# vivian556123/NeurIPS2024-CoVoMix

Measured on AMD Instinct MI355X. Metric: mel-frames/sec (VoMix 32-step + HiFi-GAN, Bx1000x80), higher is better.
Workload: dtype f16x3->f32 (fp32 operands split into fp16 hi/lo pairs, 3 MFMA products, fp32 accumulate); 1 GPU; VoMix 32-NFE (16 midpoint steps, CFG 0.7) + HiFi-GAN config_covomix, B=8 utterances x T=1000 frames per GPU, prompt 400; per_gpu_batch=8, frames=1000, nfe=32, parallelism=dp1 (utterance-sharded)

## Files before the change

### include/covomix_hip.h

```cpp
#ifndef COVOMIX_HIP_H
#define COVOMIX_HIP_H

#include <stdint.h>

#ifdef __cplusplus
extern "C" {
#endif

#define CVX_OK      0
#define CVX_EINVAL (-22)
#define CVX_EHIP   (-5)

#define CVX_ACT_NONE 0
#define CVX_ACT_GELU 1
#define CVX_ACT_SILU 2
#define CVX_ACT_TANH 3

typedef struct cvx_ctx {
    void*     stream;
    uint32_t* sat_flag;
    int32_t   n_cus;
    int32_t   flags;
} cvx_ctx;
#define CVX_CTX_NO_SATURATION_FLAG 1
typedef const cvx_ctx* cvx_stream_t;

#define CVX_ABI_VERSION 113
int         cvx_version(void);
const char* cvx_last_error_string(void);

int cvx_saturation_flag_reset(cvx_stream_t ctx);
int cvx_saturation_flag_query(uint32_t* host_out, int32_t reset, cvx_stream_t ctx);

int cvx_clock_stamps(uint64_t* stamps_dev, cvx_stream_t ctx);
int cvx_stream_create_cu_mask(const uint32_t* mask, int32_t n_words, void** out_stream);
int cvx_stream_destroy(void* stream);

typedef struct {
    const float* A;   int64_t lda;
    const float* A2;  int64_t lda2;  int32_t K1;
    const float* W;   int64_t ldw;
    float*       C;   int64_t ldc;
    const float* bias;
    const float* residual; int64_t ldr;
    int32_t M, N, K;
    int32_t act;
    const float* rope_cos; const float* rope_sin; int32_t rope_T; int32_t rope_cols;
} cvx_gemm_args;
int cvx_gemm_bias_act_f32(const cvx_gemm_args* a, cvx_stream_t s);

#define CVX_GEMM_F32_FORM_T64          0
#define CVX_GEMM_F32_FORM_T64_GENERIC  1
#define CVX_GEMM_F32_FORM_T128_DMA     2
#define CVX_GEMM_F32_FORM_T128_GENERIC 3
int cvx_gemm_f32_form(int32_t M, int32_t N, int32_t K);

typedef struct {
    const uint16_t* A_hi;  const uint16_t* A_lo;  int64_t lda_h;
    const uint16_t* A2_hi; const uint16_t* A2_lo; int64_t lda2_h;
    uint16_t* C_hi; uint16_t* C_lo; int64_t ldc_h;
    int32_t write_f32;
    uint16_t* Vt_hi; uint16_t* Vt_lo; int64_t vt_ld;
    float* workspace; int64_t workspace_floats;
    int32_t w_interleaved;
    int32_t flags;
    const float* a_scale_dev; const float* c_scale_dev; const float* vt_scale_dev;
    const float* c_gamma_dev; float* c_rowsq; int64_t c_rowsq_ld; const float* a_row_scale_dev;
    const uint16_t* R_hi; const uint16_t* R_lo; int64_t ldr_h; const float* r_scale_dev;
    const float* a2_scale_dev;
} cvx_gemm_split_io;
#define CVX_GEMM_FLAG_MEDIUM 8
#define CVX_GEMM_FLAG_NO_MEDIUM 16
#define CVX_GEMM_FLAG_ONE_TILE 4
#define CVX_GEMM_FLAG_TILE192 64
#define CVX_GEMM_FLAG_TILE256 128
#define CVX_GEMM_FLAG_TILE_MIXED 32
#define CVX_GEMM_FLAG_VT_PIECES 512
int cvx_split_f16(const float* w, uint16_t* hi, uint16_t* lo, int64_t n, float scale, cvx_stream_t s);
int cvx_split_f16_colscale_il(const float* W, int64_t ldw, int32_t N, int32_t K, const float* colscale, int64_t cs_ld,
                              const float* set_scale_dev, int64_t ss_ld, int32_t n_sets, float scale, uint16_t* out, cvx_stream_t s);
int cvx_split_f16_dev(const float* w, uint16_t* hi, uint16_t* lo, int64_t n, float scale, const float* scale_dev, cvx_stream_t s);
int cvx_gemm_f16x3(const cvx_gemm_args* a, const uint16_t* W_hi, const uint16_t* W_lo, float acc_scale,
                   const cvx_gemm_split_io* io, cvx_stream_t s);
typedef struct {
    const float* gamma; const float* beta;
    uint16_t* Y_hi; uint16_t* Y_lo; int64_t ldy_h;
    const float* y_scale_dev;
    float scale; float eps;
} cvx_gemm_norm;
int cvx_gemm_f16x3_norm(const cvx_gemm_args* a, const uint16_t* W_hi, const uint16_t* W_lo, float acc_scale,
                        const cvx_gemm_split_io* io, const cvx_gemm_norm* norm, cvx_stream_t s);
int64_t cvx_gemm_f16x3_workspace_floats(int32_t M, int32_t N, int32_t K, int32_t K1);

int cvx_adarmsnorm_f32(const float* x, const float* gamma, const float* beta, float* y,
                       uint16_t* y_hi, uint16_t* y_lo,
                       int64_t rows, int32_t D, int64_t rows_per_group, float scale, float eps,
                       cvx_stream_t s);
int cvx_rownorm_scale_f32(const float* rowsq, int64_t rows, int32_t parts, int64_t ld, float scale, float eps, float* out, cvx_stream_t s);
int cvx_adarmsnorm_scaled_f32(const float* x, const float* gamma, const float* beta, float* y,
                              uint16_t* y_hi, uint16_t* y_lo,
                              int64_t rows, int32_t D, int64_t rows_per_group, float scale, float eps,
                              const float* split_scale_dev, cvx_stream_t s);

int cvx_attention_f32(const float* qkv, float* out,
                      uint16_t* out_hi, uint16_t* out_lo,
                      int32_t Bt, int32_t T, int32_t H, float scale, cvx_stream_t s);

int cvx_attention_varlen_f32(const float* qkv, float* out, uint16_t* out_hi, uint16_t* out_lo,
                             const int32_t* cu_seqlens_dev, int32_t n_seq, int32_t max_T, int32_t H, float scale, cvx_stream_t s);

int cvx_attention_f16x3(const uint16_t* qk_hi, const uint16_t* qk_lo, const uint16_t* vt_hi, const uint16_t* vt_lo,
                        float* out, uint16_t* out_hi, uint16_t* out_lo,
                        int32_t Bt, int32_t T, int32_t Tp, int32_t H, float scale, cvx_stream_t s);
int cvx_attention_f16x3_scaled(const uint16_t* qk_hi, const uint16_t* qk_lo, const uint16_t* vt_hi, const uint16_t* vt_lo,
                               float* out, uint16_t* out_hi, uint16_t* out_lo,
                               int32_t Bt, int32_t T, int32_t Tp, int32_t H, float scale,
                               const float* qk_scale_dev, const float* v_scale_dev, const float* out_scale_dev, cvx_stream_t s);
int cvx_attention_f16x3_varlen(const uint16_t* qk_hi, const uint16_t* qk_lo, const uint16_t* vt_hi, const uint16_t* vt_lo,
                               float* out, uint16_t* out_hi, uint16_t* out_lo, const int32_t* cu_seqlens_dev,
                               int32_t n_seq, int32_t max_T, int64_t M, int32_t vt_ld, int32_t H, float scale,
                               const float* qk_scale_dev, const float* v_scale_dev, const float* out_scale_dev, cvx_stream_t s);

#define CVX_ATT_FORM_A 0
#define CVX_ATT_FORM_B 1
#define CVX_ATT_FORM_C 2
#define CVX_ATT_FORM_D 3
#define CVX_ATT_FORM_SINGLE_TERM 4
int cvx_attention_f16x3_form(int32_t n_seq, int32_t max_T, int64_t q_rows, int32_t H, int32_t single_term,
                             int32_t* query_block, int32_t* key_groups, int32_t* query_waves);

int cvx_dwconv31_gelu_res_f32(const float* x, const float* w, const float* bias, float* y,
                              int32_t Bt, int32_t T, int32_t C, cvx_stream_t s);
int cvx_dwconv31_gelu_res_varlen_f32(const float* x, const float* w, const float* bias, float* y,
                                     const int32_t* cu_seqlens_dev, int32_t n_seq, int32_t max_T, int32_t C, cvx_stream_t s);
int cvx_gemm_skinny_f32(const float* A, int32_t lda, const float* W, int64_t ldw, const float* bias, float* C, int64_t ldc,
                        int32_t M, int32_t N, int32_t K, int32_t act, cvx_stream_t s);
int cvx_cfg_combine_axpy_f32(const float* f_c, const float* f_n, const float* y, float cond_scale,
                             float coef, float* out, float* out2, float* out3, int64_t n, cvx_stream_t s);
int cvx_rk_stage_f32(const float* f_c, const float* f_n, const float* y, float cond_scale, const float* row_scale,
                     const float* const* k_prev, const float* w, int32_t m, float* k_out, float* out, float* out2, float* out3,
                     int64_t rows, int32_t dim, cvx_stream_t s);
#define CVX_RK_ERR_ROWS 32
int cvx_rk_stage_err_f32(const float* f_c, const float* f_n, const float* y, float cond_scale, const float* row_scale,
                         const float* const* k_prev, const float* w, const float* we, int32_t m, float* k_out, float* out, float* out2,
                         float* out3, int64_t rows, int32_t dim, const int32_t* map_dev, const int32_t* map_host, int32_t blocks,
                         float* partials, cvx_stream_t s);
int cvx_rk_err_finish_f32(const float* partials, const int32_t* map_dev, int32_t blocks, int32_t steps, int32_t n_seq, float* err,
                          cvx_stream_t s);

int cvx_embed_gather_f32(const int64_t* ids, int32_t S, const float* table, int32_t E, int32_t n_rows_table,
                         const float* cond, const float* cond_row, int32_t Cc, int64_t null_id,
                         float* out, int64_t M, cvx_stream_t s);

int cvx_time_fourier_f32(const float* times, const float* w, float* out, int32_t n, int32_t half,
                         cvx_stream_t s);

typedef struct { const int32_t* item_len_dev; int32_t mul, add; } cvx_item_lengths;
typedef struct {
    const float* x;  int32_t B, Cin, Lin;
    const float* Wp; const float* bias;
    float* out;      int32_t Cout, Lout;
    int32_t ksize, dil, pad, up;
    float in_slope;
    const float* res; const float* accum; float out_scale;
    cvx_item_lengths items;
} cvx_conv_args;
int     cvx_hifigan_conv1d_f32(const cvx_conv_args* a, cvx_stream_t s);
int64_t cvx_hifigan_packed_weight_floats(int32_t Cout, int32_t Cin, int32_t ksize);
int     cvx_hifigan_pack_weight_f32(const float* w, int32_t Cout, int32_t Cin, int32_t ksize,
                                    int32_t transposed, float* Wp);

int     cvx_hifigan_conv_transpose1d_f32(const cvx_conv_args* a, uint32_t* amax_bits_dev, cvx_stream_t s);
int64_t cvx_hifigan_conv_transpose1d_packed_floats(int32_t Cout, int32_t Cin, int32_t ksize, int32_t stride, int32_t pad_t);
int     cvx_hifigan_pack_conv_transpose1d_f32(const float* w, int32_t Cin, int32_t Cout, int32_t ksize, int32_t stride,
                                              int32_t pad_t, float* Wp);
int     cvx_pow2_scale_from_amax_f32(uint32_t* amax_bits_dev, float target, float* scale_dev, cvx_stream_t s);

int cvx_hifigan_post_f32(const float* x, const float* w, float bias, float* y,
                         int32_t B, int32_t Cin, int32_t L, float slope, cvx_stream_t s);

typedef struct {
    const uint16_t *z_hi, *z_lo;
    int32_t B, L, Lp, Cp_in, halo_l;
    const uint16_t *w_hi, *w_lo;
    float acc_scale;
    const float* bias;
    int32_t Np, ksize, dil;
    const float* res;
    const float* accum;
    float* out_x;
    float out_scale;
    uint16_t *out_zhi, *out_zlo;
    float z_slope;
    const float* z_scale_dev;
    cvx_item_lengths items;
} cvx_conv16_args;
int cvx_hifigan_conv1d_f16x3(const cvx_conv16_args* a, cvx_stream_t s);
int cvx_hifigan_conv1d_group_f16x3(const cvx_conv16_args* a, int32_t n, cvx_stream_t s);
int cvx_hifigan_conv1d_f16x3_form(int32_t Np, int32_t L, int32_t B, int32_t n_problems, int32_t cus);

typedef struct {
    const uint16_t *w_hi, *w_lo; float acc_scale; const float* bias;
} cvx_conv16_weights;
typedef struct {
    const float* x; const uint16_t *z_hi, *z_lo;
    int32_t B, L, Lp, Np, halo_l;
    cvx_conv16_weights c1[3], c2[3];
    int32_t ksize; int32_t dil[3];
    uint16_t *t_hi, *t_lo;
    float* xa; uint16_t *za_hi, *za_lo;
    float* xb; uint16_t *zb_hi, *zb_lo;
    const float* accum; float* out; float out_scale;
    const float* z_scale_dev;
    cvx_item_lengths items;
} cvx_resblock16_args;
int cvx_hifigan_resblock_f16x3(const cvx_resblock16_args* a, cvx_stream_t s);
int cvx_hifigan_resblock_stage_f16x3(const cvx_resblock16_args* blocks, int32_t n, cvx_stream_t s);

typedef struct {
    const float* x;
    int32_t B, L, Lp, Np, halo_l;
    cvx_conv16_weights c1, c2;
    int32_t ksize, dil;
    const float* accum; float* out; float out_scale;
    const float* z_scale_dev;
    int32_t flags;
    cvx_item_lengths items;
} cvx_respair16_args;
int cvx_hifigan_resblock_pair_f16x3(const cvx_respair16_args* a, cvx_stream_t s);

int cvx_hifigan_to_channels_last(const float* x, float* x_cl, uint16_t* z_hi, uint16_t* z_lo, int32_t B, int32_t C,
                                 int32_t L, int32_t Lp, int32_t Cp, int32_t halo_l, float slope, cvx_stream_t s);
int cvx_hifigan_to_channels_last_scaled(const float* x, float* x_cl, uint16_t* z_hi, uint16_t* z_lo, int32_t B, int32_t C,
                                        int32_t L, int32_t Lp, int32_t Cp, int32_t halo_l, float slope,
                                        const float* z_scale_dev ,
                                        cvx_stream_t s);
int cvx_hifigan_from_channels_last(const float* x_cl, float* x, int32_t B, int32_t C, int32_t L, int32_t Lp,
                                   int32_t Cp, int32_t halo_l, cvx_stream_t s);
typedef struct {
    const uint16_t *z_hi, *z_lo;
    int32_t B, L_in, Lp_in, Cp_in, halo_in;
    const uint16_t *w_hi, *w_lo;
    float acc_scale;
    const float* bias;
    int32_t Np_out, stride, n_tiles, tile_np;
    int32_t tile_taps[8], tile_pad[8];
    int64_t tile_w_off[8];
    float* out;
    int32_t L_out, Lp_out, halo_out;
    const float* z_scale_dev;
    uint32_t* amax_bits_dev;
    cvx_item_lengths items;
} cvx_convt16_args;
int cvx_hifigan_conv_transpose1d_f16x3(const cvx_convt16_args* a, cvx_stream_t s);
int cvx_hifigan_split_channels_last(const float* x_cl, uint16_t* z_hi, uint16_t* z_lo, int64_t n, float slope,
                                    const float* z_scale_dev, cvx_stream_t s);
int cvx_hifigan_post_channels_last_f32(const float* x_cl, const float* w, float bias, float* y, int32_t B, int32_t C, int32_t Np,
                                       int32_t L, int32_t Lp, int32_t halo_l, float slope, cvx_stream_t s);
int cvx_amax_pow2_scale_f32(const float* x, int64_t n, float target, float* scale_dev, uint32_t* scratch_dev, cvx_stream_t s);

int cvx_mel_magnitude_f32(const float* spec, float* mag, int64_t T, int32_t nb, int32_t nbp, cvx_stream_t s);
int cvx_mel_log_transpose_f32(const float* x, float* y, int64_t T, int32_t n_mels, cvx_stream_t s);

int cvx_wav_to_int16(const float* wav, int16_t* pcm, int64_t n, cvx_stream_t s);

typedef struct {
    const float *gamma_s, *wqkv_s, *wo_s;
    const float *gamma_c, *wq_c, *wo_c;
    const float *kv_c;
    const float *gamma_f, *w1, *b1, *w2, *b2;
    float *k_cache, *v_cache;
} cvx_t2s_layer;

typedef struct {
    int32_t dim, inner, heads, ff_inner, ff_inner_pad, depth, streams, vocab, dim_emb, n_ctx, max_len, top_k;
    int32_t batch, ctx_rows;
    float temperature;
    const cvx_t2s_layer* layers;
    const float *final_gamma, *emb, *rope_cos, *rope_sin, *uniforms;
    float *x, *q, *att, *h, *logits;
    int64_t* tokens;
    int32_t* state;
    float cfg_scale;
    int32_t uniform_steps;
    int32_t* queue;
    int32_t* dialogues;
    const float* start;
    int32_t filter_mode;
    float top_p;
    int32_t n_dialogues;
} cvx_t2s_decoder;

#define CVX_T2S_FILTER_TOP_K 0
#define CVX_T2S_FILTER_TOP_P 1

int cvx_t2s_decode_steps(const cvx_t2s_decoder* dec, int32_t n_steps, cvx_stream_t stream);

typedef struct {
    uint32_t struct_size;
    int32_t logprob_len;
    float* logprobs;
} cvx_t2s_scoring;

int cvx_t2s_decode_steps_scored(const cvx_t2s_decoder* dec, const cvx_t2s_scoring* scoring, int32_t n_steps, cvx_stream_t stream);

typedef struct cvx_t2s_per_dialogue {
    uint32_t struct_size;
    int32_t n_records;
    const void* table;
} cvx_t2s_per_dialogue;

int cvx_t2s_decode_steps_per_dialogue(const cvx_t2s_decoder* dec, const cvx_t2s_scoring* scoring, const cvx_t2s_per_dialogue* per,
                                      int32_t n_steps, cvx_stream_t stream);

#define CVX_T2S_FLAG_GUIDED 4

typedef struct cvx_t2s_mixed {
    uint32_t struct_size;
    int32_t n_guided;
} cvx_t2s_mixed;

int cvx_t2s_decode_steps_mixed(const cvx_t2s_decoder* dec, const cvx_t2s_scoring* scoring, const cvx_t2s_per_dialogue* per,
                               const cvx_t2s_mixed* mixed, int32_t n_steps, cvx_stream_t stream);

typedef struct cvx_t2s_rules {
    uint32_t struct_size;
    int32_t n_records;
    const void* table;
} cvx_t2s_rules;

int cvx_t2s_decode_steps_rules(const cvx_t2s_decoder* dec, const cvx_t2s_scoring* scoring, const cvx_t2s_per_dialogue* per,
                               const cvx_t2s_mixed* mixed, const cvx_t2s_rules* rules, int32_t n_steps, cvx_stream_t stream);

int cvx_t2s_rules_f32(const float* logits, const int64_t* history, const int32_t* hist_len, const void* table, int64_t rows, int32_t V,
                      int32_t hist_ld, int32_t eos_id, float* out, cvx_stream_t stream);

typedef struct cvx_t2s_beam {
    uint32_t struct_size;
    int32_t beam_size;
    int32_t hist_len;
    int32_t backtrack;
    float* scores;
    uint8_t* finished;
    int32_t* owner;
    int32_t* groups;
    int32_t* parents;
    int32_t* hist_tokens;
    float* hist_logprobs;
    float* short_lp;
    int32_t* short_tokens;
    float* logprobs;
} cvx_t2s_beam;

int cvx_t2s_beam_steps(const cvx_t2s_decoder* dec, const cvx_t2s_beam* beam, int32_t n_steps, cvx_stream_t stream);

typedef struct cvx_t2s_beam_queue {
    uint32_t struct_size;
    int32_t n_utterances;
    int32_t* queue;
    int32_t* utterances;
    const float* start;
    int32_t* parents;
    int32_t* hist_tokens;
    float* hist_logprobs;
    float* final_scores;
    int32_t* final_steps;
    uint8_t* final_finished;
    int64_t* tokens;
    float* logprobs;
} cvx_t2s_beam_queue;

int cvx_t2s_beam_queue_steps(const cvx_t2s_decoder* dec, const cvx_t2s_beam* beam, const cvx_t2s_beam_queue* bq, int32_t n_steps,
                             cvx_stream_t stream);

int cvx_t2s_beam_guided_steps(const cvx_t2s_decoder* dec, const cvx_t2s_beam* beam, int32_t n_steps, cvx_stream_t stream);

int cvx_t2s_beam_guided_queue_steps(const cvx_t2s_decoder* dec, const cvx_t2s_beam* beam, const cvx_t2s_beam_queue* bq, int32_t n_steps,
                                    cvx_stream_t stream);

int cvx_t2s_beam_select_f32(const float* logits, const float* scores_in, const uint8_t* finished_in, int32_t groups, int32_t beam_size,
                            int32_t streams, int32_t V, int32_t* parents, int64_t* tokens, float* token_lp, float* scores_out,
                            uint8_t* finished_out, cvx_stream_t stream);

int cvx_t2s_logprob_f32(const float* logits, const int64_t* tokens, int64_t rows, int32_t V, float* out, cvx_stream_t stream);

int cvx_t2s_sample_f32(const float* logits, const float* uniforms, int64_t rows, int32_t V, int32_t filter_mode, int32_t k,
                       float thres, float temperature, int64_t* tokens, uint8_t* kept, cvx_stream_t stream);

int cvx_geglu_f32(const float* h, float* out, int64_t rows, int32_t F, int64_t ld_out, cvx_stream_t stream);

int cvx_rope_attention_f32(const float* qkv, const float* rope_cos, const float* rope_sin, float* out,
                           int32_t Bt, int32_t T, int32_t H, float scale, float* workspace, cvx_stream_t s);
int64_t cvx_rope_attention_workspace_floats(int32_t Bt, int32_t T, int32_t H);
int cvx_hifigan_convt_f32(const cvx_conv_args* a, cvx_stream_t s);
typedef struct {
    const float* x; int32_t B, C, L;
    const float* Wp1[3]; const float* b1[3];
    const float* Wp2[3]; const float* b2[3];
    int32_t ksize; int32_t dil[3];
    float* tmp; float* out;
    const float* accum; float out_scale;
} cvx_resblock_args;
int cvx_hifigan_resblock_f32(const cvx_resblock_args* a, cvx_stream_t s);
int cvx_hifigan_pre_post_f32(const cvx_conv_args* pre, const float* post_x, const float* post_w, float post_bias,
                             float* post_y, int32_t B, int32_t C, int32_t L, float slope, cvx_stream_t s);


int64_t cvx_hubert_conv0_workspace_floats(int64_t L, int32_t C);
int cvx_hubert_conv0_gn_gelu_f32(const float* wav, int64_t n_samples, const float* w, int32_t C, int32_t k, int32_t stride,
                                 const float* gn_gamma, const float* gn_beta, float eps,
                                 float* out, float* workspace, int64_t workspace_floats, cvx_stream_t s);

int cvx_layernorm_f32(const float* x, const float* gamma, const float* beta, float* y,
                      int64_t rows, int32_t D, float eps, cvx_stream_t s);

int cvx_hubert_group_pack_f32(const float* x, float* out, int32_t T, int32_t D, int32_t groups, int32_t halo, cvx_stream_t s);

int cvx_kmeans_argmin_f32(const float* x, const float* dots, const float* cnorm, int64_t* labels, float* margin,
                          int64_t T, int32_t D, int32_t K, cvx_stream_t s);

typedef struct {
    const float* w; const uint16_t* w_hi; const uint16_t* w_lo; float inv_scale;
    const float* bias;
    int32_t N, K;
} cvx_linear;
typedef struct {
    cvx_linear qkv, out, fc1, fc2;
    const float *ln1_g, *ln1_b, *ln2_g, *ln2_b;
} cvx_hubert_layer;
typedef struct {
    int32_t n_conv; int32_t conv_k[8], conv_stride[8], conv_c[8];
    const float *conv0_w, *gn_g, *gn_b;
    cvx_linear conv[8];
    const float *ln_g, *ln_b;
    cvx_linear proj;
    int32_t dim, heads, pos_k, pos_groups;
    const cvx_linear* pos;
    const float *enc_ln_g, *enc_ln_b;
    int32_t n_layers; const cvx_hubert_layer* layers;
} cvx_hubert_model;
int32_t cvx_hubert_frames(const cvx_hubert_model* m, int64_t n_samples);
int64_t cvx_hubert_workspace_bytes(const cvx_hubert_model* m, int64_t n_samples);
int cvx_hubert_extract_features(const cvx_hubert_model* m, const float* wav, int64_t n_samples, int32_t output_layer,
                                float* out, void* workspace, int64_t workspace_bytes, cvx_stream_t s);

int cvx_resample_fir_f32(const float* x, int64_t n, const float* kern, int32_t up, int32_t down, int32_t width,
                         float* out, int64_t n_out, cvx_stream_t s);

#ifdef __cplusplus
}
#endif
#endif
```

### neurips2024-covomix_amd/_lib.py

```python
from __future__ import annotations

import ctypes as C
import os

import torch

_HERE = os.path.dirname(os.path.abspath(__file__))
LIB_PATH = os.environ.get("CVX_LIB_PATH") or os.path.join(_HERE, "libcovomix_hip.so")

_f32p = C.POINTER(C.c_float)
ABI_VERSION = 113


class GemmArgs(C.Structure):
    _fields_ = [
        ("A", C.c_void_p), ("lda", C.c_int64),
        ("A2", C.c_void_p), ("lda2", C.c_int64), ("K1", C.c_int32),
        ("W", C.c_void_p), ("ldw", C.c_int64),
        ("C", C.c_void_p), ("ldc", C.c_int64),
        ("bias", C.c_void_p),
        ("residual", C.c_void_p), ("ldr", C.c_int64),
        ("M", C.c_int32), ("N", C.c_int32), ("K", C.c_int32),
        ("act", C.c_int32),
        ("rope_cos", C.c_void_p), ("rope_sin", C.c_void_p), ("rope_T", C.c_int32), ("rope_cols", C.c_int32),
    ]


class GemmSplitIO(C.Structure):
    _fields_ = [
        ("A_hi", C.c_void_p), ("A_lo", C.c_void_p), ("lda_h", C.c_int64),
        ("A2_hi", C.c_void_p), ("A2_lo", C.c_void_p), ("lda2_h", C.c_int64),
        ("C_hi", C.c_void_p), ("C_lo", C.c_void_p), ("ldc_h", C.c_int64),
        ("write_f32", C.c_int32),
        ("Vt_hi", C.c_void_p), ("Vt_lo", C.c_void_p), ("vt_ld", C.c_int64),
        ("workspace", C.c_void_p), ("workspace_floats", C.c_int64),
        ("w_interleaved", C.c_int32),
        ("flags", C.c_int32),
        ("a_scale_dev", C.c_void_p), ("c_scale_dev", C.c_void_p), ("vt_scale_dev", C.c_void_p),
        ("c_gamma_dev", C.c_void_p), ("c_rowsq", C.c_void_p), ("c_rowsq_ld", C.c_int64), ("a_row_scale_dev", C.c_void_p),
        ("R_hi", C.c_void_p), ("R_lo", C.c_void_p), ("ldr_h", C.c_int64), ("r_scale_dev", C.c_void_p),
        ("a2_scale_dev", C.c_void_p),
    ]


class GemmNorm(C.Structure):
    _fields_ = [
        ("gamma", C.c_void_p), ("beta", C.c_void_p),
        ("Y_hi", C.c_void_p), ("Y_lo", C.c_void_p), ("ldy_h", C.c_int64),
        ("y_scale_dev", C.c_void_p),
        ("scale", C.c_float), ("eps", C.c_float),
    ]


class ItemLengths(C.Structure):
    _fields_ = [("item_len_dev", C.c_void_p), ("mul", C.c_int32), ("add", C.c_int32)]


class ConvArgs(C.Structure):
    _fields_ = [
        ("x", C.c_void_p), ("B", C.c_int32), ("Cin", C.c_int32), ("Lin", C.c_int32),
        ("Wp", C.c_void_p), ("bias", C.c_void_p),
        ("out", C.c_void_p), ("Cout", C.c_int32), ("Lout", C.c_int32),
        ("ksize", C.c_int32), ("dil", C.c_int32), ("pad", C.c_int32), ("up", C.c_int32),
        ("in_slope", C.c_float),
        ("res", C.c_void_p), ("accum", C.c_void_p), ("out_scale", C.c_float),
        ("items", ItemLengths),
    ]


class Conv16Args(C.Structure):
    _fields_ = [
        ("z_hi", C.c_void_p), ("z_lo", C.c_void_p),
        ("B", C.c_int32), ("L", C.c_int32), ("Lp", C.c_int32), ("Cp_in", C.c_int32), ("halo_l", C.c_int32),
        ("w_hi", C.c_void_p), ("w_lo", C.c_void_p), ("acc_scale", C.c_float), ("bias", C.c_void_p),
        ("Np", C.c_int32), ("ksize", C.c_int32), ("dil", C.c_int32),
        ("res", C.c_void_p), ("accum", C.c_void_p), ("out_x", C.c_void_p), ("out_scale", C.c_float),
        ("out_zhi", C.c_void_p), ("out_zlo", C.c_void_p), ("z_slope", C.c_float),
        ("z_scale_dev", C.c_void_p),
        ("items", ItemLengths),
    ]


class ConvT16Args(C.Structure):
    _fields_ = [
        ("z_hi", C.c_void_p), ("z_lo", C.c_void_p),
        ("B", C.c_int32), ("L_in", C.c_int32), ("Lp_in", C.c_int32), ("Cp_in", C.c_int32), ("halo_in", C.c_int32),
        ("w_hi", C.c_void_p), ("w_lo", C.c_void_p), ("acc_scale", C.c_float), ("bias", C.c_void_p),
        ("Np_out", C.c_int32), ("stride", C.c_int32), ("n_tiles", C.c_int32), ("tile_np", C.c_int32),
        ("tile_taps", C.c_int32 * 8), ("tile_pad", C.c_int32 * 8), ("tile_w_off", C.c_int64 * 8),
        ("out", C.c_void_p), ("L_out", C.c_int32), ("Lp_out", C.c_int32), ("halo_out", C.c_int32),
        ("z_scale_dev", C.c_void_p), ("amax_bits_dev", C.c_void_p),
        ("items", ItemLengths),
    ]


class Conv16Weights(C.Structure):
    _fields_ = [("w_hi", C.c_void_p), ("w_lo", C.c_void_p), ("acc_scale", C.c_float), ("bias", C.c_void_p)]


class Resblock16Args(C.Structure):
    _fields_ = [("x", C.c_void_p), ("z_hi", C.c_void_p), ("z_lo", C.c_void_p),
                ("B", C.c_int32), ("L", C.c_int32), ("Lp", C.c_int32), ("Np", C.c_int32), ("halo_l", C.c_int32),
                ("c1", Conv16Weights * 3), ("c2", Conv16Weights * 3),
                ("ksize", C.c_int32), ("dil", C.c_int32 * 3),
                ("t_hi", C.c_void_p), ("t_lo", C.c_void_p),
                ("xa", C.c_void_p), ("za_hi", C.c_void_p), ("za_lo", C.c_void_p),
                ("xb", C.c_void_p), ("zb_hi", C.c_void_p), ("zb_lo", C.c_void_p),
                ("accum", C.c_void_p), ("out", C.c_void_p), ("out_scale", C.c_float),
                ("z_scale_dev", C.c_void_p), ("items", ItemLengths)]


class Respair16Args(C.Structure):
    _fields_ = [("x", C.c_void_p),
                ("B", C.c_int32), ("L", C.c_int32), ("Lp", C.c_int32), ("Np", C.c_int32), ("halo_l", C.c_int32),
                ("c1", Conv16Weights), ("c2", Conv16Weights),
                ("ksize", C.c_int32), ("dil", C.c_int32),
                ("accum", C.c_void_p), ("out", C.c_void_p), ("out_scale", C.c_float),
                ("z_scale_dev", C.c_void_p), ("flags", C.c_int32), ("items", ItemLengths)]


class Ctx(C.Structure):
    _fields_ = [("stream", C.c_void_p), ("sat_flag", C.c_void_p), ("n_cus", C.c_int32), ("flags", C.c_int32)]


CTX_NO_SATURATION_FLAG = 1


class T2SLayer(C.Structure):
    _fields_ = [(n, C.c_void_p) for n in ("gamma_s", "wqkv_s", "wo_s", "gamma_c", "wq_c", "wo_c", "kv_c",
                                          "gamma_f", "w1", "b1", "w2", "b2", "k_cache", "v_cache")]


class T2SDecoder(C.Structure):
    _fields_ = [(n, C.c_int32) for n in ("dim", "inner", "heads", "ff_inner", "ff_inner_pad", "depth", "streams", "vocab",
                                         "dim_emb", "n_ctx", "max_len", "top_k", "batch", "ctx_rows")] + \
               [("temperature", C.c_float), ("layers", C.POINTER(T2SLayer))] + \
               [(n, C.c_void_p) for n in ("final_gamma", "emb", "rope_cos", "rope_sin", "uniforms",
                                          "x", "q", "att", "h", "logits", "tokens", "state")] + [("cfg_scale", C.c_float)] + \
               [("uniform_steps", C.c_int32), ("queue", C.c_void_p), ("dialogues", C.c_void_p), ("start", C.c_void_p)] + \
               [("filter_mode", C.c_int32), ("top_p", C.c_float), ("n_dialogues", C.c_int32)]


T2S_FILTER_TOP_K, T2S_FILTER_TOP_P = 0, 1
T2S_FLAG_IGNORE_EOS, T2S_FLAG_FORCED = 1, 2


class T2SScoring(C.Structure):
    _fields_ = [("struct_size", C.c_uint32), ("logprob_len", C.c_int32), ("logprobs", C.c_void_p)]


class T2SPerDialogue(C.Structure):
    _fields_ = [("struct_size", C.c_uint32), ("n_records", C.c_int32), ("table", C.c_void_p)]


T2S_PER_WORDS = 8
T2S_FLAG_GUIDED = 4


class T2SMixed(C.Structure):
    _fields_ = [("struct_size", C.c_uint32), ("n_guided", C.c_int32)]


class T2SRules(C.Structure):
    _fields_ = [("struct_size", C.c_uint32), ("n_records", C.c_int32), ("table", C.c_void_p)]


T2S_RULES_WORDS = 4
T2S_RULES_MAX_NGRAM = 8


class T2SBeam(C.Structure):
    _fields_ = [("struct_size", C.c_uint32), ("beam_size", C.c_int32), ("hist_len", C.c_int32), ("backtrack", C.c_int32)] + \
               [(n, C.c_void_p) for n in ("scores", "finished", "owner", "groups", "parents", "hist_tokens", "hist_logprobs", "short_lp",
                                          "short_tokens", "logprobs")]


class T2SBeamQueue(C.Structure):
    _fields_ = [("struct_size", C.c_uint32), ("n_utterances", C.c_int32)] + \
               [(n, C.c_void_p) for n in ("queue", "utterances", "start", "parents", "hist_tokens", "hist_logprobs", "final_scores",
                                          "final_steps", "final_finished", "tokens", "logprobs")]


class ResblockArgs(C.Structure):
    _fields_ = [("x", C.c_void_p), ("B", C.c_int32), ("C", C.c_int32), ("L", C.c_int32),
                ("Wp1", C.c_void_p * 3), ("b1", C.c_void_p * 3), ("Wp2", C.c_void_p * 3), ("b2", C.c_void_p * 3),
                ("ksize", C.c_int32), ("dil", C.c_int32 * 3),
                ("tmp", C.c_void_p), ("out", C.c_void_p), ("accum", C.c_void_p), ("out_scale", C.c_float)]


class Linear(C.Structure):
    _fields_ = [("w", C.c_void_p), ("w_hi", C.c_void_p), ("w_lo", C.c_void_p), ("inv_scale", C.c_float),
                ("bias", C.c_void_p), ("N", C.c_int32), ("K", C.c_int32)]


class HubertLayer(C.Structure):
    _fields_ = [("qkv", Linear), ("out", Linear), ("fc1", Linear), ("fc2", Linear)] + \
               [(n, C.c_void_p) for n in ("ln1_g", "ln1_b", "ln2_g", "ln2_b")]


class HubertModel(C.Structure):
    _fields_ = [("n_conv", C.c_int32), ("conv_k", C.c_int32 * 8), ("conv_stride", C.c_int32 * 8), ("conv_c", C.c_int32 * 8),
                ("conv0_w", C.c_void_p), ("gn_g", C.c_void_p), ("gn_b", C.c_void_p),
                ("conv", Linear * 8),
                ("ln_g", C.c_void_p), ("ln_b", C.c_void_p),
                ("proj", Linear),
                ("dim", C.c_int32), ("heads", C.c_int32), ("pos_k", C.c_int32), ("pos_groups", C.c_int32),
                ("pos", C.POINTER(Linear)),
                ("enc_ln_g", C.c_void_p), ("enc_ln_b", C.c_void_p),
                ("n_layers", C.c_int32), ("layers", C.POINTER(HubertLayer))]


SIGNATURES = {
    "cvx_version": (C.c_int, []),
    "cvx_hifigan_conv1d_f16x3": (C.c_int, [C.POINTER(Conv16Args), C.c_void_p]),
    "cvx_hifigan_conv_transpose1d_f16x3": (C.c_int, [C.POINTER(ConvT16Args), C.c_void_p]),
    "cvx_hifigan_split_channels_last": (C.c_int, [C.c_void_p, C.c_void_p, C.c_void_p, C.c_int64, C.c_float, C.c_void_p, C.c_void_p]),
    "cvx_hifigan_post_channels_last_f32": (C.c_int, [C.c_void_p, C.c_void_p, C.c_float, C.c_void_p, C.c_int32, C.c_int32, C.c_int32,
                                                     C.c_int32, C.c_int32, C.c_int32, C.c_float, C.c_void_p]),
    "cvx_hifigan_to_channels_last": (C.c_int, [C.c_void_p, C.c_void_p, C.c_void_p, C.c_void_p, C.c_int32, C.c_int32, C.c_int32,
                                               C.c_int32, C.c_int32, C.c_int32, C.c_float, C.c_void_p]),
    "cvx_hifigan_from_channels_last": (C.c_int, [C.c_void_p, C.c_void_p, C.c_int32, C.c_int32, C.c_int32, C.c_int32, C.c_int32,
                                                 C.c_int32, C.c_void_p]),
    "cvx_mel_magnitude_f32": (C.c_int, [C.c_void_p, C.c_void_p, C.c_int64, C.c_int32, C.c_int32, C.c_void_p]),
    "cvx_mel_log_transpose_f32": (C.c_int, [C.c_void_p, C.c_void_p, C.c_int64, C.c_int32, C.c_void_p]),
    "cvx_t2s_decode_steps": (C.c_int, [C.POINTER(T2SDecoder), C.c_int32, C.c_void_p]),
    "cvx_t2s_decode_steps_scored": (C.c_int, [C.POINTER(T2SDecoder), C.POINTER(T2SScoring), C.c_int32, C.c_void_p]),
    "cvx_t2s_decode_steps_per_dialogue": (C.c_int, [C.POINTER(T2SDecoder), C.POINTER(T2SScoring), C.POINTER(T2SPerDialogue), C.c_int32,
                                                    C.c_void_p]),
    "cvx_t2s_decode_steps_mixed": (C.c_int, [C.POINTER(T2SDecoder), C.POINTER(T2SScoring), C.POINTER(T2SPerDialogue), C.POINTER(T2SMixed),
                                             C.c_int32, C.c_void_p]),
    "cvx_t2s_decode_steps_rules": (C.c_int, [C.POINTER(T2SDecoder), C.POINTER(T2SScoring), C.POINTER(T2SPerDialogue), C.POINTER(T2SMixed),
                                             C.POINTER(T2SRules), C.c_int32, C.c_void_p]),
    "cvx_t2s_rules_f32": (C.c_int, [C.c_void_p, C.c_void_p, C.c_void_p, C.c_void_p, C.c_int64, C.c_int32, C.c_int32, C.c_int32, C.c_void_p,
                                    C.c_void_p]),
    "cvx_t2s_beam_steps": (C.c_int, [C.POINTER(T2SDecoder), C.POINTER(T2SBeam), C.c_int32, C.c_void_p]),
    "cvx_t2s_beam_queue_steps": (C.c_int, [C.POINTER(T2SDecoder), C.POINTER(T2SBeam), C.POINTER(T2SBeamQueue), C.c_int32, C.c_void_p]),
    "cvx_t2s_beam_guided_steps": (C.c_int, [C.POINTER(T2SDecoder), C.POINTER(T2SBeam), C.c_int32, C.c_void_p]),
    "cvx_t2s_beam_guided_queue_steps": (C.c_int, [C.POINTER(T2SDecoder), C.POINTER(T2SBeam), C.POINTER(T2SBeamQueue), C.c_int32, C.c_void_p]),
    "cvx_t2s_beam_select_f32": (C.c_int, [C.c_void_p, C.c_void_p, C.c_void_p, C.c_int32, C.c_int32, C.c_int32, C.c_int32, C.c_void_p, C.c_void_p,
                                          C.c_void_p, C.c_void_p, C.c_void_p, C.c_void_p]),
    "cvx_t2s_logprob_f32": (C.c_int, [C.c_void_p, C.c_void_p, C.c_int64, C.c_int32, C.c_void_p, C.c_void_p]),
    "cvx_t2s_sample_f32": (C.c_int, [C.c_void_p, C.c_void_p, C.c_int64, C.c_int32, C.c_int32, C.c_int32, C.c_float, C.c_float,
                                     C.c_void_p, C.c_void_p, C.c_void_p]),
    "cvx_geglu_f32": (C.c_int, [C.c_void_p, C.c_void_p, C.c_int64, C.c_int32, C.c_int64, C.c_void_p]),
    "cvx_hubert_conv0_workspace_floats": (C.c_int64, [C.c_int64, C.c_int32]),
    "cvx_hubert_conv0_gn_gelu_f32": (C.c_int, [C.c_void_p, C.c_int64, C.c_void_p, C.c_int32, C.c_int32, C.c_int32, C.c_void_p,
                                               C.c_void_p, C.c_float, C.c_void_p, C.c_void_p, C.c_int64, C.c_void_p]),
    "cvx_layernorm_f32": (C.c_int, [C.c_void_p, C.c_void_p, C.c_void_p, C.c_void_p, C.c_int64, C.c_int32, C.c_float, C.c_void_p]),
    "cvx_hubert_group_pack_f32": (C.c_int, [C.c_void_p, C.c_void_p, C.c_int32, C.c_int32, C.c_int32, C.c_int32, C.c_void_p]),
    "cvx_kmeans_argmin_f32": (C.c_int, [C.c_void_p, C.c_void_p, C.c_void_p, C.c_void_p, C.c_void_p, C.c_int64, C.c_int32,
                                        C.c_int32, C.c_void_p]),
    "cvx_resample_fir_f32": (C.c_int, [C.c_void_p, C.c_int64, C.c_void_p, C.c_int32, C.c_int32, C.c_int32, C.c_void_p,
                                       C.c_int64, C.c_void_p]),
    "cvx_hubert_frames": (C.c_int32, [C.POINTER(HubertModel), C.c_int64]),
    "cvx_hubert_workspace_bytes": (C.c_int64, [C.POINTER(HubertModel), C.c_int64]),
    "cvx_hubert_extract_features": (C.c_int, [C.POINTER(HubertModel), C.c_void_p, C.c_int64, C.c_int32, C.c_void_p, C.c_void_p,
                                              C.c_int64, C.c_void_p]),
    "cvx_rope_attention_f32": (C.c_int, [C.c_void_p, C.c_void_p, C.c_void_p, C.c_void_p, C.c_int32, C.c_int32, C.c_int32,
                                         C.c_float, C.c_void_p, C.c_void_p]),
    "cvx_hifigan_convt_f32": (C.c_int, [C.POINTER(ConvArgs), C.c_void_p]),
    "cvx_hifigan_resblock_f32": (C.c_int, [C.POINTER(ResblockArgs), C.c_void_p]),
    "cvx_hifigan_resblock_f16x3": (C.c_int, [C.POINTER(Resblock16Args), C.c_void_p]),
    "cvx_hifigan_resblock_stage_f16x3": (C.c_int, [C.POINTER(Resblock16Args), C.c_int32, C.c_void_p]),
    "cvx_hifigan_conv1d_group_f16x3": (C.c_int, [C.POINTER(Conv16Args), C.c_int32, C.c_void_p]),
    "cvx_hifigan_conv1d_f16x3_form": (C.c_int, [C.c_int32, C.c_int32, C.c_int32, C.c_int32, C.c_int32]),
    "cvx_hifigan_resblock_pair_f16x3": (C.c_int, [C.POINTER(Respair16Args), C.c_void_p]),
    "cvx_hifigan_conv_transpose1d_f32": (C.c_int, [C.POINTER(ConvArgs), C.c_void_p, C.c_void_p]),
    "cvx_hifigan_conv_transpose1d_packed_floats": (C.c_int64, [C.c_int32, C.c_int32, C.c_int32, C.c_int32, C.c_int32]),
    "cvx_hifigan_pack_conv_transpose1d_f32": (C.c_int, [C.c_void_p, C.c_int32, C.c_int32, C.c_int32, C.c_int32, C.c_int32, C.c_void_p]),
    "cvx_pow2_scale_from_amax_f32": (C.c_int, [C.c_void_p, C.c_float, C.c_void_p, C.c_void_p]),
    "cvx_hifigan_pre_post_f32": (C.c_int, [C.POINTER(ConvArgs), C.c_void_p, C.c_void_p, C.c_float, C.c_void_p, C.c_int32,
                                           C.c_int32, C.c_int32, C.c_float, C.c_void_p]),
    "cvx_last_error_string": (C.c_char_p, []),
    "cvx_gemm_bias_act_f32": (C.c_int, [C.POINTER(GemmArgs), C.c_void_p]),
    "cvx_gemm_f32_form": (C.c_int, [C.c_int32, C.c_int32, C.c_int32]),
    "cvx_split_f16": (C.c_int, [C.c_void_p, C.c_void_p, C.c_void_p, C.c_int64, C.c_float, C.c_void_p]),
    "cvx_gemm_f16x3_workspace_floats": (C.c_int64, [C.c_int32, C.c_int32, C.c_int32, C.c_int32]),
    "cvx_rope_attention_workspace_floats": (C.c_int64, [C.c_int32, C.c_int32, C.c_int32]),
    "cvx_hifigan_to_channels_last_scaled": (C.c_int, [C.c_void_p, C.c_void_p, C.c_void_p, C.c_void_p, C.c_int32, C.c_int32, C.c_int32,
                                                      C.c_int32, C.c_int32, C.c_int32, C.c_float, C.c_void_p, C.c_void_p]),
    "cvx_amax_pow2_scale_f32": (C.c_int, [C.c_void_p, C.c_int64, C.c_float, C.c_void_p, C.c_void_p, C.c_void_p]),
    "cvx_split_f16_dev": (C.c_int, [C.c_void_p, C.c_void_p, C.c_void_p, C.c_int64, C.c_float, C.c_void_p, C.c_void_p]),
    "cvx_split_f16_colscale_il": (C.c_int, [C.c_void_p, C.c_int64, C.c_int32, C.c_int32, C.c_void_p, C.c_int64, C.c_void_p, C.c_int64, C.c_int32,
                                            C.c_float, C.c_void_p, C.c_void_p]),
    "cvx_rownorm_scale_f32": (C.c_int, [C.c_void_p, C.c_int64, C.c_int32, C.c_int64, C.c_float, C.c_float, C.c_void_p, C.c_void_p]),
    "cvx_adarmsnorm_scaled_f32": (C.c_int, [C.c_void_p, C.c_void_p, C.c_void_p, C.c_void_p, C.c_void_p, C.c_void_p, C.c_int64,
                                            C.c_int32, C.c_int64, C.c_float, C.c_float, C.c_void_p, C.c_void_p]),
    "cvx_attention_f16x3_scaled": (C.c_int, [C.c_void_p, C.c_void_p, C.c_void_p, C.c_void_p, C.c_void_p, C.c_void_p, C.c_void_p,
                                             C.c_int32, C.c_int32, C.c_int32, C.c_int32, C.c_float, C.c_void_p, C.c_void_p,
                                             C.c_void_p, C.c_void_p]),
    "cvx_gemm_f16x3": (C.c_int, [C.POINTER(GemmArgs), C.c_void_p, C.c_void_p, C.c_float, C.POINTER(GemmSplitIO),
                                 C.c_void_p]),
    "cvx_gemm_f16x3_norm": (C.c_int, [C.POINTER(GemmArgs), C.c_void_p, C.c_void_p, C.c_float, C.POINTER(GemmSplitIO),
                                      C.POINTER(GemmNorm), C.c_void_p]),
    "cvx_adarmsnorm_f32": (C.c_int, [C.c_void_p, C.c_void_p, C.c_void_p, C.c_void_p, C.c_void_p, C.c_void_p, C.c_int64, C.c_int32,
                                     C.c_int64, C.c_float, C.c_float, C.c_void_p]),
    "cvx_attention_f32": (C.c_int, [C.c_void_p, C.c_void_p, C.c_void_p, C.c_void_p, C.c_int32, C.c_int32, C.c_int32, C.c_float,
                                    C.c_void_p]),
    "cvx_attention_f16x3": (C.c_int, [C.c_void_p, C.c_void_p, C.c_void_p, C.c_void_p, C.c_void_p, C.c_void_p, C.c_void_p,
                                      C.c_int32, C.c_int32, C.c_int32, C.c_int32, C.c_float, C.c_void_p]),
    "cvx_dwconv31_gelu_res_f32": (C.c_int, [C.c_void_p, C.c_void_p, C.c_void_p, C.c_void_p, C.c_int32, C.c_int32,
                                            C.c_int32, C.c_void_p]),
    "cvx_cfg_combine_axpy_f32": (C.c_int, [C.c_void_p, C.c_void_p, C.c_void_p, C.c_float, C.c_float, C.c_void_p,
                                           C.c_void_p, C.c_void_p, C.c_int64, C.c_void_p]),
    "cvx_rk_stage_f32": (C.c_int, [C.c_void_p, C.c_void_p, C.c_void_p, C.c_float, C.c_void_p, C.POINTER(C.c_void_p), C.POINTER(C.c_float),
                                   C.c_int32, C.c_void_p, C.c_void_p, C.c_void_p, C.c_void_p, C.c_int64, C.c_int32, C.c_void_p]),
    "cvx_rk_stage_err_f32": (C.c_int, [C.c_void_p, C.c_void_p, C.c_void_p, C.c_float, C.c_void_p, C.POINTER(C.c_void_p), C.POINTER(C.c_float),
                                       C.POINTER(C.c_float), C.c_int32, C.c_void_p, C.c_void_p, C.c_void_p, C.c_void_p, C.c_int64, C.c_int32,
                                       C.c_void_p, C.c_void_p, C.c_int32, C.c_void_p, C.c_void_p]),
    "cvx_rk_err_finish_f32": (C.c_int, [C.c_void_p, C.c_void_p, C.c_int32, C.c_int32, C.c_int32, C.c_void_p, C.c_void_p]),
    "cvx_embed_gather_f32": (C.c_int, [C.c_void_p, C.c_int32, C.c_void_p, C.c_int32, C.c_int32, C.c_void_p,
                                       C.c_void_p, C.c_int32, C.c_int64, C.c_void_p, C.c_int64, C.c_void_p]),
    "cvx_time_fourier_f32": (C.c_int, [C.c_void_p, C.c_void_p, C.c_void_p, C.c_int32, C.c_int32, C.c_void_p]),
    "cvx_hifigan_conv1d_f32": (C.c_int, [C.POINTER(ConvArgs), C.c_void_p]),
    "cvx_hifigan_packed_weight_floats": (C.c_int64, [C.c_int32, C.c_int32, C.c_int32]),
    "cvx_hifigan_pack_weight_f32": (C.c_int, [C.c_void_p, C.c_int32, C.c_int32, C.c_int32, C.c_int32, C.c_void_p]),
    "cvx_hifigan_post_f32": (C.c_int, [C.c_void_p, C.c_void_p, C.c_float, C.c_void_p, C.c_int32, C.c_int32,
                                       C.c_int32, C.c_float, C.c_void_p]),
    "cvx_wav_to_int16": (C.c_int, [C.c_void_p, C.c_void_p, C.c_int64, C.c_void_p]),
    "cvx_saturation_flag_reset": (C.c_int, [C.c_void_p]),
    "cvx_saturation_flag_query": (C.c_int, [C.POINTER(C.c_uint32), C.c_int32, C.c_void_p]),
    "cvx_stream_create_cu_mask": (C.c_int, [C.POINTER(C.c_uint32), C.c_int32, C.POINTER(C.c_void_p)]),
    "cvx_stream_destroy": (C.c_int, [C.c_void_p]),
    "cvx_clock_stamps": (C.c_int, [C.c_void_p, C.c_void_p]),
    "cvx_attention_varlen_f32": (C.c_int, [C.c_void_p, C.c_void_p, C.c_void_p, C.c_void_p, C.c_void_p, C.c_int32, C.c_int32,
                                           C.c_int32, C.c_float, C.c_void_p]),
    "cvx_attention_f16x3_varlen": (C.c_int, [C.c_void_p, C.c_void_p, C.c_void_p, C.c_void_p, C.c_void_p, C.c_void_p, C.c_void_p,
                                             C.c_void_p, C.c_int32, C.c_int32, C.c_int64, C.c_int32, C.c_int32, C.c_float,
                                             C.c_void_p, C.c_void_p, C.c_void_p, C.c_void_p]),
    "cvx_attention_f16x3_form": (C.c_int, [C.c_int32, C.c_int32, C.c_int64, C.c_int32, C.c_int32, C.POINTER(C.c_int32), C.POINTER(C.c_int32),
                                           C.POINTER(C.c_int32)]),
    "cvx_gemm_skinny_f32": (C.c_int, [C.c_void_p, C.c_int32, C.c_void_p, C.c_int64, C.c_void_p, C.c_void_p, C.c_int64, C.c_int32, C.c_int32,
                                      C.c_int32, C.c_int32, C.c_void_p]),
    "cvx_dwconv31_gelu_res_varlen_f32": (C.c_int, [C.c_void_p, C.c_void_p, C.c_void_p, C.c_void_p, C.c_void_p, C.c_int32,
                                                   C.c_int32, C.c_int32, C.c_void_p]),
}

_lib = None


class CovomixHipError(RuntimeError):
    pass


def load() -> C.CDLL:
    global _lib
    if _lib is not None:
        return _lib
    if not os.path.isfile(LIB_PATH):
        raise CovomixHipError(
            f"{LIB_PATH} not found: the gfx950 HIP library has not been built. "
            "Run `python -c 'import __graft_entry__ as g; g.build()'` (needs hipcc). "
            "covomix_amd has no CPU / PyTorch fallback.")
    lib = C.CDLL(LIB_PATH)
    lib.cvx_version.restype = C.c_int
    if lib.cvx_version() != ABI_VERSION:
        raise CovomixHipError(f"{LIB_PATH} reports ABI version {lib.cvx_version()}, this binding is written for {ABI_VERSION}: "
                              "rebuild the library (`python -c 'import __graft_entry__ as g; g.build()'`)")
    for name, (res, args) in SIGNATURES.items():
        fn = getattr(lib, name)
        fn.restype = res
        fn.argtypes = args
    _lib = lib
    return lib


_DEBUG_SYNC = os.environ.get("CVX_DEBUG_SYNC") == "1"


def check(rc: int, what: str = "") -> None:
    if _DEBUG_SYNC:
        import sys
        import torch
        print("[cvx]", what, file=sys.stderr, flush=True)
        torch.cuda.synchronize()
    if rc != 0:
        msg = load().cvx_last_error_string()
        raise CovomixHipError(f"{what or 'covomix_hip'} failed (rc={rc}): {msg.decode() if msg else ''}")
```

### neurips2024-covomix_amd/csrc/elementwise.hip

```cpp
#include "cvx_common.h"
#include <algorithm>
#include <stdarg.h>
#include <string.h>

static thread_local char g_err[512] = "";
void cvx_set_error(const char* fmt, ...)
{
    va_list ap;
    va_start(ap, fmt);
    vsnprintf(g_err, sizeof(g_err), fmt, ap);
    va_end(ap);
}
extern "C" const char* cvx_last_error_string(void) { return g_err; }

#include <mutex>
#include <map>
#include <set>
#include <utility>
void cvx_allow_dynamic_lds(const void* kernel, int bytes)
{
    static std::mutex mu;
    static std::map<std::pair<int, const void*>, int> granted;
    int dev = 0;
    if (hipGetDevice(&dev) != hipSuccess) dev = 0;
    std::lock_guard<std::mutex> lock(mu);
    int& g = granted[std::make_pair(dev, kernel)];
    if (bytes > g) {
        (void)hipFuncSetAttribute(kernel, hipFuncAttributeMaxDynamicSharedMemorySize, bytes);
        g = bytes;
    }
}
int cvx_device_cus()
{
    static std::mutex mu;
    static int n_cu[64] = {};
    int dev = 0;
    if (hipGetDevice(&dev) != hipSuccess || dev < 0 || dev >= 64) dev = 0;
    std::lock_guard<std::mutex> lock(mu);
    if (n_cu[dev] == 0) {
        int v = 0;
        if (hipDeviceGetAttribute(&v, hipDeviceAttributeMultiprocessorCount, dev) != hipSuccess || v <= 0) v = 256;
        n_cu[dev] = v;
    }
    return n_cu[dev];
}
extern "C" int cvx_stream_create_cu_mask(const uint32_t* mask, int32_t n_words, void** out)
{
    CVX_REQUIRE(mask && out && n_words > 0 && n_words <= 64, "stream_create_cu_mask: bad arguments");
    int bits = 0;
    for (int i = 0; i < n_words; ++i) bits += __builtin_popcount(mask[i]);
    CVX_REQUIRE(bits > 0, "stream_create_cu_mask: empty mask");
    hipStream_t st = nullptr;
    const hipError_t e = hipExtStreamCreateWithCUMask(&st, (uint32_t)n_words, mask);
    if (e != hipSuccess) { cvx_set_error("stream_create_cu_mask: hipExtStreamCreateWithCUMask failed: %s", hipGetErrorString(e)); return CVX_EHIP; }
    *out = reinterpret_cast<void*>(st);
    return CVX_OK;
}
extern "C" int cvx_stream_destroy(void* stream)
{
    CVX_REQUIRE(stream, "stream_destroy: the NULL stream");
    const hipError_t e = hipStreamDestroy(reinterpret_cast<hipStream_t>(stream));
    if (e != hipSuccess) { cvx_set_error("stream_destroy: %s", hipGetErrorString(e)); return CVX_EHIP; }
    return CVX_OK;
}
extern "C" int cvx_saturation_flag_reset(cvx_stream_t s)
{
    uint32_t* f = cvx_sat_flag_for(s);
    CVX_REQUIRE(f && (reinterpret_cast<uintptr_t>(f) & 3) == 0, "saturation_flag_reset: the context carries no (4-byte aligned) saturation flag");
    if (hipMemsetAsync(f, 0, sizeof(uint32_t), cvx_hip_stream(s)) != hipSuccess) { cvx_set_error("saturation_flag: memset failed"); return CVX_EHIP; }
    return CVX_OK;
}
extern "C" int cvx_saturation_flag_query(uint32_t* host_out, int32_t reset, cvx_stream_t s)
{
    uint32_t* f = cvx_sat_flag_for(s);
    CVX_REQUIRE(f && host_out, "saturation_flag_query: the context carries no saturation flag / null output");
    hipStream_t st = cvx_hip_stream(s);
    if (hipMemcpyAsync(host_out, f, sizeof(uint32_t), hipMemcpyDeviceToHost, st) != hipSuccess ||
        hipStreamSynchronize(st) != hipSuccess) { cvx_set_error("saturation_flag: read failed: %s", hipGetErrorString(hipGetLastError())); return CVX_EHIP; }
    if (reset && hipMemsetAsync(f, 0, sizeof(uint32_t), st) != hipSuccess) { cvx_set_error("saturation_flag: memset failed"); return CVX_EHIP; }
    return CVX_OK;
}
namespace {
__global__ __launch_bounds__(64) void clock_stamp_kernel(unsigned long long* __restrict__ out)
{
    unsigned xcc, hwid;
    asm volatile("s_getreg_b32 %0, hwreg(HW_REG_XCC_ID)" : "=s"(xcc));
    asm volatile("s_getreg_b32 %0, hwreg(HW_REG_HW_ID)" : "=s"(hwid));
    __builtin_amdgcn_s_sleep(64);
    const unsigned long long t = __builtin_readcyclecounter(), r = __builtin_amdgcn_s_memrealtime();
    const unsigned slot = ((xcc & 7) << 8) | ((hwid >> 8) & 0xFF);
    if (threadIdx.x == 0) { out[2 * slot] = t; out[2 * slot + 1] = r; }
}
}
extern "C" int cvx_clock_stamps(uint64_t* stamps_dev, cvx_stream_t s)
{
    CVX_REQUIRE(stamps_dev && (reinterpret_cast<uintptr_t>(stamps_dev) & 7) == 0, "clock_stamps: null / unaligned output");
    hipLaunchKernelGGL(clock_stamp_kernel, dim3(4096), dim3(64), 0, cvx_hip_stream(s), reinterpret_cast<unsigned long long*>(stamps_dev));
    CVX_CHECK_LAUNCH("cvx_clock_stamps");
    return CVX_OK;
}
extern "C" int cvx_version(void) { return CVX_ABI_VERSION; }

namespace {

__device__ __forceinline__ float wave_sum(float v)
{
#pragma unroll
    for (int o = 32; o > 0; o >>= 1) v += __shfl_xor(v, o, 64);
    return v;
}

typedef _Float16 f16x4_t __attribute__((ext_vector_type(4)));
__device__ __forceinline__ void store_split4(_Float16* hi, _Float16* lo, int64_t off, const f32x4 o, CvxSat& amax)
{
    cvx_amax4(amax, o);
    if (lo == hi + 32) off = ((off >> 5) << 6) | (off & 31);
    f16x4_t h, l;
#pragma unroll
    for (int e = 0; e < 4; ++e) {
        const float x = fminf(fmaxf(o[e], -65504.f), 65504.f);
        h[e] = (_Float16)x;
        l[e] = (_Float16)(x - (float)h[e]);
    }
    *reinterpret_cast<f16x4_t*>(hi + off) = h;
    if (lo) *reinterpret_cast<f16x4_t*>(lo + off) = l;
}

template <int NV>
__global__ __launch_bounds__(256) void adarmsnorm_kernel(const float* __restrict__ x, const float* __restrict__ gamma,
                                                        const float* __restrict__ beta, float* __restrict__ y,
                                                        _Float16* __restrict__ y_hi, _Float16* __restrict__ y_lo,
                                                        int64_t rows, int D, int64_t rows_per_group, float scale, float eps,
                                                        const float* __restrict__ split_scale, uint32_t* __restrict__ sat)
{
    const int lane = threadIdx.x & 63;
    const int64_t row = (int64_t)blockIdx.x * 4 + (threadIdx.x >> 6);
    if (row >= rows) return;
    CvxSat amax;
    const float ssc = split_scale ? *split_scale : 1.f;
    const float* xr = x + row * D;
    const int64_t g = row / rows_per_group;
    const float* gr = gamma + g * D;
    const float* br = beta ? beta + g * D : nullptr;
    float* yr = y ? y + row * D : nullptr;
    const int nvec = D >> 2;

    f32x4 v[NV], gv[NV], bv[NV];
#pragma unroll
    for (int i = 0; i < NV; ++i) {
        const int j = lane + 64 * i;
        if (j < nvec) v[i] = gload4(xr + 4 * j);
    }
#pragma unroll
    for (int i = 0; i < NV; ++i) {
        const int j = lane + 64 * i;
        if (j < nvec) {
            gv[i] = gload4(gr + 4 * j);
            if (br) bv[i] = gload4(br + 4 * j);
        }
    }
    float ss = 0.f;
#pragma unroll
    for (int i = 0; i < NV; ++i) {
        const int j = lane + 64 * i;
        if (j < nvec) ss += v[i][0] * v[i][0] + v[i][1] * v[i][1] + v[i][2] * v[i][2] + v[i][3] * v[i][3];
    }
    ss = wave_sum(ss);
    const float inv = scale / fmaxf(sqrtf(ss), eps);
#pragma unroll
    for (int i = 0; i < NV; ++i) {
        const int j = lane + 64 * i;
        if (j < nvec) {
            const f32x4 gg = gv[i];
            f32x4 o;
#pragma unroll
            for (int e = 0; e < 4; ++e) o[e] = v[i][e] * inv * gg[e];
            if (br) {
                const f32x4 bb = bv[i];
#pragma unroll
                for (int e = 0; e < 4; ++e) o[e] += bb[e];
            }
            if (y) *reinterpret_cast<f32x4*>(yr + 4 * j) = o;
            if (y_hi) { const f32x4 os = {o[0] * ssc, o[1] * ssc, o[2] * ssc, o[3] * ssc}; store_split4(y_hi, y_lo, row * D + 4 * j, os, amax); }
        }
    }
    cvx_sat_commit(sat, amax);
}

__global__ __launch_bounds__(256) void adarmsnorm_generic_kernel(const float* __restrict__ x, const float* __restrict__ gamma,
                                                                const float* __restrict__ beta, float* __restrict__ y,
                                                                _Float16* __restrict__ y_hi, _Float16* __restrict__ y_lo,
                                                                int64_t rows, int D, int64_t rows_per_group, float scale, float eps,
                                                                const float* __restrict__ split_scale, uint32_t* __restrict__ sat)
{
    const int lane = threadIdx.x & 63;
    const int64_t row = (int64_t)blockIdx.x * 4 + (threadIdx.x >> 6);
    if (row >= rows) return;
    CvxSat amax;
    const float ssc = split_scale ? *split_scale : 1.f;
    const float* xr = x + row * D;
    const int64_t g = row / rows_per_group;
    float ss = 0.f;
    for (int j = lane; j < (D >> 2); j += 64) {
        const f32x4 t = *reinterpret_cast<const f32x4*>(xr + 4 * j);
        ss += t[0] * t[0] + t[1] * t[1] + t[2] * t[2] + t[3] * t[3];
    }
    ss = wave_sum(ss);
    const float inv = scale / fmaxf(sqrtf(ss), eps);
    for (int j = lane; j < (D >> 2); j += 64) {
        const f32x4 t = *reinterpret_cast<const f32x4*>(xr + 4 * j);
        const f32x4 gg = *reinterpret_cast<const f32x4*>(gamma + g * D + 4 * j);
        f32x4 o;
#pragma unroll
        for (int e = 0; e < 4; ++e) o[e] = t[e] * inv * gg[e];
        if (beta) {
            const f32x4 bb = *reinterpret_cast<const f32x4*>(beta + g * D + 4 * j);
#pragma unroll
            for (int e = 0; e < 4; ++e) o[e] += bb[e];
        }
        if (y) *reinterpret_cast<f32x4*>(y + row * D + 4 * j) = o;
        if (y_hi) { const f32x4 os = {o[0] * ssc, o[1] * ssc, o[2] * ssc, o[3] * ssc}; store_split4(y_hi, y_lo, row * D + 4 * j, os, amax); }
    }
    cvx_sat_commit(sat, amax);
}

constexpr int DW_K = 31, DW_TT = 16;
__global__ __launch_bounds__(256) void dwconv31_kernel(const float* __restrict__ x, const float* __restrict__ w,
                                                      const float* __restrict__ bias, float* __restrict__ y,
                                                      int T, int C, const int* __restrict__ cu_seqlens)
{
    const int c = blockIdx.x * 256 + threadIdx.x;
    if (c >= C) return;
    const int t0 = blockIdx.y * DW_TT;
    int64_t base = (int64_t)blockIdx.z * T * C;
    if (cu_seqlens) {
        const int r0 = cu_seqlens[blockIdx.z];
        T = cu_seqlens[blockIdx.z + 1] - r0;
        base = (int64_t)r0 * C;
        if (t0 >= T) return;
    }
    float wk[DW_K];
#pragma unroll
    for (int k = 0; k < DW_K; ++k) wk[k] = w[c * DW_K + k];
    float xs[DW_TT + DW_K - 1];
#pragma unroll
    for (int i = 0; i < DW_TT + DW_K - 1; ++i) {
        const int t = t0 + i - DW_K / 2;
        xs[i] = (t >= 0 && t < T) ? x[base + (int64_t)t * C + c] : 0.f;
    }
    const float bc = bias[c];
#pragma unroll
    for (int o = 0; o < DW_TT; o += 2) {
        float a0 = bc, a1 = bc;
#pragma unroll
        for (int k = 0; k < DW_K; ++k) { a0 = fmaf(wk[k], xs[o + k], a0); a1 = fmaf(wk[k], xs[o + 1 + k], a1); }
        const f32x2 g2 = gelu_fast2(f32x2{a0, a1});
        const int t = t0 + o;
        if (t < T) y[base + (int64_t)t * C + c] = g2[0] + xs[o + DW_K / 2];
        if (t + 1 < T) y[base + (int64_t)(t + 1) * C + c] = g2[1] + xs[o + 1 + DW_K / 2];
    }
}

constexpr int SK_M = 32;
constexpr int SK_KC = 1024;
constexpr int SK_Q = 16;
__global__ __launch_bounds__(256) void gemm_skinny_kernel(const float* __restrict__ A, int lda, const float* __restrict__ W, int64_t ldw,
                                                         const float* __restrict__ bias, float* __restrict__ Cm, int64_t ldc,
                                                         int M, int N, int K, int act)
{
    extern __shared__ __attribute__((aligned(16))) float sk_a[];
    const int tid = threadIdx.x, lane = tid & 63, wid = tid >> 6;
    const int KC = min(K, SK_KC), ldA = KC + 4;
    const int i31 = lane & 31, g = lane >> 5;
    const float* ar = sk_a + (size_t)i31 * ldA + 4 * g;
    const int n_tiles = (N + 31) / 32;
    for (int tile0 = blockIdx.x * 4; tile0 < n_tiles; tile0 += gridDim.x * 4) {
        const int tile = tile0 + wid;
        const bool active = tile < n_tiles;
        const int n0 = tile * 32;
        f32x16 acc0, acc1;
#pragma unroll
        for (int r = 0; r < 16; ++r) { acc0[r] = 0.f; acc1[r] = 0.f; }
        for (int kc = 0; kc < K; kc += KC) {
            const int kn = min(KC, K - kc), k4 = kn >> 2, nq = kn >> 3;
            __syncthreads();
            for (int i = tid; i < SK_M * k4; i += 256) {
                const int m = i / k4, c = i - m * k4;
                *reinterpret_cast<f32x4*>(sk_a + (size_t)m * ldA + 4 * c) = m < M ? gload4(A + (size_t)m * lda + kc + 4 * c) : f32x4{0.f, 0.f, 0.f, 0.f};
            }
            __syncthreads();
            if (!active) continue;
            const float* wr = W + (int64_t)min(n0 + i31, N - 1) * ldw + kc + 4 * g;
            f32x4 wb[2][SK_Q];
#pragma unroll
            for (int u = 0; u < SK_Q; ++u) wb[0][u] = u < nq ? gload4_nt(wr + 8 * u) : f32x4{0.f, 0.f, 0.f, 0.f};
            for (int q0 = 0; q0 < nq; q0 += 2 * SK_Q) {
#pragma unroll
                for (int half = 0; half < 2; ++half) {
                    const int qb = q0 + half * SK_Q;
                    if (qb < nq) {
#pragma unroll
                        for (int u = 0; u < SK_Q; ++u)
                            wb[half ^ 1][u] = qb + SK_Q + u < nq ? gload4_nt(wr + 8 * (qb + SK_Q + u)) : f32x4{0.f, 0.f, 0.f, 0.f};
#pragma unroll
                        for (int u = 0; u < SK_Q; ++u) {
                            if (qb + u < nq) {
                                const f32x4 av = *reinterpret_cast<const f32x4*>(ar + 8 * (qb + u));
                                const f32x4 wv = wb[half][u];
                                acc0 = __builtin_amdgcn_mfma_f32_32x32x2f32(wv[0], av[0], acc0, 0, 0, 0);
                                acc1 = __builtin_amdgcn_mfma_f32_32x32x2f32(wv[1], av[1], acc1, 0, 0, 0);
                                acc0 = __builtin_amdgcn_mfma_f32_32x32x2f32(wv[2], av[2], acc0, 0, 0, 0);
                                acc1 = __builtin_amdgcn_mfma_f32_32x32x2f32(wv[3], av[3], acc1, 0, 0, 0);
                            }
                        }
                    }
                }
            }
        }
        if (!active) continue;
        if (i31 < M) {
#pragma unroll
            for (int r = 0; r < 16; ++r) {
                const int n = n0 + (r & 3) + 8 * (r >> 2) + 4 * g;
                if (n < N) {
                    float v = acc0[r] + acc1[r];
                    if (bias) v += bias[n];
                    if (act == CVX_ACT_SILU) v = silu(v);
                    else if (act == CVX_ACT_GELU) v = gelu_erf(v);
                    else if (act == CVX_ACT_TANH) v = tanhf(v);
                    Cm[(int64_t)i31 * ldc + n] = v;
                }
            }
        }
    }
}

__global__ __launch_bounds__(256) void cfg_axpy_kernel(const float* __restrict__ fc, const float* __restrict__ fn,
                                                      const float* y, float s, float coef,
                                                      float* out, float* __restrict__ out2,
                                                      float* __restrict__ out3, int64_t n)
{
    const int64_t i = (int64_t)blockIdx.x * 256 + threadIdx.x;
    if (i >= n) return;
    float v = fc[i];
    if (fn) v = v * (1.0f + s) - s * fn[i];
    const float o = y[i] + v * coef;
    out[i] = o;
    if (out2) out2[i] = o;
    if (out3) out3[i] = o;
}

struct RkStage {
    const float* fc; const float* fn; const float* y; const float* row_scale;
    const float* k0; const float* k1; const float* k2;
    float wk0, wk1, wk2, wv, s;
    float* k_out; float* out; float* out2; float* out3;
    int64_t n;
    int dim;
};

__device__ __forceinline__ float rk_cfg_combine(float v, float f, float s)
{
#pragma clang fp contract(off)
    const float a = v * (1.0f + s), b = s * f;
    return a - b;
}

template <int V, bool KEEP = false>
__device__ __forceinline__ void rk_stage_elems(const RkStage& a, int64_t i0, float* vo = nullptr)
{
    float v[V], o[V];
    if constexpr (V == 4) {
        const float4 t = *reinterpret_cast<const float4*>(a.fc + i0);
        v[0] = t.x; v[1] = t.y; v[2] = t.z; v[3] = t.w;
    } else v[0] = a.fc[i0];
    if (a.fn) {
        float f[V], s[V];
        if constexpr (V == 4) {
            const float4 t = *reinterpret_cast<const float4*>(a.fn + i0);
            f[0] = t.x; f[1] = t.y; f[2] = t.z; f[3] = t.w;
        } else f[0] = a.fn[i0];
        if (a.row_scale) {
            int64_t r = i0 / a.dim;
            int rem = (int)(i0 - r * a.dim);
#pragma unroll
            for (int e = 0; e < V; ++e) {
                s[e] = a.row_scale[r];
                if (++rem == a.dim) { rem = 0; ++r; }
            }
#pragma unroll
            for (int e = 0; e < V; ++e)
                if (s[e] != 1.0f) v[e] = rk_cfg_combine(v[e], f[e], s[e]);
        } else {
#pragma unroll
            for (int e = 0; e < V; ++e) v[e] = rk_cfg_combine(v[e], f[e], a.s);
        }
    }
    if constexpr (V == 4) {
        const float4 t = *reinterpret_cast<const float4*>(a.y + i0);
        o[0] = t.x; o[1] = t.y; o[2] = t.z; o[3] = t.w;
    } else o[0] = a.y[i0];
    if (a.k_out) {
        if constexpr (V == 4) *reinterpret_cast<float4*>(a.k_out + i0) = make_float4(v[0], v[1], v[2], v[3]);
        else a.k_out[i0] = v[0];
    }
#define RK_ADD_STAGE(K, W)                                                              \
    if ((W) != 0.f) {                                                                   \
        if constexpr (V == 4) {                                                         \
            const float4 t = *reinterpret_cast<const float4*>((K) + i0);                \
            o[0] = __builtin_fmaf(t.x, (W), o[0]); o[1] = __builtin_fmaf(t.y, (W), o[1]);   \
            o[2] = __builtin_fmaf(t.z, (W), o[2]); o[3] = __builtin_fmaf(t.w, (W), o[3]);   \
        } else o[0] = __builtin_fmaf((K)[i0], (W), o[0]);                               \
    }
    RK_ADD_STAGE(a.k0, a.wk0)
    RK_ADD_STAGE(a.k1, a.wk1)
    RK_ADD_STAGE(a.k2, a.wk2)
#undef RK_ADD_STAGE
    if (a.wv != 0.f) {
#pragma unroll
        for (int e = 0; e < V; ++e) o[e] = __builtin_fmaf(v[e], a.wv, o[e]);
    }
    if constexpr (V == 4) {
        const float4 t = make_float4(o[0], o[1], o[2], o[3]);
        *reinterpret_cast<float4*>(a.out + i0) = t;
        if (a.out2) *reinterpret_cast<float4*>(a.out2 + i0) = t;
        if (a.out3) *reinterpret_cast<float4*>(a.out3 + i0) = t;
    } else {
        a.out[i0] = o[0];
        if (a.out2) a.out2[i0] = o[0];
        if (a.out3) a.out3[i0] = o[0];
    }
    if constexpr (KEEP) {
#pragma unroll
        for (int e = 0; e < V; ++e) { vo[e] = v[e]; vo[V + e] = o[e]; }
    }
}

template <int V>
__global__ __launch_bounds__(256) void rk_stage_kernel(const RkStage a)
{
    const int64_t i0 = ((int64_t)blockIdx.x * 256 + threadIdx.x) * V;
    if (i0 >= a.n) return;
    if (V == 1 || i0 + V <= a.n) { rk_stage_elems<V>(a, i0); return; }
    for (int64_t i = i0; i < a.n; ++i) rk_stage_elems<1>(a, i);
}

struct RkErr {
    const float* e0; const float* e1; const float* e2;
    float we0, we1, we2, wev;
    const int32_t* map;
    float2* partials;
};

template <int V>
__device__ __forceinline__ void rk_err_elems(const RkStage& a, const RkErr& e, int64_t i0, float& sd, float& so)
{
    float vo[2 * V], d[V];
    rk_stage_elems<V, true>(a, i0, vo);
    const float *v = vo, *o = vo + V;
#pragma unroll
    for (int l = 0; l < V; ++l) d[l] = 0.f;
#define RK_ERR_STAGE(K, W)                                                              \
    if ((W) != 0.f) {                                                                   \
        if constexpr (V == 4) {                                                         \
            const float4 t = *reinterpret_cast<const float4*>((K) + i0);                \
            d[0] = __builtin_fmaf(t.x, (W), d[0]); d[1] = __builtin_fmaf(t.y, (W), d[1]);   \
            d[2] = __builtin_fmaf(t.z, (W), d[2]); d[3] = __builtin_fmaf(t.w, (W), d[3]);   \
        } else d[0] = __builtin_fmaf((K)[i0], (W), d[0]);                               \
    }
    RK_ERR_STAGE(e.e0, e.we0)
    RK_ERR_STAGE(e.e1, e.we1)
    RK_ERR_STAGE(e.e2, e.we2)
#undef RK_ERR_STAGE
    if (e.wev != 0.f) {
#pragma unroll
        for (int l = 0; l < V; ++l) d[l] = __builtin_fmaf(v[l], e.wev, d[l]);
    }
#pragma unroll
    for (int l = 0; l < V; ++l) {
        sd = __builtin_fmaf(d[l], d[l], sd);
        so = __builtin_fmaf(o[l], o[l], so);
    }
}

template <int V>
__global__ __launch_bounds__(256) void rk_err_stage_kernel(const RkStage a, const RkErr e)
{
    __shared__ float red[8];
    const int32_t* mp = e.map + 3 * (int64_t)blockIdx.x;
    const int64_t base = (int64_t)mp[0] * a.dim;
    const int64_t cnt = (base >= 0 && base < a.n) ? ((int64_t)mp[1] * a.dim < a.n - base ? (int64_t)mp[1] * a.dim : a.n - base) : 0;
    float sd = 0.f, so = 0.f;
    for (int64_t i = (int64_t)threadIdx.x * V; i < cnt; i += 256 * V) rk_err_elems<V>(a, e, base + i, sd, so);
    sd = wave_sum(sd);
    so = wave_sum(so);
    const int wave = threadIdx.x >> 6;
    if ((threadIdx.x & 63) == 0) { red[wave] = sd; red[4 + wave] = so; }
    __syncthreads();
    if (threadIdx.x == 0)
        e.partials[blockIdx.x] = make_float2(((red[0] + red[1]) + red[2]) + red[3], ((red[4] + red[5]) + red[6]) + red[7]);
}

__global__ __launch_bounds__(256) void rk_err_finish_kernel(const float2* __restrict__ partials, const int32_t* __restrict__ map,
                                                            float2* __restrict__ err, int steps, int n_seq, int blocks)
{
    const int i = blockIdx.x * 256 + threadIdx.x;
    if (i >= steps * n_seq) return;
    const int step = i / n_seq, q = i - step * n_seq;
    const float2* p = partials + (int64_t)step * blocks;
    float sd = 0.f, so = 0.f;
    for (int b = 0; b < blocks; ++b)
        if (map[3 * b + 2] == q) { sd += p[b].x; so += p[b].y; }
    err[i] = make_float2(sd, so);
}

__global__ __launch_bounds__(256) void embed_gather_kernel(const int64_t* __restrict__ ids, int S,
                                                          const float* __restrict__ table, int E, int n_rows_table,
                                                          const float* __restrict__ cond, const float* __restrict__ cond_row,
                                                          int Cc, int64_t null_id, float* __restrict__ out)
{
    const int64_t m = blockIdx.x;
    const int width = S * E + Cc;
    float* o = out + m * width;
    for (int j = threadIdx.x; j < width; j += 256) {
        float v;
        if (j < S * E) {
            const int s = j / E, e = j - s * E;
            int64_t id = ids ? ids[m * S + s] : null_id;
            id = id < 0 ? 0 : (id >= n_rows_table ? n_rows_table - 1 : id);
            v = table[id * E + e];
        } else {
            const int cidx = j - S * E;
            v = cond_row ? cond_row[cidx] : cond[m * Cc + cidx];
        }
        o[j] = v;
    }
}

__global__ __launch_bounds__(256) void time_fourier_kernel(const float* __restrict__ times, const float* __restrict__ w,
                                                          float* __restrict__ out, int half)
{
    const int i = blockIdx.x;
    const float t = times[i];
    for (int j = threadIdx.x; j < half; j += 256) {
        const float ang = t * w[j] * 2.0f * 3.14159265358979323846f;
        out[(int64_t)i * 2 * half + j] = sinf(ang);
        out[(int64_t)i * 2 * half + half + j] = cosf(ang);
    }
}

__global__ __launch_bounds__(256) void wav_to_int16_kernel(const float* __restrict__ wav, int16_t* __restrict__ pcm, int64_t n)
{
    const int64_t i = (int64_t)blockIdx.x * 256 + threadIdx.x;
    if (i >= n) return;
    const float v = wav[i] * 32768.0f;
    pcm[i] = (int16_t)(int32_t)v;
}

__global__ __launch_bounds__(256) void mel_magnitude_kernel(const float* __restrict__ spec, float* __restrict__ mag,
                                                           int64_t T, int nb, int nbp)
{
    const int64_t i = (int64_t)blockIdx.x * 256 + threadIdx.x;
    if (i >= T * nbp) return;
    const int64_t t = i / nbp;
    const int k = (int)(i - t * nbp);
    float v = 0.f;
    if (k < nb) {
        const float re = spec[t * 2 * nb + k], im = spec[t * 2 * nb + nb + k];
        v = sqrtf(re * re + im * im + 1e-9f);
    }
    mag[i] = v;
}

__global__ __launch_bounds__(256) void mel_log_transpose_kernel(const float* __restrict__ x, float* __restrict__ y, int64_t T, int n_mels)
{
    const int64_t i = (int64_t)blockIdx.x * 256 + threadIdx.x;
    if (i >= T * n_mels) return;
    const int m = (int)(i / T);
    const int64_t t = i - (int64_t)m * T;
    y[i] = logf(fmaxf(x[t * n_mels + m], 1e-5f));
}

}

extern "C" int cvx_mel_magnitude_f32(const float* spec, float* mag, int64_t T, int32_t nb, int32_t nbp, cvx_stream_t s)
{
    CVX_REQUIRE(spec && mag && T >= 0 && nb > 0 && nbp >= nb, "mel_magnitude: bad arguments");
    if (T == 0) return CVX_OK;
    hipLaunchKernelGGL(mel_magnitude_kernel, dim3((unsigned)((T * nbp + 255) / 256)), dim3(256), 0, cvx_hip_stream(s),
                       spec, mag, T, nb, nbp);
    CVX_CHECK_LAUNCH("cvx_mel_magnitude_f32");
    return CVX_OK;
}

extern "C" int cvx_mel_log_transpose_f32(const float* x, float* y, int64_t T, int32_t n_mels, cvx_stream_t s)
{
    CVX_REQUIRE(x && y && T >= 0 && n_mels > 0, "mel_log_transpose: bad arguments");
    if (T == 0) return CVX_OK;
    hipLaunchKernelGGL(mel_log_transpose_kernel, dim3((unsigned)((T * n_mels + 255) / 256)), dim3(256), 0,
                       cvx_hip_stream(s), x, y, T, n_mels);
    CVX_CHECK_LAUNCH("cvx_mel_log_transpose_f32");
    return CVX_OK;
}

extern "C" int cvx_adarmsnorm_scaled_f32(const float* x, const float* gamma, const float* beta, float* y,
                                  uint16_t* y_hi_, uint16_t* y_lo_,
                                  int64_t rows, int32_t D, int64_t rows_per_group, float scale, float eps,
                                  const float* split_scale_dev, cvx_stream_t s)
{
    CVX_REQUIRE(x && gamma && (y || y_hi_) && (y_hi_ || !y_lo_), "adarmsnorm: null pointer");
    _Float16* y_hi = reinterpret_cast<_Float16*>(y_hi_);
    _Float16* y_lo = reinterpret_cast<_Float16*>(y_lo_);
    CVX_REQUIRE(rows >= 0 && D > 0 && D % 4 == 0 && rows_per_group > 0, "adarmsnorm: bad shape rows=%ld D=%d", (long)rows, D);
    CVX_REQUIRE(!(y_hi && y_lo == y_hi + 32) || D % 32 == 0, "adarmsnorm: an interleaved pair (y_lo == y_hi + 32) needs D %% 32 == 0 (D=%d)", D);
    if (rows == 0) return CVX_OK;
    hipStream_t st = cvx_hip_stream(s);
    dim3 grid((unsigned)((rows + 3) / 4));
    if (y_hi) CVX_REQUIRE_SAT(s);
    uint32_t* sat = y_hi ? cvx_sat_flag_for(s) : nullptr;
    if (D <= 256)       hipLaunchKernelGGL(adarmsnorm_kernel<1>, grid, dim3(256), 0, st, x, gamma, beta, y, y_hi, y_lo, rows, D, rows_per_group, scale, eps, split_scale_dev, sat);
    else if (D <= 512)  hipLaunchKernelGGL(adarmsnorm_kernel<2>, grid, dim3(256), 0, st, x, gamma, beta, y, y_hi, y_lo, rows, D, rows_per_group, scale, eps, split_scale_dev, sat);
    else if (D <= 1024) hipLaunchKernelGGL(adarmsnorm_kernel<4>, grid, dim3(256), 0, st, x, gamma, beta, y, y_hi, y_lo, rows, D, rows_per_group, scale, eps, split_scale_dev, sat);
    else                hipLaunchKernelGGL(adarmsnorm_generic_kernel, grid, dim3(256), 0, st, x, gamma, beta, y, y_hi, y_lo, rows, D, rows_per_group, scale, eps, split_scale_dev, sat);
    CVX_CHECK_LAUNCH("cvx_adarmsnorm_scaled_f32");
    return CVX_OK;
}

extern "C" int cvx_adarmsnorm_f32(const float* x, const float* gamma, const float* beta, float* y,
                                  uint16_t* y_hi, uint16_t* y_lo,
                                  int64_t rows, int32_t D, int64_t rows_per_group, float scale, float eps,
                                  cvx_stream_t s)
{
    return cvx_adarmsnorm_scaled_f32(x, gamma, beta, y, y_hi, y_lo, rows, D, rows_per_group, scale, eps, nullptr, s);
}

namespace {
__global__ __launch_bounds__(256) void rownorm_scale_kernel(const float* __restrict__ rowsq, int64_t rows, int parts, int64_t ld,
                                                            float scale, float eps, float* __restrict__ out)
{
    const int64_t r = (int64_t)blockIdx.x * 256 + threadIdx.x;
    if (r >= rows) return;
    const float* p = rowsq + r * ld;
    float q = 0.f;
    if ((parts & 3) == 0 && (ld & 3) == 0) {
        for (int j = 0; j < parts; j += 4) { const f32x4 v = gload4(p + j); q += v[0]; q += v[1]; q += v[2]; q += v[3]; }
    } else {
        for (int j = 0; j < parts; ++j) q += p[j];
    }
    out[r] = scale / fmaxf(sqrtf(q), eps);
}
}

extern "C" int cvx_rownorm_scale_f32(const float* rowsq, int64_t rows, int32_t parts, int64_t ld, float scale, float eps, float* out, cvx_stream_t s)
{
    CVX_REQUIRE(rowsq && out && rows >= 0 && parts > 0 && parts <= 64 && ld >= parts && (((uintptr_t)rowsq & 15) == 0 || (parts & 3) || (ld & 3)),
                "rownorm_scale: bad arguments (rows=%ld parts=%d ld=%ld)", (long)rows, parts, (long)ld);
    if (rows == 0) return CVX_OK;
    hipLaunchKernelGGL(rownorm_scale_kernel, dim3((unsigned)((rows + 255) / 256)), dim3(256), 0, cvx_hip_stream(s),
                       rowsq, rows, parts, ld, scale, eps, out);
    CVX_CHECK_LAUNCH("cvx_rownorm_scale_f32");
    return CVX_OK;
}

namespace {
__global__ __launch_bounds__(256) void amax_kernel(const float* __restrict__ x, int64_t n, unsigned* __restrict__ amax_bits)
{
    __shared__ float part[4];
    float m = 0.f;
    const int64_t n4 = n / 4, stride = (int64_t)gridDim.x * 256;
    int64_t i = (int64_t)blockIdx.x * 256 + threadIdx.x;
    for (; i + 3 * stride < n4; i += 4 * stride) {
        f32x4 v[4];
#pragma unroll
        for (int u = 0; u < 4; ++u) v[u] = gload4(x + 4 * (i + u * stride));
#pragma unroll
        for (int u = 0; u < 4; ++u) m = fmaxf(m, fmaxf(fmaxf(fabsf(v[u][0]), fabsf(v[u][1])), fmaxf(fabsf(v[u][2]), fabsf(v[u][3]))));
    }
    for (; i < n4; i += stride) {
        const f32x4 v = gload4(x + 4 * i);
        m = fmaxf(m, fmaxf(fmaxf(fabsf(v[0]), fabsf(v[1])), fmaxf(fabsf(v[2]), fabsf(v[3]))));
    }
    if (blockIdx.x == 0 && threadIdx.x < (n & 3)) m = fmaxf(m, fabsf(x[4 * n4 + threadIdx.x]));
#pragma unroll
    for (int o = 32; o > 0; o >>= 1) m = fmaxf(m, __shfl_xor(m, o, 64));
    if ((threadIdx.x & 63) == 0) part[threadIdx.x >> 6] = m;
    __syncthreads();
    if (threadIdx.x == 0) {
        m = fmaxf(fmaxf(part[0], part[1]), fmaxf(part[2], part[3]));
        if (m > 0.f && m < __builtin_inff() && __float_as_uint(m) > __atomic_load_n(amax_bits, __ATOMIC_RELAXED))
            atomicMax(amax_bits, __float_as_uint(m));
    }
}
__global__ void pow2_scale_kernel(const unsigned* __restrict__ amax_bits, float target, float* __restrict__ scale)
{
    const float a = __uint_as_float(*amax_bits);
    float e = 0.f;
    if (a > 0.f) e = fminf(fmaxf(rintf(log2f(target / a)), -40.f), 40.f);
    *scale = exp2f(e);
}
}

extern "C" int cvx_amax_pow2_scale_f32(const float* x, int64_t n, float target, float* scale_dev, uint32_t* scratch_dev, cvx_stream_t s)
{
    CVX_REQUIRE(x && scale_dev && scratch_dev && n >= 0 && target > 0.f && ((uintptr_t)x & 15) == 0, "amax_pow2_scale: bad arguments");
    hipStream_t st = cvx_hip_stream(s);
    if (hipMemsetAsync(scratch_dev, 0, sizeof(uint32_t), st) != hipSuccess) { cvx_set_error("amax_pow2_scale: memset failed"); return CVX_EHIP; }
    if (n > 0) {
        const unsigned blocks = (unsigned)((n / 4 + 1023) / 1024 < 2048 ? (n / 4 + 1023) / 1024 + 1 : 2048);
        hipLaunchKernelGGL(amax_kernel, dim3(blocks), dim3(256), 0, st, x, n, scratch_dev);
    }
    hipLaunchKernelGGL(pow2_scale_kernel, dim3(1), dim3(1), 0, st, scratch_dev, target, scale_dev);
    if (hipMemsetAsync(scratch_dev, 0, sizeof(uint32_t), st) != hipSuccess) { cvx_set_error("amax_pow2_scale: memset failed"); return CVX_EHIP; }
    CVX_CHECK_LAUNCH("cvx_amax_pow2_scale_f32");
    return CVX_OK;
}

extern "C" int cvx_pow2_scale_from_amax_f32(uint32_t* amax_bits_dev, float target, float* scale_dev, cvx_stream_t s)
{
    CVX_REQUIRE(amax_bits_dev && scale_dev && target > 0.f, "pow2_scale_from_amax: bad arguments");
    hipStream_t st = cvx_hip_stream(s);
    hipLaunchKernelGGL(pow2_scale_kernel, dim3(1), dim3(1), 0, st, amax_bits_dev, target, scale_dev);
    if (hipMemsetAsync(amax_bits_dev, 0, sizeof(uint32_t), st) != hipSuccess) { cvx_set_error("pow2_scale_from_amax: memset failed"); return CVX_EHIP; }
    CVX_CHECK_LAUNCH("cvx_pow2_scale_from_amax_f32");
    return CVX_OK;
}

extern "C" int cvx_dwconv31_gelu_res_varlen_f32(const float* x, const float* w, const float* bias, float* y,
                                                const int32_t* cu_seqlens_dev, int32_t Bt, int32_t max_T, int32_t C, cvx_stream_t s)
{
    CVX_REQUIRE(x && w && bias && y, "dwconv31: null pointer");
    CVX_REQUIRE(Bt >= 0 && max_T > 0 && C > 0 && Bt <= 65535, "dwconv31: bad shape");
    CVX_REQUIRE(x != y, "dwconv31: in-place operation is not supported");
    if (Bt == 0) return CVX_OK;
    dim3 grid((C + 255) / 256, (max_T + DW_TT - 1) / DW_TT, Bt);
    hipLaunchKernelGGL(dwconv31_kernel, grid, dim3(256), 0, cvx_hip_stream(s), x, w, bias, y, max_T, C, cu_seqlens_dev);
    CVX_CHECK_LAUNCH("cvx_dwconv31_gelu_res_f32");
    return CVX_OK;
}

extern "C" int cvx_gemm_skinny_f32(const float* A, int32_t lda, const float* W, int64_t ldw, const float* bias, float* C, int64_t ldc,
                                   int32_t M, int32_t N, int32_t K, int32_t act, cvx_stream_t s)
{
    CVX_REQUIRE(A && W && C && M >= 0 && M <= SK_M && N >= 0 && K > 0 && K % 8 == 0 && lda >= K && lda % 4 == 0 && ldw >= K &&
                ldw % 4 == 0 && ldc >= N && act >= CVX_ACT_NONE && act <= CVX_ACT_TANH,
                "gemm_skinny: M <= 32, K a multiple of 8, lda / ldw multiples of 4 (M=%d N=%d K=%d)", M, N, K);
    CVX_REQUIRE(((uintptr_t)A & 15) == 0 && ((uintptr_t)W & 15) == 0, "gemm_skinny: 16-byte aligned operands");
    if (M == 0 || N == 0) return CVX_OK;
    const size_t lds = (size_t)SK_M * (std::min(K, SK_KC) + 4) * sizeof(float);
    cvx_allow_dynamic_lds(reinterpret_cast<const void*>(&gemm_skinny_kernel), (int)lds);
    const int64_t groups = ((int64_t)N + 127) / 128;
    const unsigned grid = (unsigned)std::min<int64_t>(groups, (int64_t)cvx_ctx_cus(s));
    hipLaunchKernelGGL(gemm_skinny_kernel, dim3(grid), dim3(256), lds, cvx_hip_stream(s), A, lda, W, ldw, bias, C, ldc, M, N, K, act);
    CVX_CHECK_LAUNCH("cvx_gemm_skinny_f32");
    return CVX_OK;
}

extern "C" int cvx_dwconv31_gelu_res_f32(const float* x, const float* w, const float* bias, float* y,
                                         int32_t Bt, int32_t T, int32_t C, cvx_stream_t s)
{
    return cvx_dwconv31_gelu_res_varlen_f32(x, w, bias, y, nullptr, Bt, T, C, s);
}

extern "C" int cvx_cfg_combine_axpy_f32(const float* f_c, const float* f_n, const float* y, float cond_scale,
                                        float coef, float* out, float* out2, float* out3, int64_t n, cvx_stream_t s)
{
    CVX_REQUIRE(f_c && y && out && n >= 0, "cfg_axpy: bad arguments");
    if (n == 0) return CVX_OK;
    hipLaunchKernelGGL(cfg_axpy_kernel, dim3((unsigned)((n + 255) / 256)), dim3(256), 0, cvx_hip_stream(s),
                       f_c, f_n, y, cond_scale, coef, out, out2, out3, n);
    CVX_CHECK_LAUNCH("cvx_cfg_combine_axpy_f32");
    return CVX_OK;
}

static int rk_stage_args(RkStage& a, bool* vec, const float* f_c, const float* f_n, const float* y, float cond_scale, const float* row_scale,
                         const float* const* k_prev, const float* w, int32_t m, float* k_out, float* out, float* out2, float* out3,
                         int64_t rows, int32_t dim)
{
    CVX_REQUIRE(f_c && y && out && w, "rk_stage: f_c, y, out and w must not be null");
    CVX_REQUIRE(m >= 0 && m <= 3, "rk_stage: at most 3 stored stages (m=%d)", m);
    CVX_REQUIRE(rows >= 0 && dim > 0, "rk_stage: bad shape (rows=%lld dim=%d)", (long long)rows, dim);
    CVX_REQUIRE(!row_scale || f_n, "rk_stage: row_scale without f_n");
    CVX_REQUIRE(m == 0 || k_prev, "rk_stage: k_prev is null");
    const float* k[3] = {nullptr, nullptr, nullptr};
    float wk[3] = {0.f, 0.f, 0.f};
    for (int j = 0; j < m; ++j) {
        CVX_REQUIRE(k_prev[j] || w[j] == 0.f, "rk_stage: k_prev[%d] is null and its weight is not 0", j);
        if (w[j] != 0.f) { k[j] = k_prev[j]; wk[j] = w[j]; }
    }
    CVX_REQUIRE(rows <= (int64_t)0x7fffffffffffLL / dim, "rk_stage: rows x dim too large");
    a.fc = f_c; a.fn = f_n; a.y = y; a.row_scale = row_scale;
    a.k0 = k[0]; a.k1 = k[1]; a.k2 = k[2];
    a.wk0 = wk[0]; a.wk1 = wk[1]; a.wk2 = wk[2]; a.wv = w[m]; a.s = cond_scale;
    a.k_out = k_out; a.out = out; a.out2 = out2; a.out3 = out3;
    a.n = rows * dim; a.dim = dim;
    uintptr_t bits = (uintptr_t)f_c | (uintptr_t)f_n | (uintptr_t)y | (uintptr_t)k[0] | (uintptr_t)k[1] | (uintptr_t)k[2] |
                     (uintptr_t)k_out | (uintptr_t)out | (uintptr_t)out2 | (uintptr_t)out3;
    *vec = (bits & 15) == 0;
    return CVX_OK;
}

extern "C" int cvx_rk_stage_f32(const float* f_c, const float* f_n, const float* y, float cond_scale, const float* row_scale,
                                const float* const* k_prev, const float* w, int32_t m, float* k_out, float* out, float* out2,
                                float* out3, int64_t rows, int32_t dim, cvx_stream_t s)
{
    RkStage a = {};
    bool vec = false;
    const int rc = rk_stage_args(a, &vec, f_c, f_n, y, cond_scale, row_scale, k_prev, w, m, k_out, out, out2, out3, rows, dim);
    if (rc != CVX_OK) return rc;
    if (a.n == 0) return CVX_OK;
    const int64_t threads = vec ? (a.n + 3) / 4 : a.n;
    const int64_t blocks = (threads + 255) / 256;
    CVX_REQUIRE(blocks <= 0x7fffffffLL, "rk_stage: rows x dim too large for one launch");
    if (vec) hipLaunchKernelGGL(rk_stage_kernel<4>, dim3((unsigned)blocks), dim3(256), 0, cvx_hip_stream(s), a);
    else hipLaunchKernelGGL(rk_stage_kernel<1>, dim3((unsigned)blocks), dim3(256), 0, cvx_hip_stream(s), a);
    CVX_CHECK_LAUNCH("cvx_rk_stage_f32");
    return CVX_OK;
}

extern "C" int cvx_rk_stage_err_f32(const float* f_c, const float* f_n, const float* y, float cond_scale, const float* row_scale,
                                    const float* const* k_prev, const float* w, const float* we, int32_t m, float* k_out, float* out,
                                    float* out2, float* out3, int64_t rows, int32_t dim, const int32_t* map_dev, const int32_t* map_host,
                                    int32_t blocks, float* partials, cvx_stream_t s)
{
    RkStage a = {};
    bool vec = false;
    const int rc = rk_stage_args(a, &vec, f_c, f_n, y, cond_scale, row_scale, k_prev, w, m, k_out, out, out2, out3, rows, dim);
    if (rc != CVX_OK) return rc;
    CVX_REQUIRE(we && map_dev && map_host && partials, "rk_stage_err: we, the map (device and host copy) and partials must not be null");
    CVX_REQUIRE(((uintptr_t)map_dev & 3) == 0 && ((uintptr_t)partials & 7) == 0, "rk_stage_err: map 4-byte, partials 8-byte aligned");
    CVX_REQUIRE(blocks >= 0 && rows <= 0x7fffffffLL, "rk_stage_err: bad block count %d / rows beyond int32", blocks);
    RkErr e = {};
    const float* k[3] = {nullptr, nullptr, nullptr};
    float wk[3] = {0.f, 0.f, 0.f};
    for (int j = 0; j < m; ++j) {
        CVX_REQUIRE(k_prev[j] || we[j] == 0.f, "rk_stage_err: k_prev[%d] is null and its error weight is not 0", j);
        if (we[j] != 0.f) { k[j] = k_prev[j]; wk[j] = we[j]; }
    }
    int64_t next = 0;
    for (int b = 0; b < blocks; ++b) {
        const int32_t r0 = map_host[3 * b], nr = map_host[3 * b + 1], q = map_host[3 * b + 2];
        CVX_REQUIRE(r0 == next && nr >= 1 && nr <= CVX_RK_ERR_ROWS && q >= 0, "rk_stage_err: map entry %d (first row %d, rows %d, sequence %d) "
                    "does not continue at row %lld with 1..%d rows", b, r0, nr, q, (long long)next, CVX_RK_ERR_ROWS);
        if (b > 0) {
            const int32_t pq = map_host[3 * b - 1], pn = map_host[3 * b - 2];
            CVX_REQUIRE(q == pq ? pn == CVX_RK_ERR_ROWS : q > pq, "rk_stage_err: map entry %d: sequence %d after %d (a short chunk ends its sequence)", b, q, pq);
        }
        next += nr;
    }
    CVX_REQUIRE(next == rows, "rk_stage_err: the map covers %lld rows, the launch has %lld", (long long)next, (long long)rows);
    if (a.n == 0) return CVX_OK;
    e.e0 = k[0]; e.e1 = k[1]; e.e2 = k[2];
    e.we0 = wk[0]; e.we1 = wk[1]; e.we2 = wk[2]; e.wev = we[m];
    e.map = map_dev; e.partials = reinterpret_cast<float2*>(partials);
    vec = vec && (((uintptr_t)k[0] | (uintptr_t)k[1] | (uintptr_t)k[2]) & 15) == 0 && dim % 4 == 0;
    if (vec) hipLaunchKernelGGL(rk_err_stage_kernel<4>, dim3((unsigned)blocks), dim3(256), 0, cvx_hip_stream(s), a, e);
    else hipLaunchKernelGGL(rk_err_stage_kernel<1>, dim3((unsigned)blocks), dim3(256), 0, cvx_hip_stream(s), a, e);
    CVX_CHECK_LAUNCH("cvx_rk_stage_err_f32");
    return CVX_OK;
}

extern "C" int cvx_rk_err_finish_f32(const float* partials, const int32_t* map_dev, int32_t blocks, int32_t steps, int32_t n_seq, float* err,
                                     cvx_stream_t s)
{
    CVX_REQUIRE(partials && map_dev && err, "rk_err_finish: partials, map and err must not be null");
    CVX_REQUIRE(((uintptr_t)partials & 7) == 0 && ((uintptr_t)err & 7) == 0 && ((uintptr_t)map_dev & 3) == 0, "rk_err_finish: 8-byte aligned partials and err");
    CVX_REQUIRE(blocks >= 0 && steps >= 0 && n_seq >= 0 && (int64_t)steps * n_seq <= 0x7fffffffLL && (int64_t)steps * blocks <= 0x7fffffffLL,
                "rk_err_finish: bad sizes (blocks=%d steps=%d sequences=%d)", blocks, steps, n_seq);
    const int64_t n = (int64_t)steps * n_seq;
    if (n == 0) return CVX_OK;
    hipLaunchKernelGGL(rk_err_finish_kernel, dim3((unsigned)((n + 255) / 256)), dim3(256), 0, cvx_hip_stream(s),
                       reinterpret_cast<const float2*>(partials), map_dev, reinterpret_cast<float2*>(err), steps, n_seq, blocks);
    CVX_CHECK_LAUNCH("cvx_rk_err_finish_f32");
    return CVX_OK;
}

extern "C" int cvx_embed_gather_f32(const int64_t* ids, int32_t S, const float* table, int32_t E, int32_t n_rows_table,
                                    const float* cond, const float* cond_row, int32_t Cc, int64_t null_id,
                                    float* out, int64_t M, cvx_stream_t s)
{
    CVX_REQUIRE(table && out && S > 0 && E > 0 && Cc >= 0 && M >= 0, "embed_gather: bad arguments");
    CVX_REQUIRE(cond || cond_row || Cc == 0, "embed_gather: cond and cond_row both null");
    if (M == 0) return CVX_OK;
    hipLaunchKernelGGL(embed_gather_kernel, dim3((unsigned)M), dim3(256), 0, cvx_hip_stream(s),
                       ids, S, table, E, n_rows_table, cond, cond_row, Cc, null_id, out);
    CVX_CHECK_LAUNCH("cvx_embed_gather_f32");
    return CVX_OK;
}

extern "C" int cvx_time_fourier_f32(const float* times, const float* w, float* out, int32_t n, int32_t half, cvx_stream_t s)
{
    CVX_REQUIRE(times && w && out && n >= 0 && half > 0, "time_fourier: bad arguments");
    if (n == 0) return CVX_OK;
    hipLaunchKernelGGL(time_fourier_kernel, dim3(n), dim3(256), 0, cvx_hip_stream(s), times, w, out, half);
    CVX_CHECK_LAUNCH("cvx_time_fourier_f32");
    return CVX_OK;
}

extern "C" int cvx_wav_to_int16(const float* wav, int16_t* pcm, int64_t n, cvx_stream_t s)
{
    CVX_REQUIRE(wav && pcm && n >= 0, "wav_to_int16: bad arguments");
    if (n == 0) return CVX_OK;
    hipLaunchKernelGGL(wav_to_int16_kernel, dim3((unsigned)((n + 255) / 256)), dim3(256), 0, cvx_hip_stream(s), wav, pcm, n);
    CVX_CHECK_LAUNCH("cvx_wav_to_int16");
    return CVX_OK;
}
```

### neurips2024-covomix_amd/csrc/gemm_common.h

```cpp
#pragma once
#include "cvx_common.h"

namespace cvxg {

constexpr int BN = 128;
constexpr int BK = 32;

__device__ __forceinline__ void tile_of_block(int tiles_m, int tiles_n, int map_mode, int& tile_m, int& tile_n)
{
    if (map_mode == 1) {
        const int xcd = blockIdx.x & 7, slot = blockIdx.x >> 3;
        tile_m = xcd + 8 * (slot / tiles_n);
        tile_n = slot % tiles_n;
    } else {
        tile_n = blockIdx.x % tiles_n;
        tile_m = blockIdx.x / tiles_n;
    }
}

struct SplitOut { _Float16* hi; _Float16* lo; int64_t ldc_h; int write_f32;
                  _Float16* vt_hi; _Float16* vt_lo; int64_t vt_ld;
                  const float* c_scale; const float* vt_scale; const float* a_scale;
                  int dbg; unsigned long long* trace;
                  uint32_t* sat;
                  const float* tw_gamma; float* rowsq; int rowsq_ld; const float* row_scale;
                  const _Float16* res_hi; const _Float16* res_lo; int64_t res_ld; const float* res_scale;
                  const float* a2_scale; };

__device__ __forceinline__ float total_acc_scale(float acc_scale, const SplitOut& so)
{
    const float* s = so.a2_scale ? so.a2_scale : so.a_scale;
    return s ? acc_scale / *s : acc_scale;
}
typedef _Float16 cvx_f16x4 __attribute__((ext_vector_type(4)));

__device__ __forceinline__ int vt_slot(int t) { return (t & ~12) | ((t & 4) << 1) | ((t & 8) >> 1); }

__device__ __forceinline__ int il_col(int c) { return ((c >> 5) << 6) | (c & 31); }

__device__ __forceinline__ void store_split(const SplitOut& so, int64_t idx, float v, float& amax)
{
    const float x = fminf(fmaxf(v, -65504.f), 65504.f);
    amax = cvx_amax3_c(amax, v, v);
    const _Float16 h = (_Float16)x;
    so.hi[idx] = h;
    if (so.lo) so.lo[idx] = (_Float16)(x - (float)h);
}

__device__ __forceinline__ void quad_transpose(float& v0, float& v1, float& v2, float& v3, int lane)
{
    const bool b0 = (lane & 1) != 0, b1 = (lane & 2) != 0;
    float x = b0 ? v0 : v1, y = b0 ? v2 : v3;
    float rx = __shfl_xor(x, 1, 64), ry = __shfl_xor(y, 1, 64);
    const float a0 = b0 ? rx : v0, a1 = b0 ? v1 : rx, a2 = b0 ? ry : v2, a3 = b0 ? v3 : ry;
    x = b1 ? a0 : a2; y = b1 ? a1 : a3;
    rx = __shfl_xor(x, 2, 64); ry = __shfl_xor(y, 2, 64);
    v0 = b1 ? rx : a0; v1 = b1 ? ry : a1; v2 = b1 ? a2 : rx; v3 = b1 ? a3 : ry;
}

enum : int { EPI_GENERIC = 0, EPI_QKV = 1,
             EPI_RES = 2,
             EPI_GELU_SPLIT = 3,
             EPI_BIAS = 4,
             EPI_RES_TW = 5,
             EPI_BIAS_TW = 6,
             EPI_GELU_RS = 7,
             EPI_QKV_RS = 8 };

template <int TM, int EPI = EPI_GENERIC>
__device__ __forceinline__ void gemm_epilogue(const cvx_gemm_args& p_in, f32x16 (&acc)[TM][2], int m0, int n0,
                                              int wm, int wn, int lane,
                                              const SplitOut so_in = SplitOut{nullptr, nullptr, 0, 1, nullptr, nullptr, 0})
{
    cvx_gemm_args p = p_in;
    SplitOut so = so_in;
    if constexpr (EPI == EPI_QKV) {
        p.act = CVX_ACT_NONE; p.bias = nullptr; p.residual = nullptr; so.write_f32 = 0;
        __builtin_assume(p.rope_cos != nullptr); __builtin_assume(so.vt_hi != nullptr); __builtin_assume(so.hi != nullptr);
    } else if constexpr (EPI == EPI_RES) {
        p.act = CVX_ACT_NONE; p.rope_cos = nullptr; so.write_f32 = 1; so.vt_hi = nullptr; so.vt_lo = nullptr;
        __builtin_assume(p.residual != nullptr);
    } else if constexpr (EPI == EPI_GELU_SPLIT) {
        p.act = CVX_ACT_GELU; p.rope_cos = nullptr; p.residual = nullptr; so.write_f32 = 0; so.vt_hi = nullptr; so.vt_lo = nullptr;
        __builtin_assume(p.bias != nullptr); __builtin_assume(so.hi != nullptr);
    } else if constexpr (EPI == EPI_BIAS) {
        p.act = CVX_ACT_NONE; p.rope_cos = nullptr; p.residual = nullptr; so.write_f32 = 1; so.vt_hi = nullptr; so.vt_lo = nullptr;
        so.hi = nullptr; so.lo = nullptr;
    }
    const int colw = n0 + wn * 64;
    if (colw >= p.N) return;
    const int c_lo = colw + (lane & 31);
    const int c_hi = c_lo + 32;
    if (so.vt_hi != nullptr && colw >= p.rope_cols) {
        if (colw >= p.N) return;
        const int H = p.rope_cols / 128, T = p.rope_T;
        const int head = (colw - p.rope_cols) / 64;
        const float b_lo_v = (p.bias && c_lo < p.N) ? p.bias[c_lo] : 0.f;
        const float b_hi_v = (p.bias && c_hi < p.N) ? p.bias[c_hi] : 0.f;
        const float vs = so.vt_scale ? *so.vt_scale : 1.f;
#pragma unroll
        for (int mi = 0; mi < TM; ++mi) {
#pragma unroll
            for (int rg = 0; rg < 4; ++rg) {
                const int row0 = m0 + wm * TM * 32 + mi * 32 + 8 * rg + 4 * (lane >> 5);
                if (row0 >= p.M) continue;
                const int b = row0 / T, t0 = row0 - b * T;
#pragma unroll
                for (int hsel = 0; hsel < 2; ++hsel) {
                    const int d = (lane & 31) + 32 * hsel;
                    const float bias = hsel ? b_hi_v : b_lo_v;
                    cvx_f16x4 vh, vl;
                    float amax = 0.f;
#pragma unroll
                    for (int e = 0; e < 4; ++e) {
                        const float xr = (acc[mi][hsel][4 * rg + e] + bias) * vs;
                        amax = cvx_amax3_c(amax, xr, xr);
                        const float x = fminf(fmaxf(xr, -65504.f), 65504.f);
                        vh[e] = (_Float16)x;
                        vl[e] = (_Float16)(x - (float)vh[e]);
                    }
                    cvx_sat_commit(so.sat, amax);
                    const int64_t base = ((int64_t)(b * H + head) * 64 + d) * so.vt_ld;
                    if ((t0 & 3) == 0 && t0 + 3 < T && row0 + 3 < p.M) {
                        *reinterpret_cast<cvx_f16x4*>(so.vt_hi + base + vt_slot(t0)) = vh;
                        if (so.vt_lo) *reinterpret_cast<cvx_f16x4*>(so.vt_lo + base + vt_slot(t0)) = vl;
                    } else {
#pragma unroll
                        for (int e = 0; e < 4; ++e) {
                            const int row = row0 + e;
                            if (row >= p.M) break;
                            const int bb = row / T, tt = row - bb * T;
                            const int64_t idx = ((int64_t)(bb * H + head) * 64 + d) * so.vt_ld + vt_slot(tt);
                            so.vt_hi[idx] = vh[e];
                            if (so.vt_lo) so.vt_lo[idx] = vl[e];
                        }
                    }
                }
            }
        }
        return;
    }
    const bool do_rope = (p.rope_cos != nullptr) && (colw < p.rope_cols);
    const float cs = (so.hi && so.c_scale) ? *so.c_scale : 1.f;
    const float b_lo = (p.bias && c_lo < p.N) ? p.bias[c_lo] : 0.f;
    const float b_hi = (p.bias && c_hi < p.N) ? p.bias[c_hi] : 0.f;

    const bool vec_ok = (EPI != EPI_GENERIC) || ((colw + 64 <= p.N) &&
                        (!so.write_f32 || (((uintptr_t)p.C & 15) == 0 && (p.ldc & 3) == 0)) &&
                        (!p.residual || (((uintptr_t)p.residual & 15) == 0 && (p.ldr & 3) == 0)) &&
                        (!so.hi || ((((uintptr_t)so.hi | (uintptr_t)so.lo) & 7) == 0 && (so.ldc_h & 3) == 0)));
    if (vec_ok) {
        const int q = lane & 3;
        const int c4_lo = colw + 4 * ((lane & 31) >> 2);
        constexpr int RA = 2, NG = TM * 4;
        f32x4 rb[RA + 1][2];
        auto load_res = [&](int gi, f32x4 (&r)[2]) {
            const int row_ = min(m0 + wm * TM * 32 + (gi >> 2) * 32 + 8 * (gi & 3) + 4 * (lane >> 5) + q, p.M - 1);
            const float* rp = p.residual + (int64_t)row_ * p.ldr + c4_lo;
            r[0] = *reinterpret_cast<const f32x4*>(rp);
            r[1] = *reinterpret_cast<const f32x4*>(rp + 32);
        };
        if (p.residual) {
#pragma unroll
            for (int a = 0; a < RA && a < NG; ++a) load_res(a, rb[a]);
        }
#pragma unroll
        for (int mi = 0; mi < TM; ++mi) {
#pragma unroll
            for (int rg = 0; rg < 4; ++rg) {
                const int gi = mi * 4 + rg;
                if (p.residual && gi + RA < NG) load_res(gi + RA, rb[(gi + RA) % (RA + 1)]);
                const int row0 = m0 + wm * TM * 32 + mi * 32 + 8 * rg + 4 * (lane >> 5);
                float lo[4], hi[4];
#pragma unroll
                for (int e = 0; e < 4; ++e) {
                    lo[e] = acc[mi][0][4 * rg + e] + b_lo;
                    hi[e] = acc[mi][1][4 * rg + e] + b_hi;
                    if (p.act == CVX_ACT_GELU) { lo[e] = gelu_erf(lo[e]); hi[e] = gelu_erf(hi[e]); }
                    else if (p.act == CVX_ACT_SILU) { lo[e] = silu(lo[e]); hi[e] = silu(hi[e]); }
                    if (do_rope) {
                        const int pos = min(row0 + e, p.M - 1) % p.rope_T;
                        const float c = p.rope_cos[pos * 32 + (lane & 31)];
                        const float s = p.rope_sin[pos * 32 + (lane & 31)];
                        const float nlo = __builtin_fmaf(lo[e], c, -__fmul_rn(hi[e], s));
                        const float nhi = __builtin_fmaf(hi[e], c, __fmul_rn(lo[e], s));
                        lo[e] = nlo; hi[e] = nhi;
                    }
                }
                quad_transpose(lo[0], lo[1], lo[2], lo[3], lane);
                quad_transpose(hi[0], hi[1], hi[2], hi[3], lane);
                const int row = row0 + q;
                if (row >= p.M) continue;
                f32x4 vlo = {lo[0], lo[1], lo[2], lo[3]}, vhi = {hi[0], hi[1], hi[2], hi[3]};
                if (p.residual) {
                    const f32x4 r0 = rb[gi % (RA + 1)][0], r1 = rb[gi % (RA + 1)][1];
#pragma unroll
                    for (int e = 0; e < 4; ++e) { vlo[e] += r0[e]; vhi[e] += r1[e]; }
                }
                if (so.write_f32) {
                    float* cp = p.C + (int64_t)row * p.ldc + c4_lo;
                    *reinterpret_cast<f32x4*>(cp) = vlo;
                    *reinterpret_cast<f32x4*>(cp + 32) = vhi;
                }
                if (so.hi) {
                    const bool il = so.lo == so.hi + 32;
                    const int64_t o = (int64_t)row * so.ldc_h + (il ? il_col(c4_lo) : c4_lo);
                    const int64_t o32 = il ? 64 : 32;
                    cvx_f16x4 h0, l0, h1, l1;
                    float amax = 0.f;
#pragma unroll
                    for (int e = 0; e < 4; ++e) {
                        const float s0 = vlo[e] * cs, s1 = vhi[e] * cs;
                        amax = cvx_amax3_c(amax, s0, s1);
                        const float x0 = fminf(fmaxf(s0, -65504.f), 65504.f);
                        const float x1 = fminf(fmaxf(s1, -65504.f), 65504.f);
                        h0[e] = (_Float16)x0; l0[e] = (_Float16)(x0 - (float)h0[e]);
                        h1[e] = (_Float16)x1; l1[e] = (_Float16)(x1 - (float)h1[e]);
                    }
                    cvx_sat_commit(so.sat, amax);
                    *reinterpret_cast<cvx_f16x4*>(so.hi + o) = h0;
                    *reinterpret_cast<cvx_f16x4*>(so.hi + o + o32) = h1;
                    if (so.lo) {
                        *reinterpret_cast<cvx_f16x4*>(so.lo + o) = l0;
                        *reinterpret_cast<cvx_f16x4*>(so.lo + o + o32) = l1;
                    }
                }
            }
        }
        return;
    }
    float amax_s = 0.f;
#pragma unroll
    for (int mi = 0; mi < TM; ++mi) {
#pragma unroll
        for (int r = 0; r < 16; ++r) {
            const int row = m0 + wm * TM * 32 + mi * 32 + mfma32_row(r, lane);
            if (row >= p.M) continue;
            float lo = acc[mi][0][r] + b_lo;
            float hi = acc[mi][1][r] + b_hi;
            if (p.act == CVX_ACT_GELU) { lo = gelu_erf(lo); hi = gelu_erf(hi); }
            else if (p.act == CVX_ACT_SILU) { lo = silu(lo); hi = silu(hi); }
            if (do_rope) {
                const int pos = row % p.rope_T;
                const float c = p.rope_cos[pos * 32 + (lane & 31)];
                const float s = p.rope_sin[pos * 32 + (lane & 31)];
                const float nlo = __builtin_fmaf(lo, c, -__fmul_rn(hi, s));
                const float nhi = __builtin_fmaf(hi, c, __fmul_rn(lo, s));
                lo = nlo; hi = nhi;
            }
            if (p.residual) {
                if (c_lo < p.N) lo += p.residual[(int64_t)row * p.ldr + c_lo];
                if (c_hi < p.N) hi += p.residual[(int64_t)row * p.ldr + c_hi];
            }
            if (so.write_f32) {
                if (c_lo < p.N) p.C[(int64_t)row * p.ldc + c_lo] = lo;
                if (c_hi < p.N) p.C[(int64_t)row * p.ldc + c_hi] = hi;
            }
            if (so.hi) {
                const bool il = so.lo == so.hi + 32;
                if (c_lo < p.N) store_split(so, (int64_t)row * so.ldc_h + (il ? il_col(c_lo) : c_lo), lo * cs, amax_s);
                if (c_hi < p.N) store_split(so, (int64_t)row * so.ldc_h + (il ? il_col(c_hi) : c_hi), hi * cs, amax_s);
            }
        }
    }
    cvx_sat_commit(so.sat, amax_s);
}

__device__ __forceinline__ void glds16(const void* g, void* lds_wave_base)
{
    __builtin_amdgcn_global_load_lds((const __attribute__((address_space(1))) void*)(uintptr_t)g,
                                     (__attribute__((address_space(3))) void*)lds_wave_base, 16, 0, 0);
}

struct PreSplitA { const _Float16* hi; const _Float16* lo; int64_t ld; const _Float16* hi2; const _Float16* lo2; int64_t ld2; };

bool launch_gemm_f16x3_p8s(const cvx_gemm_args& a, const PreSplitA& A, const _Float16* w_il, float acc_scale, const SplitOut& so,
                           hipStream_t st, int n_cu);

bool launch_gemm_f16x3_p8m(const cvx_gemm_args& a, const PreSplitA& A, const _Float16* w_il, float acc_scale, const SplitOut& so,
                           int ksplit, float* partial, hipStream_t st);

int classify_epilogue(const cvx_gemm_args& a, const SplitOut& so);

int validate_gemm_args(const cvx_gemm_args* a);

}
```

### neurips2024-covomix_amd/csrc/gemm_f16x3.hip

```cpp
#include "gemm_common.h"

namespace {

using namespace cvxg;
typedef _Float16 f16;
typedef _Float16 f16x4 __attribute__((ext_vector_type(4)));
typedef _Float16 f16x8 __attribute__((ext_vector_type(8)));

constexpr int TILE_H = 128 * BK;
constexpr float F16_MAX = 65504.f;

__device__ __forceinline__ void split4(const f32x4 v, f16x4& hi, f16x4& lo, float pre, float& amax)
{
#pragma unroll
    for (int e = 0; e < 4; ++e) {
        amax = cvx_amax3_c(amax, v[e] * pre, v[e] * pre);
        const float x = fminf(fmaxf(v[e] * pre, -F16_MAX), F16_MAX);
        const f16 h = (f16)x;
        hi[e] = h;
        lo[e] = (f16)(x - (float)h);
    }
}

__global__ __launch_bounds__(256, 2) void gemm_f16x3_kernel(const cvx_gemm_args p, const f16* __restrict__ Whi,
                                                           const f16* __restrict__ Wlo, float acc_scale, SplitOut so,
                                                           int tiles_m, int tiles_n, int map_mode)
{
    constexpr int TM = 2, BM = 128;
    extern __shared__ __attribute__((aligned(16))) f16 smem_h[];
    f16* const S0 = smem_h;
    constexpr int STAGE = 4 * TILE_H;

    const int tid = threadIdx.x, lane = tid & 63, wid = tid >> 6;
    const int wm = wid >> 1, wn = wid & 1;
    int tile_m, tile_n;
    tile_of_block(tiles_m, tiles_n, map_mode, tile_m, tile_n);
    if (tile_m >= tiles_m) return;
    const int m0 = tile_m * BM, n0 = tile_n * BN;

    const int srow = tid >> 3, sj = tid & 7;
    const float* pa[4];
    int64_t a_jump[4];
    int a_st[4];
#pragma unroll
    for (int i = 0; i < 4; ++i) {
        const int r = srow + 32 * i;
        const int row = min(m0 + r, p.M - 1);
        pa[i] = p.A + (int64_t)row * p.lda + 4 * sj;
        a_jump[i] = p.A2 ? (p.A2 + (int64_t)row * p.lda2 + 4 * sj) - (pa[i] + p.K1) : 0;
        const int chunk = (sj >> 1) ^ ((r >> 2) & 3);
        a_st[i] = r * BK + chunk * 8 + (sj & 1) * 4;
    }
    const f16* pwh[2];
    const f16* pwl[2];
#pragma unroll
    for (int j = 0; j < 2; ++j) {
        const int r = 32 * wid + 16 * j + (lane >> 2);
        const int c = (lane & 3) ^ ((r >> 2) & 3);
        const int64_t off = (int64_t)min(n0 + r, p.N - 1) * p.ldw + 8 * c;
        pwh[j] = Whi + off;
        pwl[j] = Wlo + off;
    }
    const int dma_off = 32 * wid * BK;
    const int switch_tile = p.A2 ? p.K1 / BK : -1;

    f32x16 acc[TM][2];
#pragma unroll
    for (int mi = 0; mi < TM; ++mi)
#pragma unroll
        for (int ni = 0; ni < 2; ++ni)
#pragma unroll
            for (int r = 0; r < 16; ++r) acc[mi][ni][r] = 0.f;

    const int i31 = lane & 31, g = lane >> 5, swz = (i31 >> 2) & 3;
    int foff[2];
#pragma unroll
    for (int s = 0; s < 2; ++s) foff[s] = i31 * BK + 8 * ((2 * s + g) ^ swz);
    const int a_row0 = wm * 64 * BK, b_row0 = wn * 64 * BK;

    f32x4 ra[4];
    const int nk = p.K / BK;
    const float a_pre = so.a_scale ? *so.a_scale : 1.0f;
    float a_amax = 0.f;
    {
        const bool sw = (0 == switch_tile);
#pragma unroll
        for (int i = 0; i < 4; ++i) { if (sw) pa[i] += a_jump[i]; ra[i] = gload4(pa[i]); pa[i] += BK; }
#pragma unroll
        for (int j = 0; j < 2; ++j) {
            glds16(pwh[j], S0 + 2 * TILE_H + dma_off + 16 * j * BK);
            glds16(pwl[j], S0 + 3 * TILE_H + dma_off + 16 * j * BK);
            pwh[j] += BK; pwl[j] += BK;
        }
#pragma unroll
        for (int i = 0; i < 4; ++i) {
            f16x4 hi, lo;
            split4(ra[i], hi, lo, a_pre, a_amax);
            *reinterpret_cast<f16x4*>(S0 + a_st[i]) = hi;
            *reinterpret_cast<f16x4*>(S0 + TILE_H + a_st[i]) = lo;
        }
    }
    __syncthreads();

    for (int kt = 0; kt < nk; ++kt) {
        const int cur = kt & 1;
        const bool has_next = kt + 1 < nk;
        const int adv = has_next ? BK : 0;
        const bool sw = (kt + 1 == switch_tile);
        f16* const Sc = S0 + cur * STAGE;
        f16* const Sn = S0 + (cur ^ 1) * STAGE;
#pragma unroll
        for (int j = 0; j < 2; ++j) {
            const f16* sh = pwh[j] - (has_next ? 0 : BK);
            const f16* sl = pwl[j] - (has_next ? 0 : BK);
            glds16(sh, Sn + 2 * TILE_H + dma_off + 16 * j * BK);
            glds16(sl, Sn + 3 * TILE_H + dma_off + 16 * j * BK);
            pwh[j] = sh + adv; pwl[j] = sl + adv;
        }
#pragma unroll
        for (int i = 0; i < 4; ++i) {
            const float* src = pa[i] + (sw ? a_jump[i] : 0) - (has_next ? 0 : BK);
            ra[i] = gload4(src);
            pa[i] = src + adv;
        }
        const f16* ah = Sc + a_row0;
        const f16* al = Sc + TILE_H + a_row0;
        const f16* wh = Sc + 2 * TILE_H + b_row0;
        const f16* wl = Sc + 3 * TILE_H + b_row0;
#pragma unroll
        for (int s = 0; s < 2; ++s) {
            f16x8 fah[TM], fal[TM], fwh[2], fwl[2];
#pragma unroll
            for (int mi = 0; mi < TM; ++mi) {
                fah[mi] = *reinterpret_cast<const f16x8*>(ah + mi * 32 * BK + foff[s]);
                fal[mi] = *reinterpret_cast<const f16x8*>(al + mi * 32 * BK + foff[s]);
            }
#pragma unroll
            for (int ni = 0; ni < 2; ++ni) {
                fwh[ni] = *reinterpret_cast<const f16x8*>(wh + ni * 32 * BK + foff[s]);
                fwl[ni] = *reinterpret_cast<const f16x8*>(wl + ni * 32 * BK + foff[s]);
            }
#pragma unroll
            for (int mi = 0; mi < TM; ++mi)
#pragma unroll
                for (int ni = 0; ni < 2; ++ni)
                    acc[mi][ni] = __builtin_amdgcn_mfma_f32_32x32x16_f16(fal[mi], fwh[ni], acc[mi][ni], 0, 0, 0);
#pragma unroll
            for (int mi = 0; mi < TM; ++mi)
#pragma unroll
                for (int ni = 0; ni < 2; ++ni)
                    acc[mi][ni] = __builtin_amdgcn_mfma_f32_32x32x16_f16(fah[mi], fwl[ni], acc[mi][ni], 0, 0, 0);
#pragma unroll
            for (int mi = 0; mi < TM; ++mi)
#pragma unroll
                for (int ni = 0; ni < 2; ++ni)
                    acc[mi][ni] = __builtin_amdgcn_mfma_f32_32x32x16_f16(fah[mi], fwh[ni], acc[mi][ni], 0, 0, 0);
        }
#pragma unroll
        for (int i = 0; i < 4; ++i) {
            f16x4 hi, lo;
            split4(ra[i], hi, lo, a_pre, a_amax);
            *reinterpret_cast<f16x4*>(Sn + a_st[i]) = hi;
            *reinterpret_cast<f16x4*>(Sn + TILE_H + a_st[i]) = lo;
        }
        __syncthreads();
    }
    cvx_sat_commit(so.sat, a_amax);
    acc_scale = total_acc_scale(acc_scale, so);
    if (acc_scale != 1.0f) {
#pragma unroll
        for (int mi = 0; mi < TM; ++mi)
#pragma unroll
            for (int ni = 0; ni < 2; ++ni)
#pragma unroll
                for (int r = 0; r < 16; ++r) acc[mi][ni][r] *= acc_scale;
    }
    gemm_epilogue<TM>(p, acc, m0, n0, wm, wn, lane, so);
}


template <int STAGES, int NT>
__global__ __launch_bounds__(256, (STAGES <= 2 ? 2 : 1)) void gemm_f16x3_dma_kernel(
    const cvx_gemm_args p_in, const PreSplitA A, const f16* __restrict__ Whi, const f16* __restrict__ Wlo,
    float acc_scale, SplitOut so, int tiles_m, int tiles_n, int map_mode, int k_per, float* __restrict__ partial)
{
    cvx_gemm_args p = p_in;
    acc_scale = total_acc_scale(acc_scale, so);
    const int k_begin = k_per > 0 ? (int)blockIdx.y * k_per : 0;
    if (k_per > 0) {
        p.K = k_per;
        p.C = partial + (int64_t)blockIdx.y * p.M * p.N; p.ldc = p.N;
        p.bias = nullptr; p.residual = nullptr; p.act = CVX_ACT_NONE; p.rope_cos = nullptr;
        so = SplitOut{nullptr, nullptr, 0, 1, nullptr, nullptr, 0};
    }
    constexpr int TM = 2, BM = 128;
    constexpr int STAGE = 4 * TILE_H;
    extern __shared__ __attribute__((aligned(16))) f16 smem_h[];
    f16* const S0 = smem_h;

    const int tid = threadIdx.x, lane = tid & 63, wid = tid >> 6;
    const int wm = wid >> 1, wn = wid & 1;
    int tile_m, tile_n;
    tile_of_block(tiles_m, tiles_n, map_mode, tile_m, tile_n);
    if (tile_m >= tiles_m) return;
    const int m0 = tile_m * BM, n0 = tile_n * BN;

    const f16* pah[2]; const f16* pal[2]; const f16* pwh[2]; const f16* pwl[2];
    int64_t jmp_h[2], jmp_l[2];
#pragma unroll
    for (int j = 0; j < 2; ++j) {
        const int r = 32 * wid + 16 * j + (lane >> 2);
        const int c = (lane & 3) ^ ((r >> 2) & 3);
        const int64_t ra = min(m0 + r, p.M - 1), rw = min(n0 + r, p.N - 1);
        pah[j] = A.hi + ra * A.ld + 8 * c;
        jmp_h[j] = A.hi2 ? (A.hi2 + ra * A.ld2 + 8 * c) - (pah[j] + p.K1) : 0;
        pwh[j] = Whi + rw * p.ldw + 8 * c;
        if constexpr (NT == 1) {
            pal[j] = pah[j] + BK; jmp_l[j] = jmp_h[j]; pwl[j] = pwh[j] + BK;
        } else {
            pal[j] = A.lo + ra * A.ld + 8 * c;
            jmp_l[j] = A.lo2 ? (A.lo2 + ra * A.ld2 + 8 * c) - (pal[j] + p.K1) : 0;
            pwl[j] = Wlo + rw * p.ldw + 8 * c;
        }
    }
    constexpr int KSTEP = (NT == 1) ? 2 * BK : BK;
    const int dma_off = 32 * wid * BK;
    if (k_begin > 0) {
        const bool in2 = A.hi2 && k_begin >= p.K1;
#pragma unroll
        for (int j = 0; j < 2; ++j) {
            pah[j] += k_begin + (in2 ? jmp_h[j] : 0);
            pal[j] += k_begin + (in2 ? jmp_l[j] : 0);
            pwh[j] += k_begin; pwl[j] += k_begin;
        }
    }
    const int switch_tile = (A.hi2 && k_begin < p.K1) ? (p.K1 - k_begin) / KSTEP : -1;
    const int nk = p.K / KSTEP;

    auto issue = [&](int t) {
        f16* const S = S0 + (t % STAGES) * STAGE + dma_off;
        const bool live = t < nk;
        const bool sw = live && (t == switch_tile);
        const int back = live ? 0 : KSTEP, adv = live ? KSTEP : 0;
#pragma unroll
        for (int j = 0; j < 2; ++j) {
            const f16* sh = pah[j] + (sw ? jmp_h[j] : 0) - back;
            const f16* sl = pal[j] + (sw ? jmp_l[j] : 0) - back;
            const f16* wh = pwh[j] - back;
            const f16* wl = pwl[j] - back;
            glds16(sh, S + 16 * j * BK);
            glds16(sl, S + TILE_H + 16 * j * BK);
            glds16(wh, S + 2 * TILE_H + 16 * j * BK);
            glds16(wl, S + 3 * TILE_H + 16 * j * BK);
            if (live) { pah[j] = sh + adv; pal[j] = sl + adv; pwh[j] = wh + adv; pwl[j] = wl + adv; }
        }
    };

    f32x16 acc[TM][2];
#pragma unroll
    for (int mi = 0; mi < TM; ++mi)
#pragma unroll
        for (int ni = 0; ni < 2; ++ni)
#pragma unroll
            for (int r = 0; r < 16; ++r) acc[mi][ni][r] = 0.f;

    const int i31 = lane & 31, g = lane >> 5, swz = (i31 >> 2) & 3;
    int foff[2];
#pragma unroll
    for (int s = 0; s < 2; ++s) foff[s] = i31 * BK + 8 * ((2 * s + g) ^ swz);
    const int a_row0 = wm * 64 * BK, b_row0 = wn * 64 * BK;

#pragma unroll
    for (int t = 0; t < STAGES - 1; ++t) issue(t);

    for (int kt = 0; kt < nk; ++kt) {
        if constexpr (STAGES == 2) asm volatile("s_waitcnt vmcnt(0)" ::: "memory");
        else if constexpr (STAGES == 3) asm volatile("s_waitcnt vmcnt(8)" ::: "memory");
        else asm volatile("s_waitcnt vmcnt(16)" ::: "memory");
        __builtin_amdgcn_s_barrier();
        issue(kt + STAGES - 1);
        const f16* Sc = S0 + (kt % STAGES) * STAGE;
        const f16* ah = Sc + a_row0;
        const f16* al = Sc + TILE_H + a_row0;
        const f16* wh = Sc + 2 * TILE_H + b_row0;
        const f16* wl = Sc + 3 * TILE_H + b_row0;
#pragma unroll
        for (int s = 0; s < 2; ++s) {
            f16x8 fah[TM], fal[TM], fwh[2], fwl[2];
#pragma unroll
            for (int mi = 0; mi < TM; ++mi) {
                fah[mi] = *reinterpret_cast<const f16x8*>(ah + mi * 32 * BK + foff[s]);
                fal[mi] = *reinterpret_cast<const f16x8*>(al + mi * 32 * BK + foff[s]);
            }
#pragma unroll
            for (int ni = 0; ni < 2; ++ni) {
                fwh[ni] = *reinterpret_cast<const f16x8*>(wh + ni * 32 * BK + foff[s]);
                fwl[ni] = *reinterpret_cast<const f16x8*>(wl + ni * 32 * BK + foff[s]);
            }
            if constexpr (NT == 1) {
#pragma unroll
                for (int mi = 0; mi < TM; ++mi)
#pragma unroll
                    for (int ni = 0; ni < 2; ++ni)
                        acc[mi][ni] = __builtin_amdgcn_mfma_f32_32x32x16_f16(fah[mi], fwh[ni], acc[mi][ni], 0, 0, 0);
#pragma unroll
                for (int mi = 0; mi < TM; ++mi)
#pragma unroll
                    for (int ni = 0; ni < 2; ++ni)
                        acc[mi][ni] = __builtin_amdgcn_mfma_f32_32x32x16_f16(fal[mi], fwl[ni], acc[mi][ni], 0, 0, 0);
            } else {
#pragma unroll
            for (int mi = 0; mi < TM; ++mi)
#pragma unroll
                for (int ni = 0; ni < 2; ++ni)
                    acc[mi][ni] = __builtin_amdgcn_mfma_f32_32x32x16_f16(fal[mi], fwh[ni], acc[mi][ni], 0, 0, 0);
#pragma unroll
            for (int mi = 0; mi < TM; ++mi)
#pragma unroll
                for (int ni = 0; ni < 2; ++ni)
                    acc[mi][ni] = __builtin_amdgcn_mfma_f32_32x32x16_f16(fah[mi], fwl[ni], acc[mi][ni], 0, 0, 0);
#pragma unroll
            for (int mi = 0; mi < TM; ++mi)
#pragma unroll
                for (int ni = 0; ni < 2; ++ni)
                    acc[mi][ni] = __builtin_amdgcn_mfma_f32_32x32x16_f16(fah[mi], fwh[ni], acc[mi][ni], 0, 0, 0);
            }
        }
    }
    asm volatile("s_waitcnt vmcnt(0)" ::: "memory");
    if (acc_scale != 1.0f) {
#pragma unroll
        for (int mi = 0; mi < TM; ++mi)
#pragma unroll
            for (int ni = 0; ni < 2; ++ni)
#pragma unroll
                for (int r = 0; r < 16; ++r) acc[mi][ni][r] *= acc_scale;
    }
    gemm_epilogue<TM>(p, acc, m0, n0, wm, wn, lane, so);
}

__global__ __launch_bounds__(256) void split_f16_kernel(const float* __restrict__ w, f16* __restrict__ hi,
                                                       f16* __restrict__ lo, int64_t n, float scale, const float* __restrict__ scale_dev,
                                                       uint32_t* __restrict__ sat)
{
    const int64_t i = (int64_t)blockIdx.x * 256 + threadIdx.x;
    if (i >= n) return;
    if (scale_dev) scale *= *scale_dev;
    cvx_sat_commit(sat, fabsf(w[i] * scale));
    const float x = fminf(fmaxf(w[i] * scale, -F16_MAX), F16_MAX);
    const f16 h = (f16)x;
    const int64_t o = (lo == hi + 32) ? (((i >> 5) << 6) | (i & 31)) : i;
    hi[o] = h;
    if (lo) lo[o] = (f16)(x - (float)h);
}

__global__ __launch_bounds__(256) void split_colscale_il_kernel(const float* __restrict__ W, int64_t ldw, int N, int K,
                                                               const float* __restrict__ colscale, int64_t cs_ld,
                                                               const float* __restrict__ set_scale, int64_t ss_ld, int n_sets, float scale,
                                                               f16* __restrict__ out, uint32_t* __restrict__ sat)
{
    const int k4 = K / 4;
    const int64_t i = (int64_t)blockIdx.x * 256 + threadIdx.x;
    if (i >= (int64_t)N * k4) return;
    const int n = (int)(i / k4), k = 4 * (int)(i - (int64_t)n * k4);
    const f32x4 w = gload4(W + (int64_t)n * ldw + k);
    const int64_t o = (int64_t)n * 2 * K + (((k >> 5) << 6) | (k & 31));
    float amax = 0.f;
    for (int s = 0; s < n_sets; ++s) {
        const f32x4 g = gload4(colscale + (int64_t)s * cs_ld + k);
        const float sc = scale * (set_scale ? set_scale[(int64_t)s * ss_ld] : 1.f);
        cvx_f16x4 h, l;
#pragma unroll
        for (int e = 0; e < 4; ++e) {
            float x = w[e] * g[e] * sc;
            amax = cvx_amax3_c(amax, x, x);
            x = fminf(fmaxf(x, -F16_MAX), F16_MAX);
            h[e] = (f16)x;
            l[e] = (f16)(x - (float)h[e]);
        }
        f16* dst = out + (int64_t)s * N * 2 * K + o;
        *reinterpret_cast<cvx_f16x4*>(dst) = h;
        *reinterpret_cast<cvx_f16x4*>(dst + 32) = l;
    }
    cvx_sat_commit(sat, amax);
}

}

extern "C" int cvx_split_f16_colscale_il(const float* W, int64_t ldw, int32_t N, int32_t K, const float* colscale, int64_t cs_ld,
                                         const float* set_scale_dev, int64_t ss_ld, int32_t n_sets, float scale, uint16_t* out, cvx_stream_t s)
{
    CVX_REQUIRE(W && colscale && out && N > 0 && K > 0 && K % 32 == 0 && ldw >= K && ldw % 4 == 0 && cs_ld % 4 == 0 && n_sets >= 0 &&
                (((uintptr_t)W | (uintptr_t)colscale | (uintptr_t)out) & 15) == 0,
                "split_f16_colscale_il: bad arguments (N=%d K=%d ldw=%ld cs_ld=%ld; K %% 32 == 0, 16-byte aligned rows)", N, K, (long)ldw, (long)cs_ld);
    if (n_sets == 0) return CVX_OK;
    CVX_REQUIRE_SAT(s);
    const int64_t n = (int64_t)N * (K / 4);
    hipLaunchKernelGGL(split_colscale_il_kernel, dim3((unsigned)((n + 255) / 256)), dim3(256), 0, cvx_hip_stream(s),
                       W, ldw, N, K, colscale, cs_ld, set_scale_dev, ss_ld, n_sets, scale, reinterpret_cast<f16*>(out), cvx_sat_flag_for(s));
    CVX_CHECK_LAUNCH("cvx_split_f16_colscale_il");
    return CVX_OK;
}

extern "C" int cvx_split_f16_dev(const float* w, uint16_t* hi, uint16_t* lo, int64_t n, float scale, const float* scale_dev,
                                 cvx_stream_t s)
{
    CVX_REQUIRE(w && hi && n >= 0, "split_f16: bad arguments");
    CVX_REQUIRE(lo != hi + 32 || n % 32 == 0, "split_f16: an interleaved pair (lo == hi + 32) needs n %% 32 == 0 (n=%ld)", (long)n);
    if (n == 0) return CVX_OK;
    CVX_REQUIRE_SAT(s);
    hipLaunchKernelGGL(split_f16_kernel, dim3((unsigned)((n + 255) / 256)), dim3(256), 0, cvx_hip_stream(s),
                       w, reinterpret_cast<f16*>(hi), reinterpret_cast<f16*>(lo), n, scale, scale_dev, cvx_sat_flag_for(s));
    CVX_CHECK_LAUNCH("cvx_split_f16");
    return CVX_OK;
}

extern "C" int cvx_split_f16(const float* w, uint16_t* hi, uint16_t* lo, int64_t n, float scale, cvx_stream_t s)
{
    return cvx_split_f16_dev(w, hi, lo, n, scale, nullptr, s);
}


__global__ __launch_bounds__(256) void splitk_reduce_kernel(const float* __restrict__ partial, int ksplit, const cvx_gemm_args p, SplitOut so)
{
    const int64_t i4 = ((int64_t)blockIdx.x * 256 + threadIdx.x) * 4;
    const int64_t total = (int64_t)p.M * p.N;
    if (i4 >= total) return;
    const int row = (int)(i4 / p.N), col = (int)(i4 - (int64_t)row * p.N);
    f32x4 v = *reinterpret_cast<const f32x4*>(partial + i4);
    for (int s = 1; s < ksplit; ++s) {
        const f32x4 w = *reinterpret_cast<const f32x4*>(partial + (int64_t)s * total + i4);
#pragma unroll
        for (int e = 0; e < 4; ++e) v[e] += w[e];
    }
#pragma unroll
    for (int e = 0; e < 4; ++e) {
        float x = v[e] + (p.bias ? p.bias[col + e] : 0.f);
        if (p.act == CVX_ACT_GELU) x = gelu_erf(x);
        else if (p.act == CVX_ACT_SILU) x = silu(x);
        if (p.residual) x += p.residual[(int64_t)row * p.ldr + col + e];
        v[e] = x;
    }
    if (so.write_f32) *reinterpret_cast<f32x4*>(p.C + (int64_t)row * p.ldc + col) = v;
    if (so.hi) {
        const float cs = so.c_scale ? *so.c_scale : 1.f;
        float amax = 0.f;
#pragma unroll
        for (int e = 0; e < 4; ++e) store_split(so, (int64_t)row * so.ldc_h + ((so.lo == so.hi + 32) ? il_col(col + e) : col + e), v[e] * cs, amax);
        cvx_sat_commit(so.sat, amax);
    }
}

typedef _Float16 f16x4_r __attribute__((ext_vector_type(4)));
__device__ __forceinline__ void store_split4_r(_Float16* hi, _Float16* lo, int64_t row_off, int col, const f32x4 o, CvxSat& amax)
{
    cvx_amax4(amax, o);
    const int64_t off = row_off + ((lo == hi + 32) ? il_col(col) : col);
    f16x4_r h, l;
#pragma unroll
    for (int e = 0; e < 4; ++e) {
        const float x = fminf(fmaxf(o[e], -65504.f), 65504.f);
        h[e] = (_Float16)x;
        l[e] = (_Float16)(x - (float)h[e]);
    }
    *reinterpret_cast<f16x4_r*>(hi + off) = h;
    if (lo) *reinterpret_cast<f16x4_r*>(lo + off) = l;
}
template <int NW>
__global__ __launch_bounds__(64 * NW) void splitk_reduce_norm_kernel(const float* __restrict__ partial, int ksplit, const cvx_gemm_args p, SplitOut so,
                                                                    const cvx_gemm_norm nm)
{
    __shared__ float qs[NW][64];
    const int lane = threadIdx.x & 63, wv = threadIdx.x >> 6;
    const int row = (int)blockIdx.x;
    const int64_t total = (int64_t)p.M * p.N;
    const int col = 4 * (int)threadIdx.x;
    const float* pr = partial + (int64_t)row * p.N + col;
    f32x4 v = gload4(pr);
    const f32x4 gv = gload4(nm.gamma + col);
    f32x4 bv = f32x4{0.f, 0.f, 0.f, 0.f}, rv = bv, bi = bv;
    if (nm.beta) bv = gload4(nm.beta + col);
    if (p.residual) rv = gload4(p.residual + (int64_t)row * p.ldr + col);
    if (p.bias) bi = gload4(p.bias + col);
    for (int s = 1; s < ksplit; ++s) {
        const f32x4 w = gload4(pr + (int64_t)s * total);
#pragma unroll
        for (int e = 0; e < 4; ++e) v[e] += w[e];
    }
    const float cs = (so.hi && so.c_scale) ? *so.c_scale : 1.f;
    const float ys = nm.y_scale_dev ? *nm.y_scale_dev : 1.f;
    CvxSat amax;
#pragma unroll
    for (int e = 0; e < 4; ++e) {
        float x = v[e] + (p.bias ? bi[e] : 0.f);
        if (p.residual) x += rv[e];
        v[e] = x;
    }
    if (so.write_f32) *reinterpret_cast<f32x4*>(p.C + (int64_t)row * p.ldc + col) = v;
    if (so.hi) store_split4_r(so.hi, so.lo, (int64_t)row * so.ldc_h, col, f32x4{v[0] * cs, v[1] * cs, v[2] * cs, v[3] * cs}, amax);
    float ss = 0.f;
    ss += v[0] * v[0] + v[1] * v[1] + v[2] * v[2] + v[3] * v[3];
    if (NW > 1) {
        qs[wv][lane] = ss;
        __syncthreads();
        ss = 0.f;
#pragma unroll
        for (int w = 0; w < NW; ++w) ss += qs[w][lane];
    }
#pragma unroll
    for (int o = 32; o > 0; o >>= 1) ss += __shfl_xor(ss, o, 64);
    const float inv = nm.scale / fmaxf(sqrtf(ss), nm.eps);
    f32x4 o;
#pragma unroll
    for (int e = 0; e < 4; ++e) o[e] = v[e] * inv * gv[e];
    if (nm.beta) {
#pragma unroll
        for (int e = 0; e < 4; ++e) o[e] += bv[e];
    }
    store_split4_r(reinterpret_cast<_Float16*>(nm.Y_hi), reinterpret_cast<_Float16*>(nm.Y_lo), (int64_t)row * nm.ldy_h, col,
                   f32x4{o[0] * ys, o[1] * ys, o[2] * ys, o[3] * ys}, amax);
    cvx_sat_commit(so.sat, amax);
}

template <int STAGES, int NT>
static void launch_dma(const cvx_gemm_args& a, const PreSplitA& A, const f16* wh, const f16* wl, float acc_scale,
                       const SplitOut& so, dim3 grid, int tiles_m, int tiles_n, int map_mode, hipStream_t st,
                       int k_per = 0, float* partial = nullptr)
{
    const size_t lds = (size_t)STAGES * 4 * TILE_H * sizeof(f16);
    cvx_allow_dynamic_lds(reinterpret_cast<const void*>(&gemm_f16x3_dma_kernel<STAGES, NT>), (int)lds);
    hipLaunchKernelGGL((gemm_f16x3_dma_kernel<STAGES, NT>), grid, dim3(256), lds, st, a, A, wh, wl, acc_scale, so,
                       tiles_m, tiles_n, map_mode, k_per, partial);
}

constexpr int SPLITK_MAX_GRID = 128;

static int splitk_factor(int M, int N, int K, int K1, bool has_a2)
{
    const int tiles = ((N + BN - 1) / BN) * ((((M + 127) / 128) + 7) / 8 * 8);
    if (tiles > SPLITK_MAX_GRID || N % 4 != 0) return 1;
    for (int cand = 4; cand >= 2; cand >>= 1) {
        const int kp = K / cand;
        if (K % cand == 0 && kp % 64 == 0 && kp >= 512 && (!has_a2 || K1 % kp == 0)) return cand;
    }
    return 1;
}

static int splitk_factor_p8m(int M, int N, int K, int K1, bool has_a2)
{
    const int tiles = ((N + 127) / 128) * ((M + 127) / 128);
    if (N % 4 != 0) return 1;
    for (int cand = 8; cand >= 2; cand >>= 1) {
        const int kp = K / cand;
        if (tiles * cand <= (cand == 8 ? 128 : 256) && K % (32 * cand) == 0 && kp >= (cand == 8 ? 128 : 256) && (!has_a2 || K1 % kp == 0)) return cand;
    }
    return 1;
}

extern "C" int64_t cvx_gemm_f16x3_workspace_floats(int32_t M, int32_t N, int32_t K, int32_t K1)
{
    if (M <= 0 || N <= 0 || K <= 0) return 0;
    const int f = splitk_factor(M, N, K, K1, K1 > 0);
    const int g = M < 2048 ? splitk_factor_p8m(M, N, K, K1, K1 > 0) : 1;
    const int m = f > g ? f : g;
    return m > 1 ? (int64_t)m * M * N : 0;
}

static int gemm_f16x3_impl(const cvx_gemm_args* a, const uint16_t* W_hi, const uint16_t* W_lo, float acc_scale,
                           const cvx_gemm_split_io* io, const cvx_gemm_norm* norm, cvx_stream_t s);

extern "C" int cvx_gemm_f16x3(const cvx_gemm_args* a, const uint16_t* W_hi, const uint16_t* W_lo, float acc_scale,
                              const cvx_gemm_split_io* io, cvx_stream_t s)
{
    return gemm_f16x3_impl(a, W_hi, W_lo, acc_scale, io, nullptr, s);
}

extern "C" int cvx_gemm_f16x3_norm(const cvx_gemm_args* a, const uint16_t* W_hi, const uint16_t* W_lo, float acc_scale,
                                   const cvx_gemm_split_io* io, const cvx_gemm_norm* norm, cvx_stream_t s)
{
    CVX_REQUIRE(a && norm && norm->gamma && norm->Y_hi, "gemm_f16x3_norm: null pointer");
    CVX_REQUIRE(a->act == CVX_ACT_NONE && a->ldc == a->N && a->N % 4 == 0 && (!io || io->write_f32 != 0 || !io->C_hi) && !a->rope_cos,
                "gemm_f16x3_norm: needs act == NONE, a contiguous fp32 C (ldc == N, written) and no RoPE");
    CVX_REQUIRE((norm->Y_lo == norm->Y_hi + 32 && norm->ldy_h == 2 * (int64_t)a->N && a->N % 32 == 0) || norm->ldy_h == a->N,
                "gemm_f16x3_norm: Y must be an interleaved pair with ldy_h == 2N or a plain pair with ldy_h == N");
    return gemm_f16x3_impl(a, W_hi, W_lo, acc_scale, io, norm, s);
}

static int gemm_f16x3_impl(const cvx_gemm_args* a, const uint16_t* W_hi, const uint16_t* W_lo, float acc_scale,
                           const cvx_gemm_split_io* io, const cvx_gemm_norm* norm, cvx_stream_t s)
{
    const int rc = cvxg::validate_gemm_args(a);
    if (rc != CVX_OK) return rc;
    bool norm_done = false;
    CVX_REQUIRE(W_hi, "gemm_f16x3: null split weights");
    const bool single = (W_lo == nullptr);
    CVX_REQUIRE(a->K % BK == 0 && a->ldw % 8 == 0, "gemm_f16x3: K must be a multiple of 32 and ldw of 8 (K=%d ldw=%ld)", a->K, (long)a->ldw);
    CVX_REQUIRE((((uintptr_t)W_hi | (uintptr_t)W_lo) & 15) == 0, "gemm_f16x3: split weights must be 16-byte aligned");
    const bool w_il = io && io->w_interleaved != 0;
    const bool a_il = io && io->A_hi && io->A_lo == io->A_hi + 32;
    if (w_il)
        CVX_REQUIRE(!single && W_lo == W_hi + 32 && a->ldw >= 2 * (int64_t)a->K && a_il,
                    "gemm_f16x3: interleaved weights need W_lo == W_hi + 32, ldw >= 2K and an interleaved pre-split A");
    if (a_il)
        CVX_REQUIRE(w_il && io->lda_h >= 2 * (int64_t)(a->A2 ? a->K1 : a->K) &&
                    (!a->A2 || (io->A2_lo == io->A2_hi + 32 && io->lda2_h >= 2 * (int64_t)(a->K - a->K1))),
                    "gemm_f16x3: interleaved A needs interleaved weights, lda_h >= 2K and an interleaved A2");
    else
        CVX_REQUIRE(!(io && a->A2 && io->A2_hi && io->A2_lo == io->A2_hi + 32),
                    "gemm_f16x3: A2 is an interleaved pair but A is not (both operands must use the same layout)");
    if (single)
        CVX_REQUIRE(io && io->A_hi && a->K % (2 * BK) == 0 && (!a->A2 || a->K1 % (2 * BK) == 0),
                    "gemm_f16x3: the single-term mode (W_lo == NULL) needs a pre-split A and K (K1) a multiple of 64");
    if ((io && (io->C_hi || io->Vt_hi)) || norm) CVX_REQUIRE_SAT(s);
    SplitOut so{nullptr, nullptr, 0, 1, nullptr, nullptr, 0};
    so.sat = cvx_sat_flag_for(s);
    PreSplitA A{nullptr, nullptr, 0, nullptr, nullptr, 0};
    if (io) {
        if (io->C_hi || io->C_lo) {
            CVX_REQUIRE(io->C_hi && (io->C_lo || single) && io->ldc_h >= ((io->Vt_hi && a->rope_cols > 0) ? a->rope_cols : a->N), "gemm_f16x3: bad split output");
            so.hi = reinterpret_cast<f16*>(io->C_hi); so.lo = reinterpret_cast<f16*>(io->C_lo); so.ldc_h = io->ldc_h;
        }
        so.write_f32 = (io->write_f32 != 0 || so.hi == nullptr) ? 1 : 0;
        so.c_scale = io->c_scale_dev; so.vt_scale = io->vt_scale_dev; so.a_scale = io->a_scale_dev;
        so.tw_gamma = io->c_gamma_dev; so.rowsq = io->c_rowsq; so.rowsq_ld = (int)io->c_rowsq_ld; so.row_scale = io->a_row_scale_dev;
        so.res_hi = reinterpret_cast<const f16*>(io->R_hi); so.res_lo = reinterpret_cast<const f16*>(io->R_lo); so.res_ld = io->ldr_h;
        so.res_scale = io->r_scale_dev; so.a2_scale = io->a2_scale_dev;
        so.dbg = 0; so.trace = nullptr;
        if (io->flags & CVX_GEMM_FLAG_ONE_TILE) so.dbg |= 8;
        if (io->flags & CVX_GEMM_FLAG_TILE192) so.dbg |= 16;
        if (io->flags & CVX_GEMM_FLAG_TILE256) so.dbg |= 32;
        if (io->flags & CVX_GEMM_FLAG_TILE_MIXED) so.dbg |= 64;
        if (io->flags & CVX_GEMM_FLAG_VT_PIECES) so.dbg |= 128;
        if (io->Vt_hi || io->Vt_lo) {
            CVX_REQUIRE(io->Vt_hi && (io->Vt_lo || single) && so.hi && a->rope_cos && a->rope_cols > 0 && a->rope_cols % 128 == 0 &&
                        (a->N - a->rope_cols) * 2 == a->rope_cols && io->vt_ld >= ((a->rope_T + 15) / 16) * 16 && io->vt_ld % 8 == 0 &&
                        a->M % a->rope_T == 0 && so.write_f32 == 0,
                        "gemm_f16x3: QKV-transpose output needs the RoPE arguments, N = 3*H*64, vt_ld >= T rounded up to 16 and write_f32 = 0");
            so.vt_hi = reinterpret_cast<f16*>(io->Vt_hi); so.vt_lo = reinterpret_cast<f16*>(io->Vt_lo); so.vt_ld = io->vt_ld;
        }
        if (io->A_hi || io->A_lo) {
            CVX_REQUIRE(io->A_hi && (io->A_lo || single) && io->lda_h % 8 == 0 && (((uintptr_t)io->A_hi | (uintptr_t)io->A_lo) & 15) == 0,
                        "gemm_f16x3: bad pre-split A");
            A.hi = reinterpret_cast<const f16*>(io->A_hi); A.lo = reinterpret_cast<const f16*>(io->A_lo); A.ld = io->lda_h;
            if (a->A2) {
                CVX_REQUIRE(io->A2_hi && (io->A2_lo || single) && io->lda2_h % 8 == 0 &&
                            (((uintptr_t)io->A2_hi | (uintptr_t)io->A2_lo) & 15) == 0, "gemm_f16x3: bad pre-split A2");
                A.hi2 = reinterpret_cast<const f16*>(io->A2_hi); A.lo2 = reinterpret_cast<const f16*>(io->A2_lo); A.ld2 = io->lda2_h;
            }
        }
    }
    const bool dn = so.tw_gamma || so.rowsq || so.row_scale || so.res_hi || so.res_lo || so.a2_scale;
    if (dn) {
        CVX_REQUIRE(!single && !norm && a->N % 64 == 0 && (!so.tw_gamma || (so.hi && ((uintptr_t)so.tw_gamma & 15) == 0)) &&
                    (!so.rowsq || (io->c_rowsq_ld >= a->N / 64 && io->c_rowsq_ld < (1ll << 20))),
                    "gemm_f16x3: deferred norm needs N %% 64 == 0, a split output for c_gamma_dev (16-byte aligned) and c_rowsq_ld >= N / 64");
        CVX_REQUIRE((so.res_hi == nullptr) == (so.res_lo == nullptr) && (!so.res_hi || (!a->residual && io->ldr_h >= (so.res_lo == so.res_hi + 32 ? 2 : 1) * (int64_t)a->N)),
                    "gemm_f16x3: a pair residual needs R_hi and R_lo, ldr_h >= N (2N interleaved) and residual == NULL");
    }
    if (a->M == 0) return CVX_OK;
    const int tiles_n = (a->N + BN - 1) / BN, tiles_m = (a->M + 127) / 128;
    const int map_mode = 1;
    const int grid_m = map_mode == 1 ? ((tiles_m + 7) / 8) * 8 : tiles_m;
    dim3 grid((unsigned)(grid_m * tiles_n));
    hipStream_t st = cvx_hip_stream(s);
    const f16* wh = reinterpret_cast<const f16*>(W_hi);
    const f16* wl = reinterpret_cast<const f16*>(W_lo);
    bool medium = a->M < 2048 || a->N < 512;
    if (!medium && A.hi && w_il && a_il && io && !(io->flags & (CVX_GEMM_FLAG_NO_MEDIUM | CVX_GEMM_FLAG_ONE_TILE))) {
        const long ncu = cvx_ctx_cus(s);
        const long t256 = (long)((a->M + 255) / 256) * ((a->N + 255) / 256), t192 = (long)((a->M + 191) / 192) * ((a->N + 255) / 256);
        const long t128 = (long)((a->M + 127) / 128) * ((a->N + 127) / 128);
        const double r256 = (double)((t256 + ncu - 1) / ncu), r192 = 0.8 * (double)((t192 + ncu - 1) / ncu);
        const double large = r192 < r256 ? r192 : r256, med = 0.31 * (double)((t128 + ncu - 1) / ncu);
        medium = (io->flags & CVX_GEMM_FLAG_MEDIUM) || med < 0.97 * large;
    }
    if (dn) {
        CVX_REQUIRE(A.hi && w_il && a_il && a->M >= 2048 && a->N >= 512,
                    "gemm_f16x3: deferred norm (c_gamma_dev / c_rowsq / a_row_scale_dev) runs on the large-problem 16x16x32 kernel only: "
                    "interleaved pre-split operands, M >= 2048, N >= 512 (M=%d N=%d K=%d)", a->M, a->N, a->K);
        medium = false;
    }
    if (A.hi && w_il && a_il && medium) {
        int ksplit = 1;
        if (io->workspace && !a->rope_cos && !so.vt_hi && a->ldc % 4 == 0) {
            const int f = splitk_factor_p8m(a->M, a->N, a->K, a->K1, a->A2 != nullptr);
            if (f > 1 && io->workspace_floats >= (int64_t)f * a->M * a->N) ksplit = f;
        }
        CVX_REQUIRE(cvxg::launch_gemm_f16x3_p8m(*a, A, wh, acc_scale, so, ksplit, ksplit > 1 ? io->workspace : nullptr, st),
                    "gemm_f16x3: interleaved operands below 2048 rows need N %% 16 == 0 (N %% 64 == 0 with RoPE), 16-byte aligned C / residual / "
                    "bias / RoPE tables and rope_cols %% 128 == 0 (M=%d N=%d K=%d)", a->M, a->N, a->K);
        if (ksplit > 1 && norm && a->N <= 1024 && a->N % 256 == 0 && a->ldc % 4 == 0 && (!a->residual || a->ldr % 4 == 0)) {
            const dim3 g((unsigned)a->M);
            if (a->N == 1024) hipLaunchKernelGGL(splitk_reduce_norm_kernel<4>, g, dim3(256), 0, st, io->workspace, ksplit, *a, so, *norm);
            else if (a->N == 768) hipLaunchKernelGGL(splitk_reduce_norm_kernel<3>, g, dim3(192), 0, st, io->workspace, ksplit, *a, so, *norm);
            else if (a->N == 512) hipLaunchKernelGGL(splitk_reduce_norm_kernel<2>, g, dim3(128), 0, st, io->workspace, ksplit, *a, so, *norm);
            else hipLaunchKernelGGL(splitk_reduce_norm_kernel<1>, g, dim3(64), 0, st, io->workspace, ksplit, *a, so, *norm);
            norm_done = true;
        } else if (ksplit > 1) {
            const int64_t quads = ((int64_t)a->M * a->N + 3) / 4;
            hipLaunchKernelGGL(splitk_reduce_kernel, dim3((unsigned)((quads + 255) / 256)), dim3(256), 0, st, io->workspace, ksplit, *a, so);
        }
    } else if (A.hi && w_il && a_il) {
        if (!cvxg::launch_gemm_f16x3_p8s(*a, A, wh, acc_scale, so, st, cvx_ctx_cus(s))) {
            CVX_REQUIRE(!dn, "gemm_f16x3: deferred norm (c_gamma_dev / c_rowsq / a_row_scale_dev) needs N %% 64 == 0 and 16-byte aligned epilogue "
                             "operands (M=%d N=%d K=%d)", a->M, a->N, a->K);
            CVX_REQUIRE(cvxg::launch_gemm_f16x3_p8m(*a, A, wh, acc_scale, so, 1, nullptr, st),
                        "gemm_f16x3: interleaved operands need N %% 16 == 0 (N %% 64 == 0 with RoPE), 16-byte aligned C / residual / bias / RoPE "
                        "tables and rope_cols %% 128 == 0 (M=%d N=%d K=%d)", a->M, a->N, a->K);
        }
    } else if (A.hi) {
        int ksplit = 1;
        if (io && io->workspace && !a->rope_cos && !so.vt_hi && a->ldc % 4 == 0) {
            const int f = splitk_factor(a->M, a->N, a->K, a->K1, a->A2 != nullptr);
            if (f > 1 && io->workspace_floats >= (int64_t)f * a->M * a->N) ksplit = f;
        }
        const int k_per = ksplit > 1 ? a->K / ksplit : 0;
        float* part = ksplit > 1 ? io->workspace : nullptr;
        dim3 g2(grid.x, (unsigned)ksplit);
        const bool deep = (int)(grid.x * ksplit) <= 256;
        if (deep) {
            if (single) launch_dma<4, 1>(*a, A, wh, wl, acc_scale, so, g2, tiles_m, tiles_n, map_mode, st, k_per, part);
            else launch_dma<4, 3>(*a, A, wh, wl, acc_scale, so, g2, tiles_m, tiles_n, map_mode, st, k_per, part);
        } else if (single) launch_dma<2, 1>(*a, A, wh, wl, acc_scale, so, g2, tiles_m, tiles_n, map_mode, st, k_per, part);
        else launch_dma<2, 3>(*a, A, wh, wl, acc_scale, so, g2, tiles_m, tiles_n, map_mode, st, k_per, part);
        if (ksplit > 1) {
            const int64_t quads = ((int64_t)a->M * a->N + 3) / 4;
            hipLaunchKernelGGL(splitk_reduce_kernel, dim3((unsigned)((quads + 255) / 256)), dim3(256), 0, st, part, ksplit, *a, so);
        }
    } else {
        const size_t lds = (size_t)2 * 4 * TILE_H * sizeof(f16);
        cvx_allow_dynamic_lds(reinterpret_cast<const void*>(gemm_f16x3_kernel), (int)lds);
        hipLaunchKernelGGL(gemm_f16x3_kernel, grid, dim3(256), lds, st, *a, wh, wl, acc_scale, so, tiles_m, tiles_n, map_mode);
    }
    CVX_CHECK_LAUNCH("cvx_gemm_f16x3");
    if (norm && !norm_done)
        return cvx_adarmsnorm_scaled_f32(a->C, norm->gamma, norm->beta, nullptr, norm->Y_hi, norm->Y_lo, a->M, a->N, a->M > 0 ? a->M : 1,
                                         norm->scale, norm->eps, norm->y_scale_dev, s);
    return CVX_OK;
}
```

### neurips2024-covomix_amd/csrc/gemm_f16x3_p8m.hip

```cpp
#include "gemm_p8s_epi.h"

namespace {

constexpr int MT_B = 128 * 128;
constexpr int MBUF_B = 2 * MT_B;
constexpr int NBUF = 5;
constexpr int MLDS_B = NBUF * MBUF_B;

#define CVX_P8M_BARRIER() asm volatile("s_barrier" ::: "memory")
#define CVX_P8M_WAIT_DMA() asm volatile("s_waitcnt vmcnt(8)" ::: "memory")
#define CVX_P8M_WAIT_LDS() asm volatile("s_waitcnt lgkmcnt(0)" ::: "memory")

template <bool HAS_A2, bool SWAP, bool PERM = false>
__device__ __forceinline__ void tile_mainloop_m(const cvx_gemm_args& p, const PreSplitA& A, const f16* __restrict__ W, char* smem,
                                                int m0, int n0, int kt0, int nk, int lane, int grp, int w4, int wr, int wc,
                                                f32x4 (&acc)[4][4])
{
    const uint32_t lds0 = (uint32_t)(uintptr_t)(__attribute__((address_space(3))) char*)smem;
    uint32_t offA[4], offA2[4], offW[4];
    const int64_t ldaB = A.ld * 2, lda2B = A.ld2 * 2, ldwB = p.ldw * 2;
#pragma unroll
    for (int j = 0; j < 4; ++j) {
        const int r = 32 * w4 + 8 * j + (lane >> 3);
        const uint32_t c = (uint32_t)(((lane & 7) ^ ((r >> 1) & 7)) * 16);
        const uint32_t ga = (uint32_t)min(m0 + r, p.M - 1), gb = (uint32_t)min(n0 + (PERM ? perm32(r) : r), p.N - 1);
        offA[j] = ga * (uint32_t)ldaB + c;
        offA2[j] = HAS_A2 ? ga * (uint32_t)lda2B + c : 0u;
        offW[j] = gb * (uint32_t)ldwB + c;
    }
    const uint32_t dst0 = (uint32_t)(32 * w4 * 128);
    const int t_sw = HAS_A2 ? p.K1 / 32 : 0x7fffffff;
    const char* const a1base = reinterpret_cast<const char*>(A.hi);
    const char* const a2base = reinterpret_cast<const char*>(A.hi2);
    const char* const wbase = reinterpret_cast<const char*>(W);

    auto issue = [&](int t, int buf) {
        const bool live = t < nk;
        const int u = kt0 + t;
        const uint32_t b = lds0 + (uint32_t)buf * MBUF_B + dst0;
        const char* abase = a1base + (int64_t)u * 128;
        uint32_t a0 = offA[0], a1 = offA[1], a2 = offA[2], a3 = offA[3];
        if constexpr (HAS_A2) {
            if (u >= t_sw) { abase = a2base + (int64_t)(u - t_sw) * 128; a0 = offA2[0]; a1 = offA2[1]; a2 = offA2[2]; a3 = offA2[3]; }
        }
        const char* wb = wbase + (int64_t)u * 128;
        uint32_t w0 = offW[0], w1 = offW[1], w2 = offW[2], w3 = offW[3];
        if (!live) { abase = wbase; wb = wbase; a0 = a1 = a2 = a3 = 0u; w0 = w1 = w2 = w3 = 0u; }
        dma2(a0, a1, b, b + 1024u, abase);
        dma2(w0, w1, b + MT_B, b + MT_B + 1024u, wb);
        dma2(a2, a3, b + 2048u, b + 3072u, abase);
        dma2(w2, w3, b + MT_B + 2048u, b + MT_B + 3072u, wb);
    };

    const int lr = lane & 15, kg = lane >> 4, sw8 = lr >> 1;
    const int aoh = (wr * 64 + lr) * 128 + 16 * (kg ^ sw8);
    const int aol = (wr * 64 + lr) * 128 + 16 * ((4 + kg) ^ sw8);
    const int boh = MT_B + (wc * 64 + lr) * 128 + 16 * (kg ^ sw8);
    const int bol = MT_B + (wc * 64 + lr) * 128 + 16 * ((4 + kg) ^ sw8);

    f16x8 fah[4], fal[4], fbh[4], fbl[4];

    issue(grp, grp);
    issue(grp + 2, grp + 2);
    CVX_P8M_WAIT_DMA();
    CVX_P8M_BARRIER();
    if (grp == 1) CVX_P8M_BARRIER();

#define CVX_P8M_MM(x, y, c) (SWAP ? __builtin_amdgcn_mfma_f32_16x16x32_f16(y, x, c, 0, 0, 0) : __builtin_amdgcn_mfma_f32_16x16x32_f16(x, y, c, 0, 0, 0))
    const int nit = (nk + 1) >> 1;
    int t = grp, bi = grp;
    for (int it = 0; it < nit; ++it, t += 2) {
        const char* sb = smem + bi * MBUF_B;
        const int bn = bi + 4 >= NBUF ? bi + 4 - NBUF : bi + 4;
#pragma unroll
        for (int i = 0; i < 4; ++i) {
            fbh[i] = *reinterpret_cast<const f16x8*>(sb + i * 16 * 128 + boh);
            fbl[i] = *reinterpret_cast<const f16x8*>(sb + i * 16 * 128 + bol);
        }
#pragma unroll
        for (int i = 0; i < 4; ++i) {
            fah[i] = *reinterpret_cast<const f16x8*>(sb + i * 16 * 128 + aoh);
            fal[i] = *reinterpret_cast<const f16x8*>(sb + i * 16 * 128 + aol);
        }
        issue(t + 4, bn);
        CVX_P8M_WAIT_LDS();
        CVX_P8M_BARRIER();
        if (t < nk) {
            __builtin_amdgcn_sched_barrier(0);
            __builtin_amdgcn_s_setprio(1);
#pragma unroll
            for (int i = 0; i < 4; ++i)
#pragma unroll
                for (int j = 0; j < 4; ++j) acc[i][j] = CVX_P8M_MM(fal[i], fbh[j], acc[i][j]);
#pragma unroll
            for (int i = 0; i < 4; ++i)
#pragma unroll
                for (int j = 0; j < 4; ++j) acc[i][j] = CVX_P8M_MM(fah[i], fbl[j], acc[i][j]);
#pragma unroll
            for (int i = 0; i < 4; ++i)
#pragma unroll
                for (int j = 0; j < 4; ++j) acc[i][j] = CVX_P8M_MM(fah[i], fbh[j], acc[i][j]);
            __builtin_amdgcn_s_setprio(0);
            __builtin_amdgcn_sched_barrier(0);
        }
        CVX_P8M_WAIT_DMA();
        CVX_P8M_BARRIER();
        bi = bi + 2 >= NBUF ? bi + 2 - NBUF : bi + 2;
    }
#undef CVX_P8M_MM
    if (grp == 0) CVX_P8M_BARRIER();
    asm volatile("s_waitcnt vmcnt(0)" ::: "memory");
}

template <bool HAS_A2, int EPI, bool PERM = false>
__global__ __launch_bounds__(512, 2) void gemm_f16x3_p8m_kernel(
    const cvx_gemm_args p_in, const PreSplitA A, const f16* __restrict__ W, float acc_scale, SplitOut so,
    int tiles_m, int tiles_n, int ksplit, int k_per, float* __restrict__ partial)
{
    extern __shared__ __attribute__((aligned(16))) char smem_p8m[];
    const int tid = threadIdx.x, lane = tid & 63;
    const int wid = __builtin_amdgcn_readfirstlane(tid >> 6);
    const int grp = wid >> 2, w4 = wid & 3, wr = w4 >> 1, wc = w4 & 1;
    int unit, tm;
    if (tiles_n * ksplit >= 8) {
        const int xcd = (int)blockIdx.x & 7, q = (int)blockIdx.x >> 3;
        unit = (q / tiles_m) * 8 + xcd; tm = q % tiles_m;
    } else {
        unit = (int)blockIdx.x % (tiles_n * ksplit); tm = (int)blockIdx.x / (tiles_n * ksplit);
    }
    if (unit >= tiles_n * ksplit || tm >= tiles_m) return;
    const int tn = unit % tiles_n, ks = unit / tiles_n;
    const int m0 = tm * 128, n0 = tn * 128;
    cvx_gemm_args p = p_in;
    acc_scale = total_acc_scale(acc_scale, so);
    int kt0 = 0, nk = p.K / 32;
    if (ksplit > 1) {
        kt0 = ks * (k_per / 32); nk = k_per / 32;
        p.C = partial + (int64_t)ks * p.M * p.N; p.ldc = p.N;
        p.bias = nullptr;
    }

    f32x4 acc[4][4];
#pragma unroll
    for (int mi = 0; mi < 4; ++mi)
#pragma unroll
        for (int ni = 0; ni < 4; ++ni) acc[mi][ni] = f32x4{0.f, 0.f, 0.f, 0.f};
    bool v_block = false;
    if constexpr (EPI == EPI_QKV) v_block = n0 >= p.rope_cols;
    const int row0 = m0 + wr * 64 + grp * 32, col0 = n0 + wc * 64;
    EpiPre<2> pre;
    epilogue_prefetch<EPI, 2, PERM>(p, so, row0, col0, lane, v_block, pre);
    if (v_block) tile_mainloop_m<HAS_A2, false, PERM>(p, A, W, smem_p8m, m0, n0, kt0, nk, lane, grp, w4, wr, wc, acc);
    else tile_mainloop_m<HAS_A2, true, PERM>(p, A, W, smem_p8m, m0, n0, kt0, nk, lane, grp, w4, wr, wc, acc);

    CVX_P8M_BARRIER();
    f32x4* const X = reinterpret_cast<f32x4*>(smem_p8m);
    const int mine = ((grp * 4 + w4) * 8) * 64 + lane, theirs = (((1 - grp) * 4 + w4) * 8) * 64 + lane;
    if (grp == 0) {
#pragma unroll
        for (int i = 0; i < 2; ++i)
#pragma unroll
            for (int j = 0; j < 4; ++j) X[mine + (i * 4 + j) * 64] = acc[2 + i][j];
    } else {
#pragma unroll
        for (int i = 0; i < 2; ++i)
#pragma unroll
            for (int j = 0; j < 4; ++j) X[mine + (i * 4 + j) * 64] = acc[i][j];
    }
    CVX_P8M_WAIT_LDS();
    CVX_P8M_BARRIER();
    f32x4 e[2][4];
    if (grp == 0) {
#pragma unroll
        for (int i = 0; i < 2; ++i)
#pragma unroll
            for (int j = 0; j < 4; ++j) e[i][j] = acc[i][j] + X[theirs + (i * 4 + j) * 64];
    } else {
#pragma unroll
        for (int i = 0; i < 2; ++i)
#pragma unroll
            for (int j = 0; j < 4; ++j) e[i][j] = X[theirs + (i * 4 + j) * 64] + acc[2 + i][j];
    }
    if (so.dbg & 1) return;
    if (v_block) epilogue_vt<2, true, false, PERM>(p, e, row0, col0, lane, so, acc_scale, &pre);
    else epilogue_rows<EPI, 2, true, PERM ? 1 : 0>(p, e, row0, col0, lane, so, acc_scale, &pre);
}

}

namespace cvxg {

bool launch_gemm_f16x3_p8m(const cvx_gemm_args& a, const PreSplitA& A, const f16* w_il, float acc_scale, const SplitOut& so,
                           int ksplit, float* partial, hipStream_t st)
{
    if (a.K % 32 != 0 || (A.hi2 && a.K1 % 32 != 0) || a.N % 16 != 0 || (a.N % 64 != 0 && (a.rope_cos || so.vt_hi))) return false;
    if ((int64_t)a.M * A.ld * 2 >= (int64_t)1 << 32 || (A.hi2 && (int64_t)a.M * A.ld2 * 2 >= (int64_t)1 << 32) ||
        (int64_t)a.N * a.ldw * 2 >= (int64_t)1 << 32) return false;
    SplitOut s2 = so;
    cvx_gemm_args a2 = a;
    int k_per = 0;
    if (ksplit > 1) {
        if (a.K % (32 * ksplit) != 0 || !partial || a.rope_cos || so.vt_hi) return false;
        k_per = a.K / ksplit;
        a2.act = CVX_ACT_NONE; a2.residual = nullptr; a2.rope_cos = nullptr; a2.rope_sin = nullptr;
        a2.C = partial; a2.ldc = a.N;
        s2.hi = nullptr; s2.lo = nullptr; s2.write_f32 = 1; s2.vt_hi = nullptr; s2.vt_lo = nullptr;
    }
    const bool vec = (!s2.write_f32 || (((uintptr_t)a2.C & 15) == 0 && (a2.ldc & 3) == 0)) &&
                     (!a2.residual || (((uintptr_t)a2.residual & 15) == 0 && (a2.ldr & 3) == 0)) &&
                     (!s2.hi || ((((uintptr_t)s2.hi | (uintptr_t)s2.lo) & 7) == 0 && (s2.ldc_h & 3) == 0)) &&
                     (!a2.bias || ((uintptr_t)a2.bias & 15) == 0) &&
                     (!a2.rope_cos || ((((uintptr_t)a2.rope_cos | (uintptr_t)a2.rope_sin) & 15) == 0 && a2.rope_cols % 128 == 0));
    if (!vec) return false;
    if (s2.vt_hi && !(a2.rope_cos && s2.hi && !s2.write_f32 && !a2.residual && a2.act == CVX_ACT_NONE)) return false;
    const int tn = (a.N + 127) / 128, tm = (a.M + 127) / 128;
    const int units = tn * (ksplit > 1 ? ksplit : 1);
    const dim3 grid((unsigned)(units >= 8 ? ((units + 7) / 8) * 8 * tm : units * tm));
    int epi = ksplit > 1 ? (int)EPI_BIAS : classify_epilogue(a2, s2);
    if (epi == EPI_QKV && a2.bias) epi = EPI_GENERIC;
    if (epi == EPI_GENERIC && s2.vt_hi) return false;
    const int ks = ksplit > 1 ? ksplit : 1;
    const bool perm = ksplit <= 1 && !A.hi2 && (epi == EPI_QKV || epi == EPI_GELU_SPLIT) && a.N % 64 == 0 && s2.hi &&
                      (((uintptr_t)s2.hi | (uintptr_t)s2.lo) & 15) == 0 && (s2.ldc_h & 7) == 0;
#define CVX_P8M_LAUNCH_P(E)                                                                                              \
    do {                                                                                                                \
        cvx_allow_dynamic_lds(reinterpret_cast<const void*>(&gemm_f16x3_p8m_kernel<false, E, true>), MLDS_B);            \
        hipLaunchKernelGGL((gemm_f16x3_p8m_kernel<false, E, true>), grid, dim3(512), MLDS_B, st, a2, A, w_il, acc_scale, s2, tm, tn, ks, k_per, partial); \
    } while (0)
    if (perm) {
        if (epi == EPI_QKV) CVX_P8M_LAUNCH_P(EPI_QKV); else CVX_P8M_LAUNCH_P(EPI_GELU_SPLIT);
        return true;
    }
#undef CVX_P8M_LAUNCH_P
#define CVX_P8M_LAUNCH(A2, E)                                                                                           \
    do {                                                                                                                \
        cvx_allow_dynamic_lds(reinterpret_cast<const void*>(&gemm_f16x3_p8m_kernel<A2, E>), MLDS_B);                    \
        hipLaunchKernelGGL((gemm_f16x3_p8m_kernel<A2, E>), grid, dim3(512), MLDS_B, st, a2, A, w_il, acc_scale, s2, tm, tn, ks, k_per, partial); \
    } while (0)
    if (A.hi2) {
        if (epi == EPI_BIAS) CVX_P8M_LAUNCH(true, EPI_BIAS); else CVX_P8M_LAUNCH(true, EPI_GENERIC);
    } else {
        switch (epi) {
            case EPI_QKV: CVX_P8M_LAUNCH(false, EPI_QKV); break;
            case EPI_RES: CVX_P8M_LAUNCH(false, EPI_RES); break;
            case EPI_GELU_SPLIT: CVX_P8M_LAUNCH(false, EPI_GELU_SPLIT); break;
            case EPI_BIAS: CVX_P8M_LAUNCH(false, EPI_BIAS); break;
            default: CVX_P8M_LAUNCH(false, EPI_GENERIC); break;
        }
    }
#undef CVX_P8M_LAUNCH
    return true;
}

}
```

Measured before the change: 23580 mel-frames/s.

## Add 64-row p8m GEMM tiles for narrow GEMMs and LDS-staged dwconv31

Result: no change. 23570 mel-frames/s, median of 3 (-0.0%).

```diff
diff --git a/include/covomix_hip.h b/include/covomix_hip.h
--- a/include/covomix_hip.h
+++ b/include/covomix_hip.h
@@ -76,6 +76,7 @@
 #define CVX_GEMM_FLAG_TILE256 128
 #define CVX_GEMM_FLAG_TILE_MIXED 32
 #define CVX_GEMM_FLAG_VT_PIECES 512
+#define CVX_GEMM_FLAG_MEDIUM_TILE128 1024
 int cvx_split_f16(const float* w, uint16_t* hi, uint16_t* lo, int64_t n, float scale, cvx_stream_t s);
 int cvx_split_f16_colscale_il(const float* W, int64_t ldw, int32_t N, int32_t K, const float* colscale, int64_t cs_ld,
                               const float* set_scale_dev, int64_t ss_ld, int32_t n_sets, float scale, uint16_t* out, cvx_stream_t s);
@@ -91,6 +92,7 @@
 int cvx_gemm_f16x3_norm(const cvx_gemm_args* a, const uint16_t* W_hi, const uint16_t* W_lo, float acc_scale,
                         const cvx_gemm_split_io* io, const cvx_gemm_norm* norm, cvx_stream_t s);
 int64_t cvx_gemm_f16x3_workspace_floats(int32_t M, int32_t N, int32_t K, int32_t K1);
+int cvx_gemm_f16x3_medium_tile_rows(int32_t M, int32_t N, int32_t K1, int32_t ksplit, int32_t flags, cvx_stream_t s);
 
 int cvx_adarmsnorm_f32(const float* x, const float* gamma, const float* beta, float* y,
                        uint16_t* y_hi, uint16_t* y_lo,
@@ -133,6 +135,11 @@
                               int32_t Bt, int32_t T, int32_t C, cvx_stream_t s);
 int cvx_dwconv31_gelu_res_varlen_f32(const float* x, const float* w, const float* bias, float* y,
                                      const int32_t* cu_seqlens_dev, int32_t n_seq, int32_t max_T, int32_t C, cvx_stream_t s);
+#define CVX_DWCONV_FORM_AUTO   0
+#define CVX_DWCONV_FORM_WINDOW 1
+#define CVX_DWCONV_FORM_STAGED 2
+int cvx_dwconv31_gelu_res_form_f32(const float* x, const float* w, const float* bias, float* y,
+                                   const int32_t* cu_seqlens_dev, int32_t n_seq, int32_t max_T, int32_t C, int32_t form, cvx_stream_t s);
 int cvx_gemm_skinny_f32(const float* A, int32_t lda, const float* W, int64_t ldw, const float* bias, float* C, int64_t ldc,
                         int32_t M, int32_t N, int32_t K, int32_t act, cvx_stream_t s);
 int cvx_cfg_combine_axpy_f32(const float* f_c, const float* f_n, const float* y, float cond_scale,
diff --git a/neurips2024-covomix_amd/_lib.py b/neurips2024-covomix_amd/_lib.py
--- a/neurips2024-covomix_amd/_lib.py
+++ b/neurips2024-covomix_amd/_lib.py
@@ -334,6 +334,9 @@
                                       C.c_int32, C.c_int32, C.c_void_p]),
     "cvx_dwconv31_gelu_res_varlen_f32": (C.c_int, [C.c_void_p, C.c_void_p, C.c_void_p, C.c_void_p, C.c_void_p, C.c_int32,
                                                    C.c_int32, C.c_int32, C.c_void_p]),
+    "cvx_gemm_f16x3_medium_tile_rows": (C.c_int, [C.c_int32, C.c_int32, C.c_int32, C.c_int32, C.c_int32, C.c_void_p]),
+    "cvx_dwconv31_gelu_res_form_f32": (C.c_int, [C.c_void_p, C.c_void_p, C.c_void_p, C.c_void_p, C.c_void_p, C.c_int32,
+                                                 C.c_int32, C.c_int32, C.c_int32, C.c_void_p]),
 }
 
 _lib = None
diff --git a/neurips2024-covomix_amd/csrc/elementwise.hip b/neurips2024-covomix_amd/csrc/elementwise.hip
--- a/neurips2024-covomix_amd/csrc/elementwise.hip
+++ b/neurips2024-covomix_amd/csrc/elementwise.hip
@@ -258,6 +258,62 @@
         const int t = t0 + o;
         if (t < T) y[base + (int64_t)t * C + c] = g2[0] + xs[o + DW_K / 2];
         if (t + 1 < T) y[base + (int64_t)(t + 1) * C + c] = g2[1] + xs[o + 1 + DW_K / 2];
+    }
+}
+
+constexpr int DWS_CH = 64, DWS_FR = 64, DWS_ROWS = DWS_FR + DW_K - 1;
+static_assert(DWS_FR % DW_TT == 0 && DWS_FR / DW_TT == 4, "one wave per DW_TT frames, four waves per block");
+__global__ __launch_bounds__(256) void dwconv31_staged_kernel(const float* __restrict__ x, const float* __restrict__ w,
+                                                             const float* __restrict__ bias, float* __restrict__ y,
+                                                             int T, int C, const int* __restrict__ cu_seqlens)
+{
+    __shared__ __attribute__((aligned(16))) float win[DWS_ROWS * DWS_CH];
+    __shared__ __attribute__((aligned(16))) float res[DWS_FR * DWS_CH];
+    const int tid = threadIdx.x;
+    const int c0 = blockIdx.x * DWS_CH, t0 = blockIdx.y * DWS_FR;
+    int64_t base = (int64_t)blockIdx.z * T * C;
+    if (cu_seqlens) {
+        const int r0 = cu_seqlens[blockIdx.z];
+        T = cu_seqlens[blockIdx.z + 1] - r0;
+        base = (int64_t)r0 * C;
+        if (t0 >= T) return;
+    }
+    const int q4 = (tid & 15) * 4, srow = tid >> 4;
+    const bool quad_in = c0 + q4 < C;
+    const f32x4 zero4 = {0.f, 0.f, 0.f, 0.f};
+#pragma unroll
+    for (int i0 = 0; i0 < DWS_ROWS; i0 += 16) {
+        const int i = i0 + srow, t = t0 + i - DW_K / 2;
+        if (i < DWS_ROWS)
+            *reinterpret_cast<f32x4*>(win + i * DWS_CH + q4) =
+                (quad_in && t >= 0 && t < T) ? *reinterpret_cast<const f32x4*>(x + base + (int64_t)t * C + c0 + q4) : zero4;
+    }
+    __syncthreads();
+    const int cl = tid & 63, g = tid >> 6, c = c0 + cl;
+    if (c < C && t0 + DW_TT * g < T) {
+        float wk[DW_K];
+#pragma unroll
+        for (int k = 0; k < DW_K; ++k) wk[k] = w[c * DW_K + k];
+        float xs[DW_TT + DW_K - 1];
+#pragma unroll
+        for (int i = 0; i < DW_TT + DW_K - 1; ++i) xs[i] = win[(DW_TT * g + i) * DWS_CH + cl];
+        const float bc = bias[c];
+#pragma unroll
+        for (int o = 0; o < DW_TT; o += 2) {
+            float a0 = bc, a1 = bc;
+#pragma unroll
+            for (int k = 0; k < DW_K; ++k) { a0 = fmaf(wk[k], xs[o + k], a0); a1 = fmaf(wk[k], xs[o + 1 + k], a1); }
+            const f32x2 g2 = gelu_fast2(f32x2{a0, a1});
+            res[(DW_TT * g + o) * DWS_CH + cl] = g2[0] + xs[o + DW_K / 2];
+            res[(DW_TT * g + o + 1) * DWS_CH + cl] = g2[1] + xs[o + 1 + DW_K / 2];
+        }
+    }
+    __syncthreads();
+#pragma unroll
+    for (int i0 = 0; i0 < DWS_FR; i0 += 16) {
+        const int i = i0 + srow, t = t0 + i;
+        if (quad_in && t < T)
+            *reinterpret_cast<f32x4*>(y + base + (int64_t)t * C + c0 + q4) = *reinterpret_cast<const f32x4*>(res + i * DWS_CH + q4);
     }
 }
 
@@ -725,17 +781,33 @@
     return CVX_OK;
 }
 
-extern "C" int cvx_dwconv31_gelu_res_varlen_f32(const float* x, const float* w, const float* bias, float* y,
-                                                const int32_t* cu_seqlens_dev, int32_t Bt, int32_t max_T, int32_t C, cvx_stream_t s)
+extern "C" int cvx_dwconv31_gelu_res_form_f32(const float* x, const float* w, const float* bias, float* y,
+                                              const int32_t* cu_seqlens_dev, int32_t Bt, int32_t max_T, int32_t C, int32_t form,
+                                              cvx_stream_t s)
 {
     CVX_REQUIRE(x && w && bias && y, "dwconv31: null pointer");
     CVX_REQUIRE(Bt >= 0 && max_T > 0 && C > 0 && Bt <= 65535, "dwconv31: bad shape");
     CVX_REQUIRE(x != y, "dwconv31: in-place operation is not supported");
+    CVX_REQUIRE(form >= CVX_DWCONV_FORM_AUTO && form <= CVX_DWCONV_FORM_STAGED, "dwconv31: unknown form %d", form);
+    const bool can_stage = C % 4 == 0 && (((uintptr_t)x | (uintptr_t)y) & 15) == 0;
+    CVX_REQUIRE(form != CVX_DWCONV_FORM_STAGED || can_stage, "dwconv31: the staged form needs C %% 4 == 0 and 16-byte aligned x, y");
     if (Bt == 0) return CVX_OK;
-    dim3 grid((C + 255) / 256, (max_T + DW_TT - 1) / DW_TT, Bt);
-    hipLaunchKernelGGL(dwconv31_kernel, grid, dim3(256), 0, cvx_hip_stream(s), x, w, bias, y, max_T, C, cu_seqlens_dev);
+    if (form != CVX_DWCONV_FORM_WINDOW && can_stage) {
+        CVX_REQUIRE((max_T + DWS_FR - 1) / DWS_FR <= 65535, "dwconv31: bad shape");
+        dim3 grid((C + DWS_CH - 1) / DWS_CH, (max_T + DWS_FR - 1) / DWS_FR, Bt);
+        hipLaunchKernelGGL(dwconv31_staged_kernel, grid, dim3(256), 0, cvx_hip_stream(s), x, w, bias, y, max_T, C, cu_seqlens_dev);
+    } else {
+        dim3 grid((C + 255) / 256, (max_T + DW_TT - 1) / DW_TT, Bt);
+        hipLaunchKernelGGL(dwconv31_kernel, grid, dim3(256), 0, cvx_hip_stream(s), x, w, bias, y, max_T, C, cu_seqlens_dev);
+    }
     CVX_CHECK_LAUNCH("cvx_dwconv31_gelu_res_f32");
     return CVX_OK;
+}
+
+extern "C" int cvx_dwconv31_gelu_res_varlen_f32(const float* x, const float* w, const float* bias, float* y,
+                                                const int32_t* cu_seqlens_dev, int32_t Bt, int32_t max_T, int32_t C, cvx_stream_t s)
+{
+    return cvx_dwconv31_gelu_res_form_f32(x, w, bias, y, cu_seqlens_dev, Bt, max_T, C, CVX_DWCONV_FORM_AUTO, s);
 }
 
 extern "C" int cvx_gemm_skinny_f32(const float* A, int32_t lda, const float* W, int64_t ldw, const float* bias, float* C, int64_t ldc,
diff --git a/neurips2024-covomix_amd/csrc/gemm_common.h b/neurips2024-covomix_amd/csrc/gemm_common.h
--- a/neurips2024-covomix_amd/csrc/gemm_common.h
+++ b/neurips2024-covomix_amd/csrc/gemm_common.h
@@ -278,7 +278,8 @@
                            hipStream_t st, int n_cu);
 
 bool launch_gemm_f16x3_p8m(const cvx_gemm_args& a, const PreSplitA& A, const _Float16* w_il, float acc_scale, const SplitOut& so,
-                           int ksplit, float* partial, hipStream_t st);
+                           int ksplit, float* partial, hipStream_t st, int n_cu);
+int gemm_p8m_tile_rows(int M, int N, bool has_a2, int ksplit, bool pin128, int n_cu);
 
 int classify_epilogue(const cvx_gemm_args& a, const SplitOut& so);
 
diff --git a/neurips2024-covomix_amd/csrc/gemm_f16x3.hip b/neurips2024-covomix_amd/csrc/gemm_f16x3.hip
--- a/neurips2024-covomix_amd/csrc/gemm_f16x3.hip
+++ b/neurips2024-covomix_amd/csrc/gemm_f16x3.hip
@@ -568,6 +568,12 @@
 
 static int gemm_f16x3_impl(const cvx_gemm_args* a, const uint16_t* W_hi, const uint16_t* W_lo, float acc_scale,
                            const cvx_gemm_split_io* io, const cvx_gemm_norm* norm, cvx_stream_t s);
+
+extern "C" int cvx_gemm_f16x3_medium_tile_rows(int32_t M, int32_t N, int32_t K1, int32_t ksplit, int32_t flags, cvx_stream_t s)
+{
+    if (M < 1 || N < 1 || K1 < 0 || ksplit < 1) return -1;
+    return cvxg::gemm_p8m_tile_rows(M, N, K1 > 0, ksplit, (flags & CVX_GEMM_FLAG_MEDIUM_TILE128) != 0, cvx_ctx_cus(s));
+}
 
 extern "C" int cvx_gemm_f16x3(const cvx_gemm_args* a, const uint16_t* W_hi, const uint16_t* W_lo, float acc_scale,
                               const cvx_gemm_split_io* io, cvx_stream_t s)
@@ -631,6 +637,7 @@
         if (io->flags & CVX_GEMM_FLAG_TILE256) so.dbg |= 32;
         if (io->flags & CVX_GEMM_FLAG_TILE_MIXED) so.dbg |= 64;
         if (io->flags & CVX_GEMM_FLAG_VT_PIECES) so.dbg |= 128;
+        if (io->flags & CVX_GEMM_FLAG_MEDIUM_TILE128) so.dbg |= 256;
         if (io->Vt_hi || io->Vt_lo) {
             CVX_REQUIRE(io->Vt_hi && (io->Vt_lo || single) && so.hi && a->rope_cos && a->rope_cols > 0 && a->rope_cols % 128 == 0 &&
                         (a->N - a->rope_cols) * 2 == a->rope_cols && io->vt_ld >= ((a->rope_T + 15) / 16) * 16 && io->vt_ld % 8 == 0 &&
@@ -686,7 +693,7 @@
             const int f = splitk_factor_p8m(a->M, a->N, a->K, a->K1, a->A2 != nullptr);
             if (f > 1 && io->workspace_floats >= (int64_t)f * a->M * a->N) ksplit = f;
         }
-        CVX_REQUIRE(cvxg::launch_gemm_f16x3_p8m(*a, A, wh, acc_scale, so, ksplit, ksplit > 1 ? io->workspace : nullptr, st),
+        CVX_REQUIRE(cvxg::launch_gemm_f16x3_p8m(*a, A, wh, acc_scale, so, ksplit, ksplit > 1 ? io->workspace : nullptr, st, cvx_ctx_cus(s)),
                     "gemm_f16x3: interleaved operands below 2048 rows need N %% 16 == 0 (N %% 64 == 0 with RoPE), 16-byte aligned C / residual / "
                     "bias / RoPE tables and rope_cols %% 128 == 0 (M=%d N=%d K=%d)", a->M, a->N, a->K);
         if (ksplit > 1 && norm && a->N <= 1024 && a->N % 256 == 0 && a->ldc % 4 == 0 && (!a->residual || a->ldr % 4 == 0)) {
@@ -704,7 +711,7 @@
         if (!cvxg::launch_gemm_f16x3_p8s(*a, A, wh, acc_scale, so, st, cvx_ctx_cus(s))) {
             CVX_REQUIRE(!dn, "gemm_f16x3: deferred norm (c_gamma_dev / c_rowsq / a_row_scale_dev) needs N %% 64 == 0 and 16-byte aligned epilogue "
                              "operands (M=%d N=%d K=%d)", a->M, a->N, a->K);
-            CVX_REQUIRE(cvxg::launch_gemm_f16x3_p8m(*a, A, wh, acc_scale, so, 1, nullptr, st),
+            CVX_REQUIRE(cvxg::launch_gemm_f16x3_p8m(*a, A, wh, acc_scale, so, 1, nullptr, st, cvx_ctx_cus(s)),
                         "gemm_f16x3: interleaved operands need N %% 16 == 0 (N %% 64 == 0 with RoPE), 16-byte aligned C / residual / bias / RoPE "
                         "tables and rope_cols %% 128 == 0 (M=%d N=%d K=%d)", a->M, a->N, a->K);
         }
diff --git a/neurips2024-covomix_amd/csrc/gemm_f16x3_p8m.hip b/neurips2024-covomix_amd/csrc/gemm_f16x3_p8m.hip
--- a/neurips2024-covomix_amd/csrc/gemm_f16x3_p8m.hip
+++ b/neurips2024-covomix_amd/csrc/gemm_f16x3_p8m.hip
@@ -8,27 +8,30 @@
 constexpr int MLDS_B = NBUF * MBUF_B;
 
 #define CVX_P8M_BARRIER() asm volatile("s_barrier" ::: "memory")
-#define CVX_P8M_WAIT_DMA() asm volatile("s_waitcnt vmcnt(8)" ::: "memory")
+#define CVX_P8M_WAIT_DMA() do { if constexpr (BM == 128) asm volatile("s_waitcnt vmcnt(8)" ::: "memory"); \
+                                else asm volatile("s_waitcnt vmcnt(6)" ::: "memory"); } while (0)
 #define CVX_P8M_WAIT_LDS() asm volatile("s_waitcnt lgkmcnt(0)" ::: "memory")
 
-template <bool HAS_A2, bool SWAP, bool PERM = false>
+template <bool HAS_A2, bool SWAP, bool PERM = false, int BM = 128>
 __device__ __forceinline__ void tile_mainloop_m(const cvx_gemm_args& p, const PreSplitA& A, const f16* __restrict__ W, char* smem,
                                                 int m0, int n0, int kt0, int nk, int lane, int grp, int w4, int wr, int wc,
-                                                f32x4 (&acc)[4][4])
-{
+                                                f32x4 (&acc)[BM / 32][4])
+{
+    constexpr int RM = BM / 32;
     const uint32_t lds0 = (uint32_t)(uintptr_t)(__attribute__((address_space(3))) char*)smem;
     uint32_t offA[4], offA2[4], offW[4];
     const int64_t ldaB = A.ld * 2, lda2B = A.ld2 * 2, ldwB = p.ldw * 2;
 #pragma unroll
     for (int j = 0; j < 4; ++j) {
         const int r = 32 * w4 + 8 * j + (lane >> 3);
-        const uint32_t c = (uint32_t)(((lane & 7) ^ ((r >> 1) & 7)) * 16);
-        const uint32_t ga = (uint32_t)min(m0 + r, p.M - 1), gb = (uint32_t)min(n0 + (PERM ? perm32(r) : r), p.N - 1);
-        offA[j] = ga * (uint32_t)ldaB + c;
-        offA2[j] = HAS_A2 ? ga * (uint32_t)lda2B + c : 0u;
+        const int ra = BM == 128 ? r : 8 * RM * w4 + 8 * (j < RM ? j : 0) + (lane >> 3);
+        const uint32_t c = (uint32_t)(((lane & 7) ^ ((r >> 1) & 7)) * 16), ca = (uint32_t)(((lane & 7) ^ ((ra >> 1) & 7)) * 16);
+        const uint32_t ga = (uint32_t)min(m0 + ra, p.M - 1), gb = (uint32_t)min(n0 + (PERM ? perm32(r) : r), p.N - 1);
+        offA[j] = ga * (uint32_t)ldaB + ca;
+        offA2[j] = HAS_A2 ? ga * (uint32_t)lda2B + ca : 0u;
         offW[j] = gb * (uint32_t)ldwB + c;
     }
-    const uint32_t dst0 = (uint32_t)(32 * w4 * 128);
+    const uint32_t dst0 = (uint32_t)(32 * w4 * 128), dstA0 = (uint32_t)(8 * RM * w4 * 128);
     const int t_sw = HAS_A2 ? p.K1 / 32 : 0x7fffffff;
     const char* const a1base = reinterpret_cast<const char*>(A.hi);
     const char* const a2base = reinterpret_cast<const char*>(A.hi2);
@@ -37,7 +40,7 @@
     auto issue = [&](int t, int buf) {
         const bool live = t < nk;
         const int u = kt0 + t;
-        const uint32_t b = lds0 + (uint32_t)buf * MBUF_B + dst0;
+        const uint32_t b = lds0 + (uint32_t)buf * MBUF_B + dst0, ba = lds0 + (uint32_t)buf * MBUF_B + dstA0;
         const char* abase = a1base + (int64_t)u * 128;
         uint32_t a0 = offA[0], a1 = offA[1], a2 = offA[2], a3 = offA[3];
         if constexpr (HAS_A2) {
@@ -46,19 +49,19 @@
         const char* wb = wbase + (int64_t)u * 128;
         uint32_t w0 = offW[0], w1 = offW[1], w2 = offW[2], w3 = offW[3];
         if (!live) { abase = wbase; wb = wbase; a0 = a1 = a2 = a3 = 0u; w0 = w1 = w2 = w3 = 0u; }
-        dma2(a0, a1, b, b + 1024u, abase);
+        dma2(a0, a1, ba, ba + 1024u, abase);
         dma2(w0, w1, b + MT_B, b + MT_B + 1024u, wb);
-        dma2(a2, a3, b + 2048u, b + 3072u, abase);
+        if constexpr (BM == 128) dma2(a2, a3, ba + 2048u, ba + 3072u, abase);
         dma2(w2, w3, b + MT_B + 2048u, b + MT_B + 3072u, wb);
     };
 
     const int lr = lane & 15, kg = lane >> 4, sw8 = lr >> 1;
-    const int aoh = (wr * 64 + lr) * 128 + 16 * (kg ^ sw8);
-    const int aol = (wr * 64 + lr) * 128 + 16 * ((4 + kg) ^ sw8);
+    const int aoh = (wr * (BM / 2) + lr) * 128 + 16 * (kg ^ sw8);
+    const int aol = (wr * (BM / 2) + lr) * 128 + 16 * ((4 + kg) ^ sw8);
     const int boh = MT_B + (wc * 64 + lr) * 128 + 16 * (kg ^ sw8);
     const int bol = MT_B + (wc * 64 + lr) * 128 + 16 * ((4 + kg) ^ sw8);
 
-    f16x8 fah[4], fal[4], fbh[4], fbl[4];
+    f16x8 fah[RM], fal[RM], fbh[4], fbl[4];
 
     issue(grp, grp);
     issue(grp + 2, grp + 2);
@@ -78,7 +81,7 @@
             fbl[i] = *reinterpret_cast<const f16x8*>(sb + i * 16 * 128 + bol);
         }
 #pragma unroll
-        for (int i = 0; i < 4; ++i) {
+        for (int i = 0; i < RM; ++i) {
             fah[i] = *reinterpret_cast<const f16x8*>(sb + i * 16 * 128 + aoh);
             fal[i] = *reinterpret_cast<const f16x8*>(sb + i * 16 * 128 + aol);
         }
@@ -89,15 +92,15 @@
             __builtin_amdgcn_sched_barrier(0);
             __builtin_amdgcn_s_setprio(1);
 #pragma unroll
-            for (int i = 0; i < 4; ++i)
+            for (int i = 0; i < RM; ++i)
 #pragma unroll
                 for (int j = 0; j < 4; ++j) acc[i][j] = CVX_P8M_MM(fal[i], fbh[j], acc[i][j]);
 #pragma unroll
-            for (int i = 0; i < 4; ++i)
+            for (int i = 0; i < RM; ++i)
 #pragma unroll
                 for (int j = 0; j < 4; ++j) acc[i][j] = CVX_P8M_MM(fah[i], fbl[j], acc[i][j]);
 #pragma unroll
-            for (int i = 0; i < 4; ++i)
+            for (int i = 0; i < RM; ++i)
 #pragma unroll
                 for (int j = 0; j < 4; ++j) acc[i][j] = CVX_P8M_MM(fah[i], fbh[j], acc[i][j]);
             __builtin_amdgcn_s_setprio(0);
@@ -112,7 +115,7 @@
     asm volatile("s_waitcnt vmcnt(0)" ::: "memory");
 }
 
-template <bool HAS_A2, int EPI, bool PERM = false>
+template <bool HAS_A2, int EPI, bool PERM = false, int BM = 128>
 __global__ __launch_bounds__(512, 2) void gemm_f16x3_p8m_kernel(
     const cvx_gemm_args p_in, const PreSplitA A, const f16* __restrict__ W, float acc_scale, SplitOut so,
     int tiles_m, int tiles_n, int ksplit, int k_per, float* __restrict__ partial)
@@ -130,7 +133,9 @@
     }
     if (unit >= tiles_n * ksplit || tm >= tiles_m) return;
     const int tn = unit % tiles_n, ks = unit / tiles_n;
-    const int m0 = tm * 128, n0 = tn * 128;
+    constexpr int RM = BM / 32, RE = BM / 64;
+    static_assert(BM == 128 || (BM == 64 && EPI != EPI_QKV), "the V^T epilogue exchanges row groups in pairs");
+    const int m0 = tm * BM, n0 = tn * 128;
     cvx_gemm_args p = p_in;
     acc_scale = total_acc_scale(acc_scale, so);
     int kt0 = 0, nk = p.K / 32;
@@ -140,58 +145,66 @@
         p.bias = nullptr;
     }
 
-    f32x4 acc[4][4];
-#pragma unroll
-    for (int mi = 0; mi < 4; ++mi)
+    f32x4 acc[RM][4];
+#pragma unroll
+    for (int mi = 0; mi < RM; ++mi)
 #pragma unroll
         for (int ni = 0; ni < 4; ++ni) acc[mi][ni] = f32x4{0.f, 0.f, 0.f, 0.f};
     bool v_block = false;
     if constexpr (EPI == EPI_QKV) v_block = n0 >= p.rope_cols;
-    const int row0 = m0 + wr * 64 + grp * 32, col0 = n0 + wc * 64;
-    EpiPre<2> pre;
-    epilogue_prefetch<EPI, 2, PERM>(p, so, row0, col0, lane, v_block, pre);
-    if (v_block) tile_mainloop_m<HAS_A2, false, PERM>(p, A, W, smem_p8m, m0, n0, kt0, nk, lane, grp, w4, wr, wc, acc);
-    else tile_mainloop_m<HAS_A2, true, PERM>(p, A, W, smem_p8m, m0, n0, kt0, nk, lane, grp, w4, wr, wc, acc);
+    const int row0 = m0 + wr * (BM / 2) + grp * (BM / 4), col0 = n0 + wc * 64;
+    EpiPre<RE> pre;
+    epilogue_prefetch<EPI, RE, PERM>(p, so, row0, col0, lane, v_block, pre);
+    if (BM == 128 && v_block) tile_mainloop_m<HAS_A2, false, PERM, BM>(p, A, W, smem_p8m, m0, n0, kt0, nk, lane, grp, w4, wr, wc, acc);
+    else tile_mainloop_m<HAS_A2, true, PERM, BM>(p, A, W, smem_p8m, m0, n0, kt0, nk, lane, grp, w4, wr, wc, acc);
 
     CVX_P8M_BARRIER();
     f32x4* const X = reinterpret_cast<f32x4*>(smem_p8m);
     const int mine = ((grp * 4 + w4) * 8) * 64 + lane, theirs = (((1 - grp) * 4 + w4) * 8) * 64 + lane;
     if (grp == 0) {
 #pragma unroll
-        for (int i = 0; i < 2; ++i)
-#pragma unroll
-            for (int j = 0; j < 4; ++j) X[mine + (i * 4 + j) * 64] = acc[2 + i][j];
-    } else {
-#pragma unroll
-        for (int i = 0; i < 2; ++i)
+        for (int i = 0; i < RE; ++i)
+#pragma unroll
+            for (int j = 0; j < 4; ++j) X[mine + (i * 4 + j) * 64] = acc[RE + i][j];
+    } else {
+#pragma unroll
+        for (int i = 0; i < RE; ++i)
 #pragma unroll
             for (int j = 0; j < 4; ++j) X[mine + (i * 4 + j) * 64] = acc[i][j];
     }
     CVX_P8M_WAIT_LDS();
     CVX_P8M_BARRIER();
-    f32x4 e[2][4];
+    f32x4 e[RE][4];
     if (grp == 0) {
 #pragma unroll
-        for (int i = 0; i < 2; ++i)
+        for (int i = 0; i < RE; ++i)
 #pragma unroll
             for (int j = 0; j < 4; ++j) e[i][j] = acc[i][j] + X[theirs + (i * 4 + j) * 64];
     } else {
 #pragma unroll
-        for (int i = 0; i < 2; ++i)
-#pragma unroll
-            for (int j = 0; j < 4; ++j) e[i][j] = X[theirs + (i * 4 + j) * 64] + acc[2 + i][j];
+        for (int i = 0; i < RE; ++i)
+#pragma unroll
+            for (int j = 0; j < 4; ++j) e[i][j] = X[theirs + (i * 4 + j) * 64] + acc[RE + i][j];
     }
     if (so.dbg & 1) return;
-    if (v_block) epilogue_vt<2, true, false, PERM>(p, e, row0, col0, lane, so, acc_scale, &pre);
-    else epilogue_rows<EPI, 2, true, PERM ? 1 : 0>(p, e, row0, col0, lane, so, acc_scale, &pre);
+    if constexpr (BM == 128) {
+        if (v_block) { epilogue_vt<2, true, false, PERM>(p, e, row0, col0, lane, so, acc_scale, &pre); return; }
+    }
+    epilogue_rows<EPI, RE, true, PERM ? 1 : 0>(p, e, row0, col0, lane, so, acc_scale, &pre);
 }
 
 }
 
 namespace cvxg {
 
+int gemm_p8m_tile_rows(int M, int N, bool has_a2, int ksplit, bool pin128, int n_cu)
+{
+    const long tiles128 = (((long)M + 127) / 128) * (((long)N + 127) / 128);
+    return (!pin128 && !has_a2 && ksplit <= 1 && M >= 2048 && N <= 128 && tiles128 < n_cu) ? 64 : 128;
+}
+
 bool launch_gemm_f16x3_p8m(const cvx_gemm_args& a, const PreSplitA& A, const f16* w_il, float acc_scale, const SplitOut& so,
-                           int ksplit, float* partial, hipStream_t st)
+                           int ksplit, float* partial, hipStream_t st, int n_cu)
 {
     if (a.K % 32 != 0 || (A.hi2 && a.K1 % 32 != 0) || a.N % 16 != 0 || (a.N % 64 != 0 && (a.rope_cos || so.vt_hi))) return false;
     if ((int64_t)a.M * A.ld * 2 >= (int64_t)1 << 32 || (A.hi2 && (int64_t)a.M * A.ld2 * 2 >= (int64_t)1 << 32) ||
@@ -213,13 +226,29 @@
                      (!a2.rope_cos || ((((uintptr_t)a2.rope_cos | (uintptr_t)a2.rope_sin) & 15) == 0 && a2.rope_cols % 128 == 0));
     if (!vec) return false;
     if (s2.vt_hi && !(a2.rope_cos && s2.hi && !s2.write_f32 && !a2.residual && a2.act == CVX_ACT_NONE)) return false;
-    const int tn = (a.N + 127) / 128, tm = (a.M + 127) / 128;
-    const int units = tn * (ksplit > 1 ? ksplit : 1);
-    const dim3 grid((unsigned)(units >= 8 ? ((units + 7) / 8) * 8 * tm : units * tm));
     int epi = ksplit > 1 ? (int)EPI_BIAS : classify_epilogue(a2, s2);
     if (epi == EPI_QKV && a2.bias) epi = EPI_GENERIC;
     if (epi == EPI_GENERIC && s2.vt_hi) return false;
     const int ks = ksplit > 1 ? ksplit : 1;
+    const int bm = (epi == EPI_QKV || s2.vt_hi) ? 128 : gemm_p8m_tile_rows(a.M, a.N, A.hi2 != nullptr, ks, (so.dbg & 256) != 0, n_cu);
+    const int tn = (a.N + 127) / 128, tm = (a.M + bm - 1) / bm;
+    const int units = tn * (ksplit > 1 ? ksplit : 1);
+    const dim3 grid((unsigned)(units >= 8 ? ((units + 7) / 8) * 8 * tm : units * tm));
+    if (bm == 64) {
+#define CVX_P8M_LAUNCH_N(E)                                                                                              \
+    do {                                                                                                                \
+        cvx_allow_dynamic_lds(reinterpret_cast<const void*>(&gemm_f16x3_p8m_kernel<false, E, false, 64>), MLDS_B);       \
+        hipLaunchKernelGGL((gemm_f16x3_p8m_kernel<false, E, false, 64>), grid, dim3(512), MLDS_B, st, a2, A, w_il, acc_scale, s2, tm, tn, ks, k_per, partial); \
+    } while (0)
+        switch (epi) {
+            case EPI_RES: CVX_P8M_LAUNCH_N(EPI_RES); break;
+            case EPI_GELU_SPLIT: CVX_P8M_LAUNCH_N(EPI_GELU_SPLIT); break;
+            case EPI_BIAS: CVX_P8M_LAUNCH_N(EPI_BIAS); break;
+            default: CVX_P8M_LAUNCH_N(EPI_GENERIC); break;
+        }
+#undef CVX_P8M_LAUNCH_N
+        return true;
+    }
     const bool perm = ksplit <= 1 && !A.hi2 && (epi == EPI_QKV || epi == EPI_GELU_SPLIT) && a.N % 64 == 0 && s2.hi &&
                       (((uintptr_t)s2.hi | (uintptr_t)s2.lo) & 15) == 0 && (s2.ldc_h & 7) == 0;
 #define CVX_P8M_LAUNCH_P(E)                                                                                              \
```
